# ThotDjehuty/polaroid

Hardware: AMD Instinct MI355X
Metric: Mrows/sec filter+groupby-agg on 1e9-row f64/i64; achieved HBM GB/s vs peak (higher is better)
Workload: dtype f64; 1 GPU; filter(close > 250).group_by(symbol).agg(open/high/low/close.sum()) 1e+09 rows per GPU, 100 groups (metric size; configs[1] = 1e8 rows); rows_per_gpu=1000000000, groups=100, global_batch=1000000000, columns=symbol:i64 open,high,low,close:f64, parallelism=single GPU

## Files before the change

### polaroid_amd/csrc/groupby.hip

```cpp
#include <hip/hip_runtime.h>

#include <algorithm>
#include <cmath>
#include <cstdio>
#include <cstdlib>
#include <cstring>
#include <mutex>
#include <numeric>
#include <string>
#include <tuple>
#include <vector>

#include "groupby_kernels.hpp"

namespace plgpu {

static int d2h_stage(int n, void* const* dst, const void* const* src, const size_t* bytes, hipStream_t s) {
    return plgpu_memcpy_d2h_many(n, dst, src, bytes, (void*)s);
}


#ifdef PLGPU_CHECKS
static std::vector<GbChecksTake>& gb_checks_takers() {
    static std::vector<GbChecksTake> v;
    return v;
}
void gb_checks_register(GbChecksTake f) { gb_checks_takers().push_back(f); }
#endif

constexpr int kPartMaxBits = 16;
constexpr int kPartOneLevel = 8;
constexpr int kPsDigitBits = 8;
constexpr int kPsThreads = 256;
constexpr int kPsPer = 16;
constexpr int kPsTile = kPsThreads * kPsPer;

struct PartOut {
    uint64_t* key;
    uint64_t* acc[kMaxAcc];
    uint32_t* rows;
    uint8_t* nulls;
    int64_t cap;
};

constexpr int kKeyRangeSlots = 256;
struct PsGeom {
    int64_t n;
    int64_t ntiles;
    const uint64_t* range;
    const uint32_t* tstart;
    const uint32_t* tpart;
    int32_t sh;
    int32_t dbits;
    int64_t* keyrange;
    int64_t sentinel;
    int32_t has_sentinel;
    int32_t _pad;
};

struct PsTile {
    int64_t base;
    int64_t lo, hi;
    int64_t mbase;
    int64_t ntq, tl;
};

__device__ __forceinline__ PsTile ps_tile(const PsGeom& g, int64_t t) {
    PsTile x;
    if (g.range == nullptr) {
        x.base = x.lo = t * kPsTile;
        x.hi = std::min<int64_t>(g.n, x.lo + kPsTile);
        x.mbase = 0;
        x.ntq = g.ntiles;
        x.tl = t;
    } else {
        const uint32_t q = g.tpart[t];
        const uint32_t t0 = g.tstart[q];
        x.ntq = (int64_t)(g.tstart[q + 1] - t0);
        x.tl = t - t0;
        x.mbase = (int64_t)t0 << g.dbits;
        const int64_t r0 = (int64_t)g.range[q], r1 = (int64_t)g.range[q + 1];
        x.base = (r0 & ~(int64_t)(kPsTile - 1)) + x.tl * kPsTile;
        x.lo = std::max<int64_t>(r0, x.base);
        x.hi = std::min<int64_t>(r1, x.base + kPsTile);
    }
    return x;
}

template <typename F>
__device__ __forceinline__ void ps_rows(const PsTile& tl, int c0, F&& f) {
    const uint32_t i0 = (uint32_t)(c0 + (int)(threadIdx.x & 63));
    if (tl.lo == tl.base && tl.hi - tl.base == kPsTile) {
#pragma unroll
        for (int k = 0; k < kPsPer; ++k) f(k, i0 + (uint32_t)(k * 64));
    } else {
        const uint32_t first = (uint32_t)(tl.lo - tl.base), last = (uint32_t)(tl.hi - tl.base - 1);
#pragma unroll
        for (int k = 0; k < kPsPer; ++k) f(k, min(max(i0 + (uint32_t)(k * 64), first), last));
    }
}

// ... 505 lines not shown
        if (runs) atomicAdd((unsigned long long*)&p.status[ST_RUNS], runs);
#pragma unroll
        for (int off = 32; off >= 1; off >>= 1) nlocal += __shfl_xor(nlocal, off, 64);
        if ((threadIdx.x & 63) == 0) red[0][threadIdx.x >> 6] = nlocal;
        __syncthreads();
        if (threadIdx.x == 0) {
            uint32_t t = 0;
            for (int w = 0; w < kPlanThreads / 64; ++w) t += red[0][w];
            atomicMax((unsigned long long*)&p.status[ST_LOCAL], (unsigned long long)t);
        }
        return;
    }
    const AccSpec& ac = p.acc[a];
    uint32_t mx = 0, mn = 0x7FF;
    const bool sqlo = ac.dop != DOP_NONE && (ac.dop & DOP_OPMASK) == DOP_SQLO;
    if (ac.flags & (A_FSUM | A_FSUMCAST)) {
        for (int64_t i0 = s0 + threadIdx.x; i0 < s1; i0 += (int64_t)blockDim.x * kPlanBatch) {
            uint64_t xb[kPlanBatch];
            bool okb[kPlanBatch];
#pragma unroll
            for (int u = 0; u < kPlanBatch; ++u) {
                const int64_t i = i0 + (int64_t)u * blockDim.x;
                const int64_t r = plan_row(i, n, samples);
                bool v = false;
                xb[u] = (i < s1 && r < n) ? acc_value(ac, r, v) : 0;
                if (psimple && i < s1 && r < n)
                    v = v && dev_valid(p.pred_col, r) && simple_pred(pisf, pop, dev_load(p.pred_col, r), pimm);
                okb[u] = i < s1 && r < n && v;
            }
#pragma unroll
            for (int u = 0; u < kPlanBatch; ++u) {
                if (!okb[u]) continue;
                uint64_t x = xb[u];
                if (ac.flags & A_FSUMCAST) x = f64_bits((double)(int64_t)x);
                const uint32_t ex = (uint32_t)(x >> 52) & 0x7FF;
                if (ex != 0x7FF && ex > mx) mx = ex;
                uint32_t el = ex;
                if (sqlo && ex != 0) {
                    const uint64_t m = (x & 0x000FFFFFFFFFFFFFull) | (1ull << 52);
                    el = ex + (uint32_t)__builtin_ctzll(m);
                }
                if ((x & 0x7fffffffffffffffull) != 0 && ex != 0x7FF && el < mn) mn = el;
            }
        }
    }
#pragma unroll
    for (int off = 32; off >= 1; off >>= 1) {
        const uint32_t o = __shfl_xor(mx, off, 64);
        mx = mx > o ? mx : o;
        const uint32_t q = __shfl_xor(mn, off, 64);
        mn = mn < q ? mn : q;
    }
    if ((threadIdx.x & 63) == 0) {
        red[0][threadIdx.x >> 6] = mx;
        red[1][threadIdx.x >> 6] = mn;
    }
    __syncthreads();
    if (threadIdx.x == 0) {
        for (int w = 1; w < kPlanThreads / 64; ++w) {
            mx = red[0][w] > mx ? red[0][w] : mx;
            mn = red[1][w] < mn ? red[1][w] : mn;
        }
        if (mx) atomicMax((unsigned long long*)&p.status[ST_MAXEX + a], (unsigned long long)mx);
        if (mn != 0x7FF) atomicMax((unsigned long long*)&p.status[ST_MINEX + a], (unsigned long long)(0x7FF - mn));
    }
}

static int32_t plan_bottom(uint64_t maxex) {
    int e = maxex == 0 ? 2046 : (int)maxex + kHeadroomBinades;
    if (e > 2046) e = 2046;
    return e - 1075 - (kSumWindowBits - 53);
}

__global__ void gb_init_table_kernel(uint64_t* gtab, int64_t words_per_field, int nfields, uint64_t min_init_mask) {
    for (int f = 0; f < nfields; ++f) {
        const uint64_t v = f == 0 ? kEmptyKey : (((min_init_mask >> f) & 1ull) ? ~0ull : 0ull);
        uint64_t* q = gtab + (int64_t)f * words_per_field;
        for (int64_t i = (int64_t)blockIdx.x * blockDim.x + threadIdx.x; i < words_per_field;
             i += (int64_t)gridDim.x * blockDim.x)
            q[i] = v;
    }
}


constexpr int kVarWords = 16;

__device__ __forceinline__ bool abs192(uint64_t& w0, uint64_t& w1, uint64_t& w2) {
    const bool neg = (int64_t)w2 < 0;
    if (neg) {
        w0 = ~w0; w1 = ~w1; w2 = ~w2;
        w0 += 1;
        const uint64_t c0 = w0 == 0;
        w1 += c0;
        w2 += (c0 && w1 == 0) ? 1 : 0;
    }
    return neg;
}

__device__ bool big_add_shifted(uint64_t (&acc)[kVarWords], const uint64_t* m, int k, int sh, bool negate) {
    int top = k - 1;
    while (top >= 0 && m[top] == 0) --top;
    if (top < 0) return true;
    const int bitlen = top * 64 + 64 - __clzll(m[top]);
    if (sh < 0 || bitlen + sh > kVarWords * 64 - 2) return false;
    const int ws = sh >> 6, bs = sh & 63;
    uint64_t carry = negate ? 1 : 0;
    for (int i = 0; i < kVarWords; ++i) {
        const int j = i - ws;
        uint64_t t = 0;
        if (j >= 0 && j <= k) {
            const uint64_t lo = j < k ? m[j] : 0ull;
            const uint64_t hi = (j >= 1 && j - 1 < k) ? m[j - 1] : 0ull;
            t = bs ? (lo << bs) | (hi >> (64 - bs)) : lo;
        }
        if (negate) t = ~t;
        const uint64_t s1 = acc[i] + t;
        const uint64_t c1 = s1 < t ? 1ull : 0ull;
        const uint64_t s2 = s1 + carry;
        const uint64_t c2 = s2 < s1 ? 1ull : 0ull;
        acc[i] = s2;
        carry = c1 | c2;
    }
    return true;
}

__device__ double big_to_double(const uint64_t (&acc)[kVarWords], int e2) {
    if ((int64_t)acc[kVarWords - 1] < 0) return 0.0;
    int t = kVarWords - 1;
    while (t >= 0 && acc[t] == 0) --t;
    if (t < 0) return 0.0;
    const int p = t * 64 + 63 - __clzll(acc[t]);
    const int q = p - 63;
    uint64_t x;
    bool sticky = false;
    if (q <= 0) {
        x = acc[0] << (-q);
    } else {
        const int w = q >> 6, b = q & 63;
        x = b ? (acc[w] >> b) | (acc[w + 1] << (64 - b)) : acc[w];
        sticky = b ? (acc[w] & ((1ull << b) - 1)) != 0 : false;
        for (int i = 0; i < w && !sticky; ++i) sticky = acc[i] != 0;
    }
    uint64_t keep = x >> 11;
    const uint64_t rem = x & 0x7FF;
    if (rem > 0x400 || (rem == 0x400 && (sticky || (keep & 1)))) ++keep;
    int ex = p - 52 + e2;
    if (keep == (1ull << 53)) {
        keep >>= 1;
        ++ex;
    }
    return ldexp((double)keep, ex);
}

__device__ bool var_exact(uint64_t a0, uint64_t a1, uint64_t a2, int b1, uint64_t h0, uint64_t h1, uint64_t h2,
                          int b2, uint64_t l0, uint64_t l1, uint64_t l2, int b3, uint64_t n, double& num) {
    (void)abs192(a0, a1, a2);
    const bool hneg = abs192(h0, h1, h2), lneg = abs192(l0, l1, l2);
    const uint64_t W1[3] = {a0, a1, a2};
    uint64_t sq[6] = {0, 0, 0, 0, 0, 0};
    for (int i = 0; i < 3; ++i) {
        unsigned __int128 c = 0;
        for (int j = 0; j < 3; ++j) {
            c += (unsigned __int128)W1[i] * W1[j] + sq[i + j];
            sq[i + j] = (uint64_t)c;
            c >>= 64;
        }
        sq[i + 3] = (uint64_t)c;
    }
    auto times_n = [&](uint64_t w0, uint64_t w1, uint64_t w2, uint64_t (&o)[4]) {
        unsigned __int128 c = (unsigned __int128)w0 * n;
        o[0] = (uint64_t)c;
        c = (c >> 64) + (unsigned __int128)w1 * n;
        o[1] = (uint64_t)c;
        c = (c >> 64) + (unsigned __int128)w2 * n;
        o[2] = (uint64_t)c;
        o[3] = (uint64_t)(c >> 64);
    };
    uint64_t nh[4], nl[4];
    times_n(h0, h1, h2, nh);
    times_n(l0, l1, l2, nl);
    const int e = min(min(b2, b3), 2 * b1);
    uint64_t acc[kVarWords];
    for (int i = 0; i < kVarWords; ++i) acc[i] = 0;
    if (!big_add_shifted(acc, nh, 4, b2 - e, hneg)) return false;
    if (!big_add_shifted(acc, nl, 4, b3 - e, lneg)) return false;
    if (!big_add_shifted(acc, sq, 6, 2 * b1 - e, true)) return false;
    num = big_to_double(acc, e);
    return true;
}

struct FinParams {
    OutSpec out[PLGPU_MAX_COLS * 2];
    int32_t nout;
    int32_t _pad;
    int64_t* out_keys;
    uint32_t* out_key_valid;
    uint64_t* out_first;
    int64_t cap;
    const double* wide[kMaxAcc];
    uint8_t* vbytes;
};

__device__ void fin_slot(const GbParams& p, const FinParams& fp, const uint64_t* tab, int64_t stride, int64_t s,
                         int special, int64_t g, uint64_t len) {
    if (g >= fp.cap) return;
    auto F = [&](int f) { return tab + (int64_t)f * stride + s; };
    const bool null_key = special == 1;
    fp.out_keys[g] = null_key ? 0 : (int64_t)(special == 2 ? kEmptyKey : *F(0));
    fp.vbytes[g] = null_key ? 0 : 1;
    if (fp.out_first) fp.out_first[g] = *F(p.f_first);
    for (int o = 0; o < fp.nout; ++o) {
        const OutSpec& os = fp.out[o];
        const AccSpec& ac = p.acc[os.acc];
        bool valid = true;
        const uint64_t cnt = ac.f_cnt >= 0 ? *F(ac.f_cnt) : len;
        const uint64_t flags = ac.f_flags >= 0 ? *F(ac.f_flags) : 0;
        switch (os.kind) {
        case PLGPU_AGG_LEN: ((uint32_t*)os.values)[g] = (uint32_t)len; break;
        case PLGPU_AGG_COUNT: ((uint32_t*)os.values)[g] = (uint32_t)cnt; break;
        case PLGPU_AGG_SUM:
        case PLGPU_AGG_MEAN: {
            if (os.kind == PLGPU_AGG_SUM && !os.in_isf) {
                dev_store(os.values, os.out_dtype, g, *F(ac.f_isum));
                break;
            }
            double sum;
            if (flags & FL_NAN || ((flags & FL_PINF) && (flags & FL_NINF))) sum = __builtin_nan("");
            else if (flags & FL_PINF) sum = __builtin_inf();
            else if (flags & FL_NINF) sum = -__builtin_inf();
            else if (fp.wide[os.acc]) sum = fp.wide[os.acc][s];
            else sum = fx_to_double(*F(ac.f_sum), *F(ac.f_sum + 1),
                                    *F(ac.f_sum + 2), p.bottoms[os.acc]);
            if (os.kind == PLGPU_AGG_MEAN) {
                if (cnt == 0) { valid = false; sum = 0.0; }
                else sum = sum / (double)cnt;
            }
            dev_store(os.values, os.out_dtype, g, f64_bits(sum));
            break;
        }
        case PLGPU_AGG_VAR:
        case PLGPU_AGG_STD: {
            double v = 0.0;
            if (cnt <= (uint64_t)os.ddof) {
                valid = false;
            } else if (flags) {
                v = __builtin_nan("");
            } else {
                const AccSpec& ah = p.acc[os.acc_hi];
                const AccSpec& al = p.acc[os.acc_lo];
                const uint64_t hf = *F(ah.f_flags) | *F(al.f_flags);
                double num = 0.0;
                const bool ok = hf == 0 &&
                                var_exact(*F(ac.f_sum), *F(ac.f_sum + 1),
                                          *F(ac.f_sum + 2), p.bottoms[os.acc],
                                          *F(ah.f_sum), *F(ah.f_sum + 1),
                                          *F(ah.f_sum + 2), p.bottoms[os.acc_hi],
                                          *F(al.f_sum), *F(al.f_sum + 1),
                                          *F(al.f_sum + 2), p.bottoms[os.acc_lo], cnt, num);
                if (!ok) {
                    atomicOr((unsigned long long*)&p.status[ST_VAR_OUT], 1ull);
                } else {
                    v = (num / (double)cnt) / (double)(cnt - (uint64_t)os.ddof);
                    if (os.kind == PLGPU_AGG_STD) v = __builtin_sqrt(v);
                }
            }
            ((double*)os.values)[g] = v;
            break;
        }
        case PLGPU_AGG_MIN:
        case PLGPU_AGG_MAX: {
            const uint64_t o = *F(os.kind == PLGPU_AGG_MIN ? ac.f_min : ac.f_max);
            const bool none = os.kind == PLGPU_AGG_MIN ? (o == ~0ull) : (o == 0ull);
            if (os.in_isf) {
                double v;
                if (cnt == 0) { valid = false; v = 0.0; }
                else if (none) v = __builtin_nan("");
                else v = as_f64(unord_f64(o));
                dev_store(os.values, os.out_dtype, g, f64_bits(v));
            } else {
                const uint64_t v = cnt == 0 ? 0ull : (os.in_uns ? o : (o ^ 0x8000000000000000ull));
                if (cnt == 0) valid = false;
                dev_store(os.values, os.out_dtype, g, v);
            }
            break;
        }
        case PLGPU_AGG_FIRST:
        case PLGPU_AGG_LAST: {
            const int64_t row = (int64_t)*F(os.kind == PLGPU_AGG_FIRST ? p.f_first : p.f_last);
            if (!gb_ok(row >= 0 && row < p.n, CK_FIRST_ROW)) {
                valid = false;
                break;
            }
            const uint64_t v0 = acc_value(ac, row, valid);
            const uint64_t v = valid ? v0 : 0ull;
            dev_store(os.values, os.out_dtype, g, v);
            break;
        }
        default: break;
        }
        if (os.validity) fp.vbytes[(int64_t)(1 + o) * fp.cap + g] = valid ? 1 : 0;
    }
}

__global__ __launch_bounds__(256) void gb_finalize_kernel(GbParams p, FinParams fp) {
    const int64_t total = p.gcap + 2;
    const int lane = threadIdx.x & 63, wid = threadIdx.x >> 6;
    const uint64_t lt = lane == 0 ? 0ull : (~0ull >> (64 - lane));
    __shared__ uint64_t wcnt[4];
    __shared__ unsigned long long gbase;
    const int64_t per = (((total + gridDim.x - 1) / gridDim.x) + 255) & ~int64_t(255);
    const int64_t lo = std::min<int64_t>(total, (int64_t)blockIdx.x * per), hi = std::min<int64_t>(total, lo + per);
    uint64_t mine = 0;
    for (int64_t s = lo + threadIdx.x; s < hi; s += blockDim.x) mine += *gfield(p, p.f_len, s) != 0 ? 1 : 0;
#pragma unroll
    for (int off = 32; off >= 1; off >>= 1) mine += __shfl_xor(mine, off, 64);
    if (lane == 0) wcnt[wid] = mine;
    __syncthreads();
    if (threadIdx.x == 0) {
        const uint64_t t = wcnt[0] + wcnt[1] + wcnt[2] + wcnt[3];
        gbase = t ? atomicAdd((unsigned long long*)&p.status[ST_GROUPS_OUT], (unsigned long long)t) : 0ull;
    }
    __syncthreads();
    uint64_t run = gbase;
    for (int64_t s0 = lo; s0 < hi; s0 += blockDim.x) {
        const int64_t s = s0 + threadIdx.x;
        const uint64_t len = s < hi ? *gfield(p, p.f_len, s) : 0ull;
        const uint64_t live = __ballot(len != 0);
        __syncthreads();
        if (lane == 0) wcnt[wid] = (uint64_t)__popcll(live);
        __syncthreads();
        uint64_t before = 0, chunk = 0;
        for (int w = 0; w < 4; ++w) {
            before += w < wid ? wcnt[w] : 0;
            chunk += wcnt[w];
        }
        const uint64_t base = run + before;
        run += chunk;
        if (len == 0) continue;
        const int64_t g = (int64_t)base + __popcll(live & lt);
        fin_slot(p, fp, p.gtab, p.gcap + 2, s, s == p.gcap ? 1 : (s == p.gcap + 1 ? 2 : 0), g, len);
    }
}

__global__ __launch_bounds__(256) void gb_finalize_regions_kernel(GbParams p, FinParams fp,
                                                                  const uint64_t* __restrict__ off, int lbits) {
    const int q = blockIdx.x;
    const uint64_t b = off[q], c = off[q + 1] - b;
    const int64_t t0 = (int64_t)q << lbits;
    for (uint64_t i = threadIdx.x; i < c; i += blockDim.x) {
        const int64_t s = t0 + (int64_t)i;
        fin_slot(p, fp, p.rtab, p.rcap, s, 0, (int64_t)(b + i), p.rtab[(int64_t)p.f_len * p.rcap + s]);
    }
    if (threadIdx.x == 0 && c) atomicAdd((unsigned long long*)&p.status[ST_GROUPS_OUT], (unsigned long long)c);
}

struct PackValid {
    uint32_t* dst[PLGPU_MAX_COLS * 2 + 1];
    int32_t n;
};
__global__ void gb_pack_valid_kernel(const uint8_t* __restrict__ vb, int64_t cap, PackValid pv) {
    const int64_t words = ((cap + 63) / 64) * 2;
    for (int64_t i = (int64_t)blockIdx.x * blockDim.x + threadIdx.x; i < words * pv.n;
         i += (int64_t)gridDim.x * blockDim.x) {
        const int c = (int)(i / words);
        const int64_t w = i - (int64_t)c * words;
        if (pv.dst[c] == nullptr) continue;
        const uint8_t* b = vb + (int64_t)c * cap + w * 32;
        const int m = (int)std::max<int64_t>(0, std::min<int64_t>(32, cap - w * 32));
        uint32_t bits = 0;
        for (int j = 0; j < m; ++j) bits |= (uint32_t)(b[j] != 0) << j;
        pv.dst[c][w] = bits;
    }
}

__global__ void widen_u32_kernel(const uint32_t* __restrict__ a, int64_t* __restrict__ b, int64_t n) {
    for (int64_t i = (int64_t)blockIdx.x * blockDim.x + threadIdx.x; i < n; i += (int64_t)gridDim.x * blockDim.x)
        b[i] = (int64_t)a[i];
}

template <typename T>
__global__ void gather_kernel(const T* __restrict__ src, const int64_t* __restrict__ perm, T* __restrict__ dst,
                              int64_t n) {
    for (int64_t i = (int64_t)blockIdx.x * blockDim.x + threadIdx.x; i < n; i += (int64_t)gridDim.x * blockDim.x)
        if (gb_ok(perm[i] >= 0 && perm[i] < n, CK_PERM)) dst[i] = src[perm[i]];
}
__global__ void narrow_i64_kernel(const int64_t* __restrict__ a, void* __restrict__ b, int32_t dt, int64_t n) {
    for (int64_t i = (int64_t)blockIdx.x * blockDim.x + threadIdx.x; i < n; i += (int64_t)gridDim.x * blockDim.x)
        dev_store(b, dt, i, (uint64_t)a[i]);
}
__global__ void gather_bits_kernel(const uint32_t* __restrict__ src, const int64_t* __restrict__ perm,
                                   uint32_t* __restrict__ dst, int64_t n) {
    const int64_t words = (n + 31) / 32;
    for (int64_t w = (int64_t)blockIdx.x * blockDim.x + threadIdx.x; w < words;
         w += (int64_t)gridDim.x * blockDim.x) {
        uint32_t bits = 0;
        const int m = (int)std::min<int64_t>(32, n - w * 32);
        for (int k = 0; k < m; ++k) {
            const int64_t j = perm[w * 32 + k];
            bits |= ((src[j >> 5] >> (j & 31)) & 1u) << k;
        }
        dst[w] = bits;
    }
}

__device__ __forceinline__ int dest_rank(uint64_t kind, uint64_t key, int world) {
    if (kind != 0 || world <= 1) return 0;
    const uint64_t h = (key ^ (key >> 31)) * 0xC2B2AE3D27D4EB4Full;
    return (int)((h >> 33) % (uint64_t)world);
}

__device__ __forceinline__ bool slot_record(const GbParams& p, int64_t s, uint64_t& kind, uint64_t& key) {
    if (*gfield(p, p.f_len, s) == 0) return false;
    kind = s == p.gcap ? 1 : (s == p.gcap + 1 ? 2 : 0);
    key = kind == 0 ? *gfield(p, 0, s) : (kind == 2 ? kEmptyKey : 0);
    return true;
}

__global__ void gb_export_count_kernel(GbParams p, int world, uint64_t* counts) {
    for (int64_t s = (int64_t)blockIdx.x * blockDim.x + threadIdx.x; s < p.gcap + 2;
         s += (int64_t)gridDim.x * blockDim.x) {
        uint64_t kind, key;
        if (!slot_record(p, s, kind, key)) continue;
        atomicAdd((unsigned long long*)&counts[dest_rank(kind, key, world)], 1ull);
    }
}

__global__ void gb_export_kernel(GbParams p, int world, uint64_t* cursor, uint64_t* out, WideRec wr, int rw) {
    for (int64_t s = (int64_t)blockIdx.x * blockDim.x + threadIdx.x; s < p.gcap + 2;
         s += (int64_t)gridDim.x * blockDim.x) {
        uint64_t kind, key;
        if (!slot_record(p, s, kind, key)) continue;
        const uint64_t idx = atomicAdd((unsigned long long*)&cursor[dest_rank(kind, key, world)], 1ull);
        uint64_t* r = out + idx * rw;
        r[0] = kind;
        r[1] = key;
        for (int f = 1; f < p.nfields; ++f) r[1 + f] = *gfield(p, f, s);
        for (int i = 0; i < wr.n; ++i) {
            const int64_t* d = wr.digits[i] + s * wr.nwords[i];
            for (int k = 0; k < wr.nwords[i]; ++k) r[wr.off[i] + k] = (uint64_t)d[k];
        }
    }
}

__device__ __forceinline__ bool shl192(uint64_t& w0, uint64_t& w1, uint64_t& w2, int d, int guard = 0) {
    if (d == 0 && guard == 0) return true;
    const uint64_t sign = (uint64_t)((int64_t)w2 >> 63);
    const int top = d + guard;
    if (top >= 191) return (w0 | w1 | w2) == 0;
    const uint64_t x[3] = {w0, w1, w2};
    for (int b = 191 - top; b < 192; b += 64) {
        const int lo = b, hi = b + 64 < 192 ? b + 64 : 192;
// ... 435 lines not shown
        if (rc) return rc;
        di.out_dtype = lp.out_dtype;
        di.kind = 0;
        di.cb = -1;
        if (lp.n == 1 && lp.code[0].op == D_COL) {
            di.kind = 1;
            di.ca = lp.code[0].arg;
            continue;
        }
        if (lp.n != 3 || lp.code[2].arg != PLGPU_F64) continue;
        int32_t op;
        switch (lp.code[2].op) {
        case D_ADD_F: op = DOP_ADD; break;
        case D_SUB_F: op = DOP_SUB; break;
        case D_MUL_F: op = DOP_MUL; break;
        case D_DIV_F: op = DOP_DIV; break;
        case D_DIV_FS: op = DOP_DIVS; break;
        default: continue;
        }
        const DevInstr &i0 = lp.code[0], &i1 = lp.code[1];
        auto f64col = [&](const DevInstr& i) { return i.op == D_COL && cols[i.arg].dtype == PLGPU_F64; };
        if (f64col(i0) && f64col(i1)) {
            di.kind = 2, di.ca = i0.arg, di.cb = i1.arg, di.dop = op;
        } else if (f64col(i0) && i1.op == D_LIT) {
            di.kind = 2, di.ca = i0.arg, di.dop = op | DOP_LIT, di.imm = i1.imm;
        } else if (i0.op == D_LIT && f64col(i1)) {
            di.kind = 2, di.ca = i1.arg, di.dop = op | DOP_LIT | DOP_SWAP, di.imm = i0.imm;
        }
    }
    return PLGPU_OK;
}

struct GbRun {
    Plan pl;
    DevProgram dp;
    int pred = 0;
    hipStream_t s = nullptr;
    DevBuf<uint64_t> status;
    int32_t* bottoms = nullptr;
    DevBuf<uint64_t> gtab;
    uint64_t st[ST_WORDS];
    int32_t hb[kMaxAcc];
    int gbits = 10;
    int attempts = 0;
    float ms = 0.f;
    int32_t key_dtype = PLGPU_I64;
    bool maintain = false;
    bool want_first = false;
    int world = 1;
    uint32_t wide = 0;
    int wide_exmin[kMaxAcc] = {0};
    int wide_exmax[kMaxAcc] = {0};
    DevBuf<int64_t> wide_digits[kMaxAcc];
    DevBuf<double> wide_sum[kMaxAcc];
    int64_t est_groups = -1;
    bool wide_round = true;
    std::string plan_ckey;
    bool kp_fallback = false;
    bool kp_bad = false;
    bool part = false;
    int pbits = 0;
    int part_lbits = 0;
    int part_blocks = 1;
    int part_levels = 0;
    int rbits = 0;
    bool compact_ok = false;
    bool compact_now = false;
    DevBuf<uint32_t> region_cnt;
    DevBuf<uint64_t> rtab;
    bool has_null_key = false;
    int64_t null_key = 0;
    DevBuf<uint64_t> pbuf;
    DevBuf<uint64_t> prange;
    const uint64_t* part_range = nullptr;
    int64_t part_rows_total = 0;
    std::vector<uint64_t> part_hrange;
    PartOut pout;
    const plgpu_column* cols = nullptr;
    int32_t ncols = 0;
    const Deriv* deriv = nullptr;
    std::vector<InSpec> ins;
    std::vector<plgpu_column> mat;
    std::vector<int> acc_input;

    GbRun() {
        std::memset(st, 0, sizeof st);
        std::memset(hb, 0, sizeof hb);
        std::memset(&pout, 0, sizeof pout);
    }
    ~GbRun() {
        for (auto& c : mat) plgpu_column_release(&c);
    }
};

static int d2h_status(GbRun& R) {
    void* d[1] = {R.st};
    const void* src[1] = {R.status};
    const size_t b[1] = {sizeof R.st};
    return d2h_stage(1, d, src, b, R.s);
}

static int gb_materialize(GbRun& R, int j, plgpu_column* out) {
    if (R.deriv == nullptr || j < 0 || j >= (int)R.deriv->in.size())
        return fail(PLGPU_ERR_INVALID, "internal: derived input index out of range");
    const DerivIn& di = R.deriv->in[j];
    plgpu_column c;
    std::memset(&c, 0, sizeof c);
    int rc;
    if (di.kind == 3) {
        const plgpu_column& x = R.cols[di.ca];
        if ((rc = make_owned_column(&c, PLGPU_F64, x.offset + x.length, false, R.s))) return rc;
        c.offset = x.offset;
        c.length = x.length;
        c.validity = x.validity;
        c.null_count = x.null_count;
        const int g = (int)std::min<int64_t>((x.length + 255) / 256, 256 * 32);
        if (x.length > 0) sq_split_kernel<<<g, 256, 0, R.s>>>(to_dev(x), x.length, di.dop, (uint64_t*)c.values);
        if (hipGetLastError() != hipSuccess) {
            plgpu_column_release(&c);
            return fail(PLGPU_ERR_HIP, "var square split");
        }
    } else {
        rc = plgpu_eval(R.cols, R.ncols, di.prog, di.n, &c, R.s);
        if (rc) return rc;
    }
    R.mat.push_back(c);
    *out = c;
    return PLGPU_OK;
}

static int gb_unfuse(GbRun& R) {
    GbParams& p = R.pl.p;
    for (int a = 0; a < p.nacc; ++a) {
        if (p.acc[a].dop == DOP_NONE) continue;
        plgpu_column c;
        int rc = gb_materialize(R, R.acc_input[a] - R.ncols, &c);
        if (rc) return rc;
        p.acc[a].c = to_dev(c);
        p.acc[a].dop = DOP_NONE;
        std::memset(&p.acc[a].c2, 0, sizeof p.acc[a].c2);
        if (p.pred_acc == a) p.pred_acc = -1;
    }
    return PLGPU_OK;
}

static bool gb_has_fused(const GbRun& R) {
    for (int a = 0; a < R.pl.p.nacc; ++a)
        if (R.pl.p.acc[a].dop != DOP_NONE) return true;
    return false;
}

static int gb_prepare(GbRun& R, const plgpu_column* key, const plgpu_column* cols, int32_t ncols,
                      const plgpu_instr* program, int32_t n_instr, const plgpu_agg* aggs, int32_t naggs,
                      bool maintain_order, bool force_counts, void* stream, const Deriv* deriv = nullptr) {
    R.s = as_stream(stream);
    if (key == nullptr) return fail(PLGPU_ERR_INVALID, "key is NULL");
    if (ncols < 0 || ncols > PLGPU_MAX_COLS) return fail(PLGPU_ERR_INVALID, "too many columns (max 8)");
    if (naggs < 0 || naggs > PLGPU_MAX_COLS * 2) return fail(PLGPU_ERR_INVALID, "too many aggregations (max 16)");
    if (!dtype_is_int(key->dtype)) return fail(PLGPU_ERR_SCHEMA, "group-by key must be an integer column");
    for (int i = 0; i < ncols; ++i)
        if (cols[i].length != key->length) return fail(PLGPU_ERR_SHAPE, "columns must match the key length");
    R.key_dtype = key->dtype;
    R.maintain = maintain_order;
    R.cols = cols;
    R.ncols = ncols;
    R.deriv = deriv;
    std::memset(&R.dp, 0, sizeof R.dp);
    int rc;
    if (program != nullptr && n_instr > 0) {
        if ((rc = lower_program(cols, ncols, program, n_instr, &R.dp))) return rc;
        if (R.dp.out_dtype != PLGPU_BOOL) return fail(PLGPU_ERR_SCHEMA, "filter predicate must be of type `Boolean`");
        R.pred = R.dp.simple ? 1 : 2;
    }
    R.ins = column_inputs(cols, ncols);
// ... 113 lines not shown
}

bool plan_cache_get(const std::string& key, PlanStats* out) {
    std::lock_guard<std::mutex> g(g_plan_mu);
    for (size_t i = g_plan_cache.size(); i-- > 0;) {
        if (g_plan_cache[i].first != key) continue;
        *out = g_plan_cache[i].second;
        std::rotate(g_plan_cache.begin() + (ptrdiff_t)i, g_plan_cache.begin() + (ptrdiff_t)i + 1, g_plan_cache.end());
        return true;
    }
    return false;
}

void plan_cache_erase(const std::string& key) {
    std::lock_guard<std::mutex> g(g_plan_mu);
    for (size_t i = 0; i < g_plan_cache.size(); ++i)
        if (g_plan_cache[i].first == key) {
            g_plan_cache.erase(g_plan_cache.begin() + (ptrdiff_t)i);
            return;
        }
}

void plan_cache_put(const std::string& key, const PlanStats& v) {
    std::lock_guard<std::mutex> g(g_plan_mu);
    for (auto& e : g_plan_cache)
        if (e.first == key) {
            e.second = v;
            return;
        }
    if (g_plan_cache.size() >= kPlanCacheEntries) g_plan_cache.erase(g_plan_cache.begin());
    g_plan_cache.emplace_back(key, v);
}
}

namespace {
std::vector<std::pair<std::string, MkPack>> g_pack_cache;

std::string pack_key(const MkKeys& mk, int64_t n) {
    std::string k((const char*)&mk, sizeof mk);
    k.append((const char*)&n, sizeof n);
    return k;
}

bool pack_cache_get(const std::string& key, MkPack* out) {
    std::lock_guard<std::mutex> g(g_plan_mu);
    for (auto& e : g_pack_cache)
        if (e.first == key) {
            *out = e.second;
            return true;
        }
    return false;
}

void pack_cache_put(const std::string& key, const MkPack& v) {
    std::lock_guard<std::mutex> g(g_plan_mu);
    for (auto& e : g_pack_cache)
        if (e.first == key) {
            e.second = v;
            return;
        }
    if (g_pack_cache.size() >= kPlanCacheEntries) g_pack_cache.erase(g_pack_cache.begin());
    g_pack_cache.emplace_back(key, v);
}
}

void gb_plan_cache_clear() {
    std::lock_guard<std::mutex> g(g_plan_mu);
    g_plan_cache.clear();
    g_pack_cache.clear();
}

static int gb_hll_count(GbRun& R, int64_t* out) {
    DevBuf<uint32_t> regs;
    std::vector<uint32_t> h(1 << kHllBits);
    int rc = regs.alloc(h.size() * 4, R.s);
    if (rc) return rc;
    hipError_t e = hipMemsetAsync(regs, 0, h.size() * 4, R.s);
    if (e == hipSuccess) {
        KtScope kt("gb_hll_kernel", R.s);
        gb_hll_kernel<<<num_cus() * 4, 256, 0, R.s>>>(R.pl.p.key, R.pl.p.n, regs);
        e = hipGetLastError();
    }
    if (e == hipSuccess) e = hipMemcpyAsync(h.data(), regs, h.size() * 4, hipMemcpyDeviceToHost, R.s);
    if (e == hipSuccess) e = hipStreamSynchronize(R.s);
    if (e != hipSuccess) return hip_fail(e, "gb_hll_kernel");
    *out = (int64_t)hll_estimate(h.data());
    return PLGPU_OK;
}

static int gb_plan(GbRun& R, const int32_t* fixed) {
    Plan& pl = R.pl;
    GbParams& p = pl.p;
    const int64_t n = p.n;
    const bool ps = R.pred == 1;
    const bool use_cache = fixed == nullptr && options().plan_cache != 0 && n >= (int64_t(1) << 24);
    const std::string ckey = use_cache ? plan_key(R) : std::string();
    PlanStats cached;
    const bool hit = use_cache && plan_cache_get(ckey, &cached);
    if (hit) {
        std::memcpy(R.st, cached.st, sizeof R.st);
        R.plan_ckey = ckey;
    } else {
        {
            KtScope kt("gb_plan_kernel", R.s);
            gb_plan_kernel<<<p.nacc * kPlanBlocks + kPlanKeyBlocks, kPlanThreads, 0, R.s>>>(
                p, R.status + kPlanSetWord, kPlanSamples, ps ? 1 : 0, ps ? R.dp.simple_isf : 0,
                ps ? R.dp.simple_op : 0, ps ? R.dp.simple_imm : 0ull);
        }
        PLGPU_HIP(hipGetLastError());
        if (int rs = d2h_status(R)) return rs;
        bool unsampled = false;
        for (int a = 0; a < p.nacc; ++a)
            if ((p.acc[a].flags & (A_FSUM | A_FSUMCAST)) && R.st[ST_MAXEX + a] == 0) unsampled = true;
        if (ps && unsampled) {
            gb_plan_kernel<<<p.nacc * kPlanBlocks, kPlanThreads, 0, R.s>>>(p, R.status + kPlanSetWord, kPlanSamples,
                                                                           0, 0, 0, 0ull);
            PLGPU_HIP(hipGetLastError());
            if (int rs = d2h_status(R)) return rs;
        }
        if (use_cache) {
            std::memcpy(cached.st, R.st, sizeof R.st);
            cached.hll = -1;
            plan_cache_put(ckey, cached);
        }
    }
    R.st[ST_SAMPLED] = (uint64_t)std::min<int64_t>(n, kPlanSamples);
    pl.runs = options().runs >= 0 ? options().runs != 0 : R.st[ST_RUNS] * 2 > R.st[ST_SAMPLED];
    for (int a = 0; a < kMaxAcc; ++a) R.hb[a] = a < p.nacc ? plan_bottom(R.st[ST_MAXEX + a]) : 0;
    if (fixed)
        for (int a = 0; a < kMaxAcc; ++a) R.hb[a] = fixed[a];
    int64_t hll = -1;
    const uint64_t local = R.st[ST_LOCAL];
    const uint64_t per_range = (uint64_t)std::min<int64_t>(n, kPlanSamples) / kPlanKeyBlocks;
    const bool clustered = n >= (int64_t(1) << 22) && local > 0 && local * 4 <= per_range * 3 && options().local != 0;
    if (clustered && R.st[ST_DISTINCT] >= (uint64_t)kPlanSetSlots / 2)
        hll = std::min<int64_t>(n, (int64_t)local * kPlanKeyBlocks * 2);
    if (hll < 0 && R.st[ST_DISTINCT] >= (uint64_t)kPlanSetSlots / 2 && n > 4 * (int64_t)kPlanSamples) {
        if (p.kp.n > 0) {
            if (options().debug)
                fprintf(stderr, "[plgpu] key pack fallback: %llu distinct of %llu sampled\n",
                        (unsigned long long)R.st[ST_DISTINCT], (unsigned long long)R.st[ST_SAMPLED]);
            R.kp_fallback = true;
            return PLGPU_OK;
        }
        if (hit && cached.hll >= 0) {
            hll = cached.hll;
        } else {
            int rc = gb_hll_count(R, &hll);
            if (rc) return rc;
            if (use_cache) {
                cached.hll = hll;
                plan_cache_put(ckey, cached);
            }
        }
    }
    size_tables(&pl, R.st[ST_DISTINCT], R.st[ST_SAMPLED], &R.gbits, hll, &R.est_groups);
    const int gpath = options().gb_path;
    if (gpath == 0) {
        pl.use_lds = false;
        pl.lds_bytes = 0;
    } else if ((gpath == 1 || gpath == 2) && !pl.use_lds) {
        int lb = 12;
        while (lb > 6 && (size_t)p.nfields * ((1u << lb) + 2) * 8 + kWgScratch > 160 * 1024) --lb;
        pl.use_lds = true;
        p.lbits = lb;
        p.lcap = 1 << lb;
        pl.lds_bytes = (size_t)p.nfields * (p.lcap + 2) * 8;
    }
    pl.local = false;
    const int lbits0 = p.lbits, lcap0 = p.lcap;
    const size_t lds0 = pl.lds_bytes;
    {
        if (!pl.use_lds && clustered && gpath < 0) {
            const int lb = log2_ceil(std::max<int64_t>(64, 2 * (int64_t)local));
            const size_t bytes = (size_t)p.nfields * ((1u << lb) + 2) * 8;
            if (bytes + kWgScratch <= (size_t)160 * 1024) {
                pl.local = pl.use_lds = true;
                p.lbits = lb;
// ... 152 lines not shown
    case 1: return gbp_pass<1, false, false, NUL>(R, g, none, cnt, part, scatter, out);
    default: return gbp_pass<2, false, false, NUL>(R, g, none, cnt, part, scatter, out);
    }
}
static hipError_t gbp_pass1(const GbRun& R, bool f8, bool nul, const PsGeom& g, uint32_t* cnt, uint64_t* part,
                            bool scatter, const PartOut& out) {
    return nul ? gbp_pass1_nul<true>(R, f8, g, cnt, part, scatter, out)
               : gbp_pass1_nul<false>(R, f8, g, cnt, part, scatter, out);
}

static int gbp_alloc(GbRun& R, int64_t sel, bool nul, DevBuf<uint64_t>* owner, PartOut* o) {
    const GbParams& p = R.pl.p;
    const int64_t rows = ((int64_t)std::max<int64_t>(sel, 2) + 17) & ~int64_t(15);
    const bool want_rows = p.f_first >= 0 || p.f_last >= 0;
    const size_t rwords = want_rows ? ((size_t)rows + 1) / 2 : 0;
    const size_t words = (size_t)rows * (1 + p.nacc) + rwords + (nul ? ((size_t)rows + 7) / 8 : 0);
    int rc = owner->alloc(words * 8, R.s);
    if (rc) return rc;
    uint64_t* buf = owner->get();
    std::memset(o, 0, sizeof *o);
    o->key = buf;
    for (int a = 0; a < p.nacc; ++a) o->acc[a] = buf + (size_t)rows * (1 + a);
    o->rows = want_rows ? (uint32_t*)(buf + (size_t)rows * (1 + p.nacc)) : nullptr;
    o->nulls = nul ? (uint8_t*)(buf + (size_t)rows * (1 + p.nacc) + rwords) : nullptr;
    o->cap = rows;
    return PLGPU_OK;
}

static int gb_partition(GbRun& R) {
    GbParams& p = R.pl.p;
    hipStream_t s = R.s;
    if (p.key.values == nullptr || p.key.dtype == PLGPU_STR || p.n <= 0 || p.n >= 0xFFFFFFFFll)
        return fail(PLGPU_ERR_INVALID, "partitioned group-by: needs a key column and 1 .. 2^32 - 1 rows");
    for (int a = 0; a < p.nacc; ++a)
        if (p.acc[a].c.values == nullptr)
            return fail(PLGPU_ERR_INVALID, "partitioned group-by: an aggregated column without values");
    const int B = R.pbits;
    const int lv = options().part_levels;
    const bool two = B >= 2 && (B > kPartOneLevel || lv == 2) && !(lv == 1 && B <= kPartOneLevel);
    const int b1 = two ? B / 2 : B, b2 = B - b1;
    const int P1 = 1 << b1, P = 1 << B;
    auto c8 = [](const DevCol& c) { return dtype_bytes(c.dtype) == 8 && c.dtype != PLGPU_STR; };
    bool f8 = c8(p.key) && R.pred <= 1 && (R.pred == 0 || c8(p.pred_col));
    for (int a = 0; a < p.nacc; ++a) f8 = f8 && c8(p.acc[a].c);
    bool nul = p.key.validity != nullptr || (R.pred == 1 && p.pred_col.validity != nullptr);
    const bool nul_cnt = nul;
    for (int a = 0; a < p.nacc; ++a) nul = nul || p.acc[a].c.validity != nullptr;
    bool nul_out = R.pl.sum_only ? p.key.validity != nullptr : nul;
    const bool want_sent = R.pl.sum_only && p.key.validity != nullptr && p.key.dtype == PLGPU_I64 && f8 &&
                           options().part_null_sentinel != 0;
    PsGeom g1;
    std::memset(&g1, 0, sizeof g1);
    g1.n = p.n;
    g1.ntiles = (p.n + kPsTile - 1) / kPsTile;
    g1.sh = b1 ? 64 - b1 : 0;
    g1.dbits = b1;
    const int64_t ncnt1 = g1.ntiles << b1;
    DevBuf<uint32_t> cnt;
    DevBuf<uint64_t> part;
    int rc = R.prange.alloc((size_t)(P + 1 + (two ? P1 + 1 : 0)) * 8, s);
    uint64_t* range = R.prange;
    uint64_t* range1 = two ? R.prange + P + 1 : range;
    if (!rc) rc = cnt.alloc((size_t)ncnt1 * 4, s);
    if (!rc)
        rc = part.alloc((size_t)((ncnt1 + kScanChunk - 1) / kScanChunk + 2 + 2 * kKeyRangeSlots) * 8, s);
    std::vector<uint64_t> hr1((size_t)P1 + 1);
    std::vector<int64_t> krange(2 * kKeyRangeSlots);
    for (int i = 0; i < kKeyRangeSlots; ++i) krange[2 * i] = INT64_MAX, krange[2 * i + 1] = INT64_MIN;
    if (!rc && want_sent) {
        g1.keyrange = (int64_t*)(part + (ncnt1 + kScanChunk - 1) / kScanChunk + 2);
        if (hipMemcpyAsync(g1.keyrange, krange.data(), krange.size() * 8, hipMemcpyHostToDevice, s) != hipSuccess)
            rc = fail(PLGPU_ERR_HIP, "key range init");
    }
    if (!rc) {
        hipError_t e = gbp_pass1(R, f8, nul_cnt, g1, cnt, part, false, R.pout);
        const int64_t nb = std::max<int64_t>(1, (ncnt1 + kScanChunk - 1) / kScanChunk);
        if (e == hipSuccess) {
            gbp_bounds_kernel<<<(P1 + 256) / 256, 256, 0, s>>>(cnt, part + nb, P1, g1.ntiles, range1);
            e = hipGetLastError();
        }
        if (e == hipSuccess) e = hipMemcpyAsync(hr1.data(), range1, (size_t)(P1 + 1) * 8, hipMemcpyDeviceToHost, s);
        if (e == hipSuccess && g1.keyrange)
            e = hipMemcpyAsync(krange.data(), g1.keyrange, krange.size() * 8, hipMemcpyDeviceToHost, s);
        if (e == hipSuccess) e = hipStreamSynchronize(s);
        if (e != hipSuccess) rc = hip_fail(e, "gbp_count_kernel");
    }
    R.has_null_key = false;
    if (!rc && g1.keyrange) {
        int64_t lo = INT64_MAX, hi = INT64_MIN;
        for (int i = 0; i < kKeyRangeSlots; ++i) lo = std::min(lo, krange[2 * i]), hi = std::max(hi, krange[2 * i + 1]);
        if (lo > hi) R.null_key = 0, R.has_null_key = true;
        else if (hi < INT64_MAX) R.null_key = hi + 1, R.has_null_key = true;
        else if (lo > INT64_MIN + 1) R.null_key = lo - 1, R.has_null_key = true;
        g1.keyrange = nullptr;
        if (R.has_null_key) {
            g1.has_sentinel = 1;
            g1.sentinel = R.null_key;
            nul_out = false;
        }
    }
    DevBuf<uint64_t> buf1;
    PartOut out1;
    if (!rc) rc = gbp_alloc(R, (int64_t)hr1[P1], nul_out, &buf1, &out1);
    if (!rc) {
        const hipError_t e = gbp_pass1(R, f8, nul, g1, cnt, part, true, out1);
        if (e != hipSuccess) rc = hip_fail(e, "gbp_scatter_kernel");
    }
    cnt.reset();
    part.reset();
    if (rc) return rc;
    std::vector<uint64_t> hr;
    if (!two) {
        R.pbuf = std::move(buf1);
        R.pout = out1;
        hr = hr1;
    } else {
        std::vector<uint32_t> ts((size_t)P1 + 1);
        uint64_t t = 0;
        for (int q = 0; q < P1; ++q) {
            ts[q] = (uint32_t)t;
            if (hr1[q + 1] > hr1[q]) t += ((hr1[q + 1] - 1) / kPsTile) - (hr1[q] / kPsTile) + 1;
        }
        ts[P1] = (uint32_t)t;
        PsGeom g2;
        std::memset(&g2, 0, sizeof g2);
        g2.ntiles = (int64_t)t;
        g2.range = range1;
        g2.sh = 64 - B;
        g2.dbits = b2;
        g2.has_sentinel = g1.has_sentinel;
        g2.sentinel = g1.sentinel;
        const int64_t ncnt2 = g2.ntiles << b2;
        DevBuf<uint32_t> meta;
        rc = meta.alloc((size_t)(P1 + 1 + std::max<int64_t>(g2.ntiles, 1)) * 4, s);
        if (!rc) rc = cnt.alloc((size_t)std::max<int64_t>(ncnt2, 1) * 4, s);
        if (!rc) rc = part.alloc((size_t)((ncnt2 + kScanChunk - 1) / kScanChunk + 2) * 8, s);
        hr.resize((size_t)P + 1);
        if (!rc) {
            g2.tstart = meta;
            g2.tpart = meta + P1 + 1;
            hipError_t e = hipMemcpyAsync(meta, ts.data(), ts.size() * 4, hipMemcpyHostToDevice, s);
            if (e == hipSuccess && g2.ntiles > 0) {
                gbp_tpart_kernel<<<(unsigned)std::min<int64_t>((g2.ntiles + 255) / 256, 4096), 256, 0, s>>>(
                    meta, P1, g2.ntiles, meta + P1 + 1);
                e = hipGetLastError();
            }
            if (e == hipSuccess && g2.ntiles > 0)
                e = nul_out ? gbp_pass<0, true, true, true>(R, g2, out1, cnt, part, false, out1)
                            : gbp_pass<0, true, true>(R, g2, out1, cnt, part, false, out1);
            if (e == hipSuccess) {
                gbp_bounds2_kernel<<<(P + 256) / 256, 256, 0, s>>>(cnt, range1, meta, P1, b2, range);
                e = hipGetLastError();
            }
            if (e == hipSuccess) e = hipMemcpyAsync(hr.data(), range, (size_t)(P + 1) * 8, hipMemcpyDeviceToHost, s);
            if (e == hipSuccess) e = hipStreamSynchronize(s);
            if (e != hipSuccess) rc = hip_fail(e, "gbp_count_kernel (level 2)");
        }
        if (!rc) rc = gbp_alloc(R, (int64_t)hr[P], nul_out, &R.pbuf, &R.pout);
        if (!rc && g2.ntiles > 0) {
            const hipError_t e = nul_out ? gbp_pass<0, true, true, true>(R, g2, out1, cnt, part, true, R.pout)
                                         : gbp_pass<0, true, true>(R, g2, out1, cnt, part, true, R.pout);
            if (e != hipSuccess) rc = hip_fail(e, "gbp_scatter_kernel (level 2)");
        }
        if (rc) return rc;
    }
    uint64_t maxpart = 0;
    for (int q = 0; q < P; ++q) maxpart = std::max<uint64_t>(maxpart, hr[q + 1] - hr[q]);
    R.part_hrange = hr;
    R.part_rows_total = (int64_t)hr[P];
    R.part_range = range;
    R.part_levels = two ? 2 : 1;
    const int64_t wpc = 4;
    int nb = (int)std::max<int64_t>(1, (wpc * (int64_t)num_cus() + P - 1) / P);
    while ((int64_t)maxpart > (int64_t)nb * (kMaxRowsPerWg / 2)) nb *= 2;
    R.part_blocks = nb;
    if (nb == 1 && options().part_direct != 0) {
        R.rbits = R.part_lbits;
        R.gbits = R.pbits + R.part_lbits;
    }
    return PLGPU_OK;
}

int radix_partition8(const DevCol& key, const DevCol* cols, int ncols, int64_t n, int bits, hipStream_t s,
                     RadixParts* out) {
    if (ncols < 0 || ncols > kMaxAcc || bits < 0 || bits > kPartMaxBits || n <= 0 || n >= 0xFFFFFFFFll)
        return fail(PLGPU_ERR_INVALID, "radix partition: 0..6 columns, 0..16 bits, 1 .. 2^32 - 1 rows");
    auto c8 = [](const DevCol& c) {
        return c.values != nullptr && c.validity == nullptr && dtype_bytes(c.dtype) == 8 && c.dtype != PLGPU_STR;
    };
    if (!c8(key)) return fail(PLGPU_ERR_INVALID, "radix partition: null-free 8-byte columns");
    for (int i = 0; i < ncols; ++i)
        if (!c8(cols[i])) return fail(PLGPU_ERR_INVALID, "radix partition: null-free 8-byte columns");
    GbRun R;
    R.s = s;
    GbParams& p = R.pl.p;
    std::memset(&p, 0, sizeof p);
    p.key = key;
    p.n = n;
    p.nacc = ncols;
    for (int i = 0; i < ncols; ++i) p.acc[i].c = cols[i];
    p.pred_acc = -1;
    p.f_first = p.f_last = -1;
    R.pred = 0;
    R.pbits = bits;
    const int rc = gb_partition(R);
    if (rc) return rc;
    out->buf = std::move(R.pbuf);
    out->key = R.pout.key;
    for (int i = 0; i < ncols; ++i) out->col[i] = R.pout.acc[i];
    out->range = std::move(R.prange);
    out->bounds = R.part_range;
    out->hrange = R.part_hrange;
    out->levels = R.part_levels;
    return PLGPU_OK;
}

static hipError_t launch_partitioned(const GbRun& R) {
    Plan pp = R.pl;
    GbParams& q = pp.p;
    const GbParams& p = R.pl.p;
    std::memset(&q.key, 0, sizeof q.key);
    q.key.values = R.pout.key;
    q.key.dtype = PLGPU_I64;
    for (int a = 0; a < p.nacc; ++a) {
        DevCol c;
        std::memset(&c, 0, sizeof c);
        c.values = R.pout.acc[a];
        c.dtype = p.acc[a].isf ? PLGPU_F64 : PLGPU_I64;
        q.acc[a].c = c;
    }
    q.n = R.part_rows_total;
    q.row_begin = 0;
    q.n_full = 0;
    q.part_range = R.part_range;
    q.part_rows = R.pout.rows;
    q.part_nulls = R.pout.nulls;
    q.has_null_key = R.has_null_key ? 1 : 0;
    q.null_key = R.null_key;
    q.part_blocks = R.part_blocks;
    q.lbits = R.part_lbits;
    q.lcap = 1 << R.part_lbits;
    if (pp.sum_only && p.nacc >= 1 && p.nacc <= 6) {
        const int grid = (1 << R.pbits) * R.part_blocks;
        switch (p.nacc) {
        case 1: return launch_part_fast_limbs<1>(pp, grid, R.s);
        case 2: return launch_part_fast_limbs<2>(pp, grid, R.s);
        case 3: return launch_part_fast_limbs<3>(pp, grid, R.s);
        case 4: return launch_part_fast_limbs<4>(pp, grid, R.s);
        case 5: return launch_part_fast_limbs<5>(pp, grid, R.s);
        default: return launch_part_fast_limbs<6>(pp, grid, R.s);
        }
    }
    const size_t lds = (size_t)p.nfields * (q.lcap + 2) * 8;
    static bool attr_set = false;
    if (!attr_set) {
        (void)hipFuncSetAttribute((const void*)gb_kernel<0, true, true>, hipFuncAttributeMaxDynamicSharedMemorySize,
                                  160 * 1024);
        attr_set = true;
    }
    DevProgram none;
    std::memset(&none, 0, sizeof none);
    gb_kernel<0, true, true><<<(1 << R.pbits) * R.part_blocks, kGbThreads, lds, R.s>>>(q, none);
    return hipGetLastError();
}

static int gb_alloc_table(GbRun& R) {
    GbParams& p = R.pl.p;
    R.gtab.reset();
    R.rtab.reset();
    p.rtab = nullptr;
    p.rcap = 0;
    p.region_cnt = nullptr;
    p.gbits = R.gbits;
    p.rbits = R.rbits;
    if (R.compact_now) {
        p.rcap = int64_t(1) << (R.pbits + R.part_lbits);
        int rc = R.rtab.alloc((size_t)p.rcap * p.nfields * 8, R.s);
        if (rc) return rc;
        p.rtab = R.rtab;
        p.region_cnt = R.region_cnt;
        p.gbits = std::max(16, R.pbits + 2);
        p.rbits = 0;
    }
    p.gcap = int64_t(1) << p.gbits;
    const size_t wpf = (size_t)(p.gcap + 2);
    int rc = R.gtab.alloc(wpf * p.nfields * 8, R.s);
    if (rc) return rc;
    p.gtab = R.gtab;
    const int ig = (int)std::min<int64_t>((int64_t)(wpf + 255) / 256, 256 * 8);
    gb_init_table_kernel<<<ig, 256, 0, R.s>>>(R.gtab, (int64_t)wpf, p.nfields, p.min_init_mask);
    PLGPU_HIP(hipMemsetAsync(R.status, 0, 6 * 8, R.s));
    PLGPU_HIP(hipMemsetAsync(R.status + ST_MAXEX, 0, (ST_WORDS - ST_MAXEX) * 8, R.s));
    PLGPU_HIP(hipGetLastError());
    return PLGPU_OK;
}

static int gb_refit(GbRun& R, uint32_t flagged, int32_t* hint, bool* changed, uint32_t* wide) {
    GbParams& p = R.pl.p;
    *changed = false;
    *wide = 0;
    for (int a = 0; a < kMaxAcc; ++a) hint[a] = R.hb[a];
    if (!flagged) return PLGPU_OK;
    for (int a = 0; a < p.nacc; ++a)
        if ((flagged >> a) & 1u) gb_maxexp_kernel<<<std::max(1, num_cus() * 4), 256, 0, R.s>>>(p, a);
    PLGPU_HIP(hipGetLastError());
    if (int rs = d2h_status(R)) return rs;
    for (int a = 0; a < p.nacc; ++a) {
        if (!((flagged >> a) & 1u)) continue;
        const int tmax = std::max((int)R.st[ST_MAXEX + a], 1);
        const int tmin = std::max(0x7FF - (int)R.st[ST_MINEX + a], 1);
        if (tmax - tmin <= kSumWindowBits - 53) {
            hint[a] = tmax - 1075 - (kSumWindowBits - 53);
            *changed = *changed || hint[a] != R.hb[a];
        } else {
            *wide |= 1u << a;
            R.wide_exmin[a] = std::min(tmin, tmax);
            R.wide_exmax[a] = tmax;
        }
    }
    return PLGPU_OK;
}

static int gb_wide(GbRun& R, bool round = true) {
    GbParams& p = R.pl.p;
    for (int a = 0; a < p.nacc; ++a) {
        if (!((R.wide >> a) & 1u)) continue;
        R.wide_digits[a].reset();
        R.wide_sum[a].reset();
        const int exmin = R.wide_exmin[a];
        const int nwords = wide_nwords(exmin, R.wide_exmax[a]);
        const size_t slots = (size_t)(p.gcap + 2);
        int rc = R.wide_digits[a].alloc(slots * nwords * 8, R.s);
        if (!rc && round) rc = R.wide_sum[a].alloc(slots * 8, R.s);
        if (rc) return rc;
        PLGPU_HIP(hipMemsetAsync(R.wide_digits[a], 0, slots * nwords * 8, R.s));
        const int g = std::max(1, num_cus() * 8);
        if (R.pred == 0) gb_wide_kernel<0><<<g, 256, 0, R.s>>>(p, R.dp, a, exmin, nwords, R.wide_digits[a]);
        else if (R.pred == 1) gb_wide_kernel<1><<<g, 256, 0, R.s>>>(p, R.dp, a, exmin, nwords, R.wide_digits[a]);
        else gb_wide_kernel<2><<<g, 256, 0, R.s>>>(p, R.dp, a, exmin, nwords, R.wide_digits[a]);
        if (round) {
            const int fg = (int)std::min<int64_t>((p.gcap + 2 + 255) / 256, 256 * 16);
            gb_wide_round_kernel<<<fg, 256, 0, R.s>>>(p, exmin, nwords, R.wide_digits[a], R.wide_sum[a]);
        }
        PLGPU_HIP(hipGetLastError());
    }
    return PLGPU_OK;
}

static int wide_layout(const GbRun& R, WideRec& wr) {
    std::memset(&wr, 0, sizeof wr);
    int w = R.pl.p.nfields + 1;
    for (int a = 0; a < R.pl.p.nacc; ++a) {
        if (!((R.wide >> a) & 1u)) continue;
        wr.acc[wr.n] = a;
        wr.nwords[wr.n] = wide_nwords(R.wide_exmin[a], R.wide_exmax[a]);
        wr.off[wr.n] = w;
        wr.digits[wr.n] = R.wide_digits[a];
        w += wr.nwords[wr.n];
        ++wr.n;
    }
    return w;
}

static int gb_main(GbRun& R, bool auto_refit, bool* refit, int32_t* hint) {
    Plan& pl = R.pl;
    GbParams& p = pl.p;
    const int64_t n = p.n;
    const bool debug = options().debug != 0;
    if (refit) *refit = false;
    hipEvent_t ev0 = ev_acquire(), ev1 = ev_acquire();
    if (ev0 == nullptr || ev1 == nullptr) {
        ev_release(ev0);
        ev_release(ev1);
        return fail(PLGPU_ERR_HIP, "hipEventCreate failed");
    }
    int rc = PLGPU_OK;
    if (R.part && n > 0 && R.pbuf == nullptr) rc = gb_partition(R);
    for (R.attempts = 0; rc == PLGPU_OK; ++R.attempts) {
        R.compact_now = R.compact_ok && R.part && n > 0 && pl.sum_only && pl.limbs == 2 && R.rbits > 0 &&
                        R.part_blocks == 1 && R.wide == 0 && options().part_compact != 0;
        if (R.compact_now && R.region_cnt == nullptr &&
            (rc = R.region_cnt.alloc(((size_t)1 << R.pbits) * 4, R.s)))
            break;
        if ((rc = gb_alloc_table(R))) break;
        PLGPU_HIP(hipMemcpyAsync(R.bottoms, R.hb, sizeof R.hb, hipMemcpyHostToDevice, R.s));
        for (int a = 0; a < kMaxAcc; ++a) p.bottom[a] = R.hb[a];
        PLGPU_HIP(hipEventRecord(ev0, R.s));
        if (n > 0 && R.part) {
            KtScope kt("gb_part_agg_kernel", R.s);
            PLGPU_HIP(launch_partitioned(R));
        } else if (n > 0) {
            if (p.n_full > 0) {
                PLGPU_HIP(launch_fast_dispatch(pl, R.dp, R.pred, R.s));
            } else {
                PLGPU_HIP(launch_main_dispatch(pl, R.dp, R.pred, R.s));
            }
        }
        PLGPU_HIP(hipEventRecord(ev1, R.s));
        if (int rs = d2h_status(R)) return rs;
        if (debug) {
            fprintf(stderr,
                    "[plgpu] gb attempt %d: n=%lld grid=%d/%d lds=%d lcap=%d gcap=%lld nfields=%d lds_bytes=%zu "
                    "fast=%lld sumonly=%d distinct=%llu/%llu newkeys=%llu special=%llu global_rows=%llu full=%llu "
                    "selected=%llu fx=%llx limbs=%d runs=%d nacc=%d\n",
                    R.attempts, (long long)n, pl.grid, pl.fast_grid, (int)pl.use_lds, p.lcap, (long long)p.gcap,
                    p.nfields, pl.lds_bytes, (long long)p.n_full, (int)pl.sum_only,
                    (unsigned long long)R.st[ST_DISTINCT], (unsigned long long)R.st[ST_SAMPLED],
                    (unsigned long long)R.st[ST_NEWKEYS], (unsigned long long)R.st[ST_SPECIAL],
                    (unsigned long long)R.st[ST_GLOBAL_ROWS], (unsigned long long)R.st[ST_TABLE_FULL],
                    (unsigned long long)R.st[ST_SELECTED], (unsigned long long)R.st[ST_FXFLAGS], pl.limbs, (int)pl.runs,
                    p.nacc);
        }
        if (R.st[ST_KPACK]) {
            R.kp_bad = true;
            break;
        }
        bool again = false;
        if (R.st[ST_TABLE_FULL] > 0 && R.compact_now) {
            R.compact_ok = false;
            again = true;
        } else if (R.st[ST_TABLE_FULL] > 0) {
            R.rbits = 0;
            R.gbits = std::max(R.gbits + 3, log2_ceil((int64_t)R.st[ST_NEWKEYS] * 4));
            if (R.attempts == 0 && p.key.values != nullptr && p.kp.n == 0) {
                int64_t hll = 0;
                if ((rc = gb_hll_count(R, &hll))) break;
                R.gbits = std::max(R.gbits, log2_ceil(std::min<int64_t>(n, hll + hll / 4 + 1024) * 2));
            }
            again = true;
        }
        uint32_t flagged = 0;
        for (int a = 0; a < p.nacc; ++a)
            if ((p.acc[a].flags & (A_FSUM | A_FSUMCAST)) && ((R.st[ST_FXFLAGS] >> (2 * a)) & 3u)) flagged |= 1u << a;
        flagged &= ~R.wide;
        if (flagged && pl.limbs == 2 && (p.n_full > 0 || R.part) && pl.sum_only) {
            pl.limbs = 3;
            again = true;
            uint32_t over = 0;
            for (int a = 0; a < p.nacc; ++a)
                if ((R.st[ST_FXFLAGS] >> (2 * a)) & 1u) over |= 1u << a;
            flagged = over;
        }
        if (flagged) {
            int32_t h[kMaxAcc];
            bool changed = false;
            uint32_t wide = 0;
            if ((rc = gb_refit(R, flagged, h, &changed, &wide))) break;
            if (wide && !auto_refit) {
                rc = fail(PLGPU_ERR_CAPACITY,
                          "f64 sum: the values of one column span more binades than the partitioned "
                          "group-by's fixed-point window; use the single-GPU group-by for this column");
                break;
            }
            R.wide |= wide;
            if (wide && R.compact_now) again = true;
            if (changed) {
                if (auto_refit) {
                    for (int a = 0; a < kMaxAcc; ++a)
                        if (!((R.wide >> a) & 1u)) R.hb[a] = h[a];
                    again = true;
                } else {
                    if (refit) *refit = true;
                    if (hint)
                        for (int a = 0; a < kMaxAcc; ++a) hint[a] = h[a];
                }
            }
        }
        if (!again) break;
        if (R.attempts >= 3) {
            rc = fail(PLGPU_ERR_CAPACITY, "group-by did not converge after retries");
            break;
        }
    }
    if (rc == PLGPU_OK) (void)hipEventElapsedTime(&R.ms, ev0, ev1);
    ev_release(ev0);
    ev_release(ev1);
    if (!R.plan_ckey.empty() &&
        (rc != PLGPU_OK || R.attempts > 0 || R.kp_bad ||
         (int64_t)R.st[ST_NEWKEYS] > 2 * std::max<int64_t>(R.est_groups, 4096)))
        plan_cache_erase(R.plan_ckey);
    if (rc == PLGPU_OK && R.wide && !R.kp_bad) rc = gb_wide(R, R.wide_round);
    return rc;
}

static int64_t gb_groups(const GbRun& R) {
    return (int64_t)R.st[ST_NEWKEYS] + ((R.st[ST_SPECIAL] & 1) ? 1 : 0) + ((R.st[ST_SPECIAL] & 2) ? 1 : 0);
}

static void gb_fill_info(const GbRun& R, plgpu_groupby_info* info) {
    const GbParams& p = R.pl.p;
    std::memset(info, 0, sizeof *info);
    info->rows_in = p.n;
    info->rows_selected = (int64_t)R.st[ST_SELECTED];
    info->groups = gb_groups(R);
    info->global_path_rows = (int64_t)R.st[ST_GLOBAL_ROWS];
    info->reruns = R.attempts;
    info->lds_slots = R.pl.use_lds ? p.lcap : 0;
    info->grid = p.n_full > 0 ? R.pl.launched_grid : R.pl.grid;
    info->table_capacity = p.gcap;
    info->main_kernel_ms = R.ms;
    info->path = R.part ? 3 : (p.n_full > 0 ? (R.pl.launched_var ? 4 : (R.pl.sum_only ? 2 : 1)) : 0);
    info->sum_limbs = (p.n_full > 0 || R.part) && R.pl.sum_only ? R.pl.limbs : 3;
    info->local_range = R.pl.local ? 1 : 0;
    info->register_runs = p.n_full > 0 && !R.part && R.pl.launched_runs ? 1 : 0;
    info->key_pack = p.kp.n;
    info->part_layout = R.part ? (R.pbits | (R.part_levels << 8)) : 0;
    info->fused_variant = p.n_full > 0 && !R.part ? R.pl.launched_variant : 0;
    for (int a = 0; a < p.nacc; ++a)
        if (((R.st[ST_FXFLAGS] >> (2 * a)) & 2u) && !((R.wide >> a) & 1u)) info->sum_inexact |= 1 << a;
}

static int gb_finalize(GbRun& R, int32_t naggs, plgpu_column* out_key, plgpu_column* out_aggs,
                       DevBuf<uint64_t>* keep_first = nullptr) {
    Plan& pl = R.pl;
    GbParams& p = pl.p;
    hipStream_t s = R.s;
    const int64_t groups = gb_groups(R);
    FinParams fp;
    std::memset(&fp, 0, sizeof fp);
    int rc = make_owned_column(out_key, PLGPU_I64, groups, true, s);
    for (int i = 0; i < naggs && rc == PLGPU_OK; ++i) {
        const OutSpec& o = pl.outs[i];
        const bool nullable = o.kind == PLGPU_AGG_MEAN || o.kind == PLGPU_AGG_MIN || o.kind == PLGPU_AGG_MAX ||
                              o.kind == PLGPU_AGG_FIRST || o.kind == PLGPU_AGG_LAST || o.kind == PLGPU_AGG_VAR ||
                              o.kind == PLGPU_AGG_STD;
        if (o.kind == PLGPU_AGG_VAR || o.kind == PLGPU_AGG_STD) {
            const bool wide = ((R.wide >> o.acc) | (R.wide >> o.acc_hi) | (R.wide >> o.acc_lo)) & 1u;
            if (wide || R.hb[o.acc] < -484)
                rc = fail(PLGPU_ERR_CAPACITY, "var: the fused second moment is out of its exact range");
        }
        if (rc == PLGPU_OK) rc = make_owned_column(&out_aggs[i], o.out_dtype, groups, nullable, s);
    }
    DevBuf<uint64_t> first;
    if (rc == PLGPU_OK && (R.maintain || keep_first) && groups > 0) rc = first.alloc(groups * 8, s);
    if (rc == PLGPU_OK && groups > 0) {
        fp.nout = naggs;
        for (int i = 0; i < naggs; ++i) {
            fp.out[i] = pl.outs[i];
            fp.out[i].values = (void*)out_aggs[i].values;
            fp.out[i].validity = (uint32_t*)out_aggs[i].validity;
        }
        fp.out_keys = (int64_t*)out_key->values;
        fp.out_key_valid = (uint32_t*)out_key->validity;
        fp.out_first = first;
        fp.cap = groups;
        for (int a = 0; a < kMaxAcc; ++a) fp.wide[a] = R.wide_sum[a];
        DevBuf<uint8_t> vbytes;
        rc = vbytes.alloc((size_t)(1 + naggs) * groups, s);
        if (rc) {
            plgpu_column_release(out_key);
            for (int i = 0; i < naggs; ++i) plgpu_column_release(&out_aggs[i]);
            return rc;
        }
        fp.vbytes = vbytes;
        const int fg = (int)std::min<int64_t>((p.gcap + 2 + 255) / 256, 256 * 16);
        DevBuf<uint64_t> roff;
        const int nreg = R.compact_now ? 1 << R.pbits : 0;
        if (nreg) {
            const int64_t nb = std::max<int64_t>(1, (nreg + kScanChunk - 1) / kScanChunk);
            rc = roff.alloc((size_t)(nreg + 1 + nb + 2) * 8, s);
            if (!rc && scan_exclusive<uint32_t>(R.region_cnt, nreg, roff, roff + nreg + 1, s) != hipSuccess)
                rc = fail(PLGPU_ERR_HIP, "region count scan");
            if (rc) {
                plgpu_column_release(out_key);
                for (int i = 0; i < naggs; ++i) plgpu_column_release(&out_aggs[i]);
                return rc;
            }
        }
        {
            KtScope kt("gb_finalize_kernel", s);
            if (nreg) gb_finalize_regions_kernel<<<nreg, 256, 0, s>>>(p, fp, roff, R.part_lbits);
            gb_finalize_kernel<<<fg, 256, 0, s>>>(p, fp);
            PackValid pv;
            std::memset(&pv, 0, sizeof pv);
            pv.n = 1 + naggs;
            pv.dst[0] = (uint32_t*)out_key->validity;
            for (int i = 0; i < naggs; ++i) pv.dst[1 + i] = (uint32_t*)out_aggs[i].validity;
            const int64_t work = ((groups + 63) / 64) * 2 * pv.n;
            gb_pack_valid_kernel<<<(unsigned)std::min<int64_t>((work + 255) / 256, 4096), 256, 0, s>>>(vbytes, groups,
                                                                                                       pv);
        }
        vbytes.reset();
        roff.reset();
        hipError_t e = hipGetLastError();
        if (e != hipSuccess) rc = hip_fail(e, "gb_finalize_kernel");
        uint64_t produced = 0, var_out = 0;
        if (rc == PLGPU_OK) {
            void* d[2] = {&produced, &var_out};
            const void* src[2] = {R.status + ST_GROUPS_OUT, R.status + ST_VAR_OUT};
            const size_t b[2] = {8, 8};
            rc = d2h_stage(2, d, src, b, s);
        }
        if (rc == PLGPU_OK && var_out)
            rc = fail(PLGPU_ERR_CAPACITY, "var: the fused second moment is out of its exact range");
        if (rc == PLGPU_OK && (int64_t)produced != groups) {
            char buf[256];
            snprintf(buf, sizeof buf,
                     "internal: group count mismatch (inserted %llu + specials %llu, finalized %llu, "
                     "global rows %llu, table_full %llu)",
                     (unsigned long long)R.st[ST_NEWKEYS], (unsigned long long)R.st[ST_SPECIAL],
                     (unsigned long long)produced, (unsigned long long)R.st[ST_GLOBAL_ROWS],
                     (unsigned long long)R.st[ST_TABLE_FULL]);
            rc = fail(PLGPU_ERR_CAPACITY, buf);
        }
    }
    if (rc == PLGPU_OK && R.maintain && groups > 1) {
        plgpu_column fc, pidx;
        std::memset(&fc, 0, sizeof fc);
        std::memset(&pidx, 0, sizeof pidx);
        fc.dtype = PLGPU_I64;
        fc.length = groups;
        fc.values = first;
        rc = plgpu_arg_sort(&fc, 0, 0, &pidx, s);
        DevBuf<int64_t> dperm;
        if (rc == PLGPU_OK) rc = dperm.alloc(groups * 8, s);
        if (rc == PLGPU_OK) {
            const int gg = (int)std::min<int64_t>((groups + 255) / 256, 4096);
            widen_u32_kernel<<<gg, 256, 0, s>>>((const uint32_t*)pidx.values, dperm, groups);
            auto permute = [&](plgpu_column* c) -> int {
                plgpu_column nc;
                int r2 = make_owned_column(&nc, c->dtype, groups, c->validity != nullptr, s);
                if (r2) return r2;
                switch (dtype_bytes(c->dtype)) {
                case 8:
                    gather_kernel<uint64_t><<<gg, 256, 0, s>>>((const uint64_t*)c->values, dperm,
                                                               (uint64_t*)nc.values, groups);
                    break;
                case 4:
                    gather_kernel<uint32_t><<<gg, 256, 0, s>>>((const uint32_t*)c->values, dperm,
                                                               (uint32_t*)nc.values, groups);
                    break;
                case 2:
                    gather_kernel<uint16_t><<<gg, 256, 0, s>>>((const uint16_t*)c->values, dperm,
                                                               (uint16_t*)nc.values, groups);
                    break;
                case 1:
                    gather_kernel<uint8_t><<<gg, 256, 0, s>>>((const uint8_t*)c->values, dperm,
                                                              (uint8_t*)nc.values, groups);
                    break;
                default:
                    plgpu_column_release(&nc);
                    return fail(PLGPU_ERR_SCHEMA, "group order: unsupported output dtype");
                }
                if (c->validity) {
                    (void)hipMemsetAsync((void*)nc.validity, 0, ((groups + 63) / 64) * 8, s);
                    gather_bits_kernel<<<gg, 256, 0, s>>>((const uint32_t*)c->validity, dperm,
                                                          (uint32_t*)nc.validity, groups);
                }
                plgpu_column_release(c);
                *c = nc;
                return PLGPU_OK;
            };
            rc = permute(out_key);
            for (int i = 0; i < naggs && rc == PLGPU_OK; ++i) rc = permute(&out_aggs[i]);
            if (rc == PLGPU_OK && keep_first) {
                DevBuf<uint64_t> sf;
                rc = sf.alloc(groups * 8, s);
                if (rc == PLGPU_OK) {
                    gather_kernel<uint64_t><<<gg, 256, 0, s>>>(first, dperm, sf, groups);
                    first = std::move(sf);
                }
            }
            hipError_t e = hipGetLastError();
            if (rc == PLGPU_OK && e != hipSuccess) rc = hip_fail(e, "permute");
        }
        dperm.reset();
        plgpu_column_release(&pidx);
    }
    if (rc == PLGPU_OK && R.key_dtype != PLGPU_I64 && dtype_bytes(R.key_dtype) > 0) {
        plgpu_column nk;
        rc = make_owned_column(&nk, R.key_dtype, groups, true, s);
        if (rc == PLGPU_OK && groups > 0) {
            const int gg = (int)std::min<int64_t>((groups + 255) / 256, 4096);
            narrow_i64_kernel<<<gg, 256, 0, s>>>((const int64_t*)out_key->values, (void*)nk.values, R.key_dtype,
                                                 groups);
            (void)hipMemcpyAsync((void*)nk.validity, out_key->validity, ((groups + 63) / 64) * 8,
                                 hipMemcpyDeviceToDevice, s);
        }
        if (rc == PLGPU_OK) {
            plgpu_column_release(out_key);
            *out_key = nk;
        }
    }
    if (rc == PLGPU_OK) {
        out_key->null_count = (R.st[ST_SPECIAL] & 1) ? 1 : 0;
        hipError_t e = hipStreamSynchronize(s);
        if (e != hipSuccess) rc = hip_fail(e, "finalize sync");
    }
    if (rc == PLGPU_OK && keep_first) *keep_first = std::move(first);
    if (rc) {
        plgpu_column_release(out_key);
        for (int i = 0; i < naggs; ++i) plgpu_column_release(&out_aggs[i]);
    }
    return rc;
}

__global__ void mk_hash_kernel(MkKeys k, int64_t n, uint64_t seed, uint64_t mask, uint64_t* __restrict__ out) {
    for (int64_t r = (int64_t)blockIdx.x * blockDim.x + threadIdx.x; r < n; r += (int64_t)gridDim.x * blockDim.x) {
        out[r] = mk_row_hash(k, r, seed) & mask;
    }
}

__device__ __forceinline__ int64_t g_lookup(const GbParams& p, uint64_t key) {
    if (key == kEmptyKey) return p.gcap + 1;
    const int lim = g_probe_limit(p);
    for (int i = 0; i < lim; ++i) {
        const uint64_t s = g_slot(p, key, (uint64_t)i);
        const uint64_t k = p.gtab[s];
        if (k == key) return (int64_t)s;
        if (k == kEmptyKey) return -1;
    }
    return -1;
}

__global__ __launch_bounds__(256) void mk_rep_kernel(GbParams p, MkKeys k, uint64_t* __restrict__ vw,
                                                     uint32_t* __restrict__ vm) {
    const int64_t total = p.gcap + 2;
    for (int64_t s = (int64_t)blockIdx.x * blockDim.x + threadIdx.x; s < total; s += (int64_t)gridDim.x * blockDim.x) {
        if (*gfield(p, p.f_len, s) == 0) continue;
        const int64_t rep = (int64_t)*gfield(p, p.f_first, s);
        if (!gb_ok(rep >= 0 && rep < p.n, CK_REP_ROW)) continue;
        uint32_t m = 0;
        for (int i = 0; i < k.n; ++i) {
            const bool v = dev_valid(k.c[i], rep);
            m |= (v ? 1u : 0u) << i;
            vw[(int64_t)i * total + s] = v ? mk_word(k.c[i], rep) : 0ull;
        }
        vm[s] = m;
    }
}

__global__ __launch_bounds__(256) void mk_verify_kernel(GbParams p, MkKeys k, const uint64_t* __restrict__ hashes,
                                                        int64_t n, const uint64_t* __restrict__ vw,
                                                        const uint32_t* __restrict__ vm,
                                                        uint32_t* __restrict__ collision) {
    const int64_t total = p.gcap + 2;
    bool bad = false;
    for (int64_t r = (int64_t)blockIdx.x * blockDim.x + threadIdx.x; r < n; r += (int64_t)gridDim.x * blockDim.x) {
        const int64_t s = g_lookup(p, hashes[r]);
        if (s < 0 || !gb_ok(s < total, CK_VERIFY_SLOT) || *gfield(p, p.f_len, s) == 0) continue;
        const uint32_t m = vm[s];
        for (int i = 0; i < k.n; ++i) {
            const bool v = dev_valid(k.c[i], r);
            bad |= v != (bool)((m >> i) & 1u);
            if (!v) continue;
            if (k.c[i].dtype == PLGPU_STR)
                bad |= !str_equal(k.c[i], r, k.c[i], (int64_t)*gfield(p, p.f_first, s));
            else
                bad |= mk_word(k.c[i], r) != vw[(int64_t)i * total + s];
        }
    }
    if (__any(bad) && (threadIdx.x & 63) == 0) atomicOr(collision, 1u);
}

__global__ void mk_gather_key_kernel(DevCol c, const uint64_t* __restrict__ rows, int64_t g_n, int64_t n, void* out,
                                     uint32_t* out_valid) {
    for (int64_t g = (int64_t)blockIdx.x * blockDim.x + threadIdx.x; g < g_n; g += (int64_t)gridDim.x * blockDim.x) {
        const int64_t r = (int64_t)rows[g];
        if (!gb_ok(r >= 0 && r < n, CK_KEY_ROW)) continue;
        const bool v = dev_valid(c, r);
        const uint64_t x = dev_load(c, r);
        if (c.dtype == PLGPU_BOOL) {
            if (x & 1) atomicOr(&((uint32_t*)out)[g >> 5], 1u << (g & 31));
        } else {
            dev_store(out, c.dtype, g, x);
        }
        if (out_valid && v) atomicOr(&out_valid[g >> 5], 1u << (g & 31));
    }
}

}

using namespace plgpu;

static int gb_single_impl(const plgpu_column* key, const plgpu_column* cols, int32_t ncols, const Deriv* deriv,
                          const plgpu_instr* program, int32_t n_instr, const plgpu_agg* aggs, int32_t naggs,
                          int32_t maintain_order, plgpu_column* out_key, plgpu_column* out_aggs,
                          plgpu_groupby_info* info, void* stream) {
    if (out_key == nullptr) return fail(PLGPU_ERR_INVALID, "out_key is NULL");
    std::memset(out_key, 0, sizeof *out_key);
    for (int i = 0; i < naggs && out_aggs; ++i) std::memset(&out_aggs[i], 0, sizeof(plgpu_column));
    GbRun R;
    int rc = gb_prepare(R, key, cols, ncols, program, n_instr, aggs, naggs, maintain_order != 0, false, stream,
                        deriv);
    R.compact_ok = maintain_order == 0;
    if (!rc) rc = gb_plan(R, nullptr);
    if (!rc) rc = gb_main(R, true, nullptr, nullptr);
    if (rc) return rc;
    if (info) gb_fill_info(R, info);
    return gb_finalize(R, naggs, out_key, out_aggs);
}

PLGPU_API int plgpu_group_by_agg(const plgpu_column* key, const plgpu_column* cols, int32_t ncols,
                                 const plgpu_instr* program, int32_t n_instr, const plgpu_agg* aggs, int32_t naggs,
                                 int32_t maintain_order, plgpu_column* out_key, plgpu_column* out_aggs,
                                 plgpu_groupby_info* info, void* stream) {
    return gb_single_impl(key, cols, ncols, nullptr, program, n_instr, aggs, naggs, maintain_order, out_key,
                          out_aggs, info, stream);
}

PLGPU_API int plgpu_debug_checks(uint32_t* out) {
    if (out == nullptr) return fail(PLGPU_ERR_INVALID, "NULL argument");
    *out = 0;
#ifdef PLGPU_CHECKS
    PLGPU_HIP(hipDeviceSynchronize());
    for (GbChecksTake f : gb_checks_takers()) *out |= f();
    return PLGPU_OK;
#else
    return PLGPU_OK;
#endif
}

struct plgpu_gb_partial {
    GbRun run;
};

PLGPU_API int plgpu_gb_record_words(const plgpu_column* cols, int32_t ncols, const plgpu_agg* aggs, int32_t naggs,
                                    int32_t* out_words) {
    if (out_words == nullptr || (cols == nullptr && ncols > 0)) return fail(PLGPU_ERR_INVALID, "NULL argument");
    if (ncols < 0 || ncols > PLGPU_MAX_COLS) return fail(PLGPU_ERR_INVALID, "too many columns (max 8)");
    std::vector<plgpu_column> c2(cols, cols + ncols);
    for (auto& c : c2) c.length = 0;
    plgpu_column k;
    std::memset(&k, 0, sizeof k);
    k.dtype = PLGPU_I64;
    Plan pl;
    DevProgram dp;
    std::memset(&dp, 0, sizeof dp);
    const std::vector<InSpec> ins = column_inputs(c2.data(), ncols);
    const int rc = plan_groupby(&k, c2.data(), ncols, ins.data(), ncols, aggs, naggs, false, dp, &pl, true);
    if (rc) return rc;
    *out_words = pl.p.nfields + 1;
    return PLGPU_OK;
}

PLGPU_API int plgpu_gb_plan_bottoms(const plgpu_column* key, const plgpu_column* cols, int32_t ncols,
                                    const plgpu_agg* aggs, int32_t naggs, int32_t* out_bottoms, void* stream) {
    if (out_bottoms == nullptr) return fail(PLGPU_ERR_INVALID, "out_bottoms is NULL");
    GbRun R;
    int rc = gb_prepare(R, key, cols, ncols, nullptr, 0, aggs, naggs, false, true, stream);
    if (!rc) rc = gb_plan(R, nullptr);
    if (rc) return rc;
    for (int a = 0; a < kMaxAcc; ++a) out_bottoms[a] = R.hb[a];
    return PLGPU_OK;
}

PLGPU_API int plgpu_gb_partial_begin(const plgpu_column* key, const plgpu_column* cols, int32_t ncols,
                                     const plgpu_instr* program, int32_t n_instr, const plgpu_agg* aggs,
                                     int32_t naggs, const int32_t* bottoms, int32_t world, plgpu_gb_partial** out,
                                     int64_t* out_records, int32_t* out_bottoms_used, int32_t* out_refit,
                                     int32_t* out_bottoms_hint, plgpu_groupby_info* info, void* stream) {
    if (out == nullptr || out_records == nullptr || out_bottoms_used == nullptr || out_refit == nullptr ||
        out_bottoms_hint == nullptr)
        return fail(PLGPU_ERR_INVALID, "NULL argument");
    if (world < 1) return fail(PLGPU_ERR_INVALID, "world must be >= 1");
    *out = nullptr;
    for (int i = 0; i < naggs && aggs; ++i)
        if (aggs[i].kind == PLGPU_AGG_FIRST || aggs[i].kind == PLGPU_AGG_LAST)
            return fail(PLGPU_ERR_INVALID, "first / last aggregations are not supported on the partitioned path");
    plgpu_gb_partial* h = new plgpu_gb_partial();
    GbRun& R = h->run;
    R.world = world;
    R.wide_round = false;
    bool refit = false;
    int rc = gb_prepare(R, key, cols, ncols, program, n_instr, aggs, naggs, false, true, stream);
    if (!rc) rc = gb_plan(R, bottoms);
    if (!rc) rc = gb_main(R, bottoms == nullptr, &refit, out_bottoms_hint);
    if (rc) {
        delete h;
        return rc;
    }
    for (int a = 0; a < kMaxAcc; ++a) {
        out_bottoms_used[a] = R.hb[a];
        if (!refit) out_bottoms_hint[a] = R.hb[a];
    }
    *out_refit = refit ? 1 : 0;
    *out_records = gb_groups(R);
    if (info) gb_fill_info(R, info);
    *out = h;
    return PLGPU_OK;
}

PLGPU_API int plgpu_gb_partial_wide(const plgpu_gb_partial* h, int32_t* out_wide, int32_t* out_exmin,
                                    int32_t* out_exmax) {
    if (h == nullptr || out_wide == nullptr || out_exmin == nullptr || out_exmax == nullptr)
        return fail(PLGPU_ERR_INVALID, "NULL argument");
    const GbRun& R = h->run;
    const GbParams& p = R.pl.p;
    for (int a = 0; a < kMaxAcc; ++a) {
        out_wide[a] = 0;
        out_exmin[a] = 0x7FF;
        out_exmax[a] = 0;
        if (a >= p.nacc || !(p.acc[a].flags & (A_FSUM | A_FSUMCAST))) continue;
        if ((R.wide >> a) & 1u) {
            out_wide[a] = 1;
            out_exmin[a] = R.wide_exmin[a];
            out_exmax[a] = R.wide_exmax[a];
        } else {
            out_exmin[a] = std::max(1, R.hb[a] + 1075);
            out_exmax[a] = std::min(0x7FE, std::max(out_exmin[a], R.hb[a] + 1075 + kSumWindowBits - 53));
        }
    }
    return PLGPU_OK;
}

PLGPU_API int plgpu_gb_partial_set_wide(plgpu_gb_partial* h, const int32_t* wide, const int32_t* exmin,
                                        const int32_t* exmax) {
    if (h == nullptr || wide == nullptr || exmin == nullptr || exmax == nullptr)
        return fail(PLGPU_ERR_INVALID, "NULL argument");
    GbRun& R = h->run;
    const GbParams& p = R.pl.p;
    uint32_t mask = 0;
    for (int a = 0; a < kMaxAcc; ++a) {
        if (!wide[a]) continue;
        if (a >= p.nacc || !(p.acc[a].flags & (A_FSUM | A_FSUMCAST)))
            return fail(PLGPU_ERR_INVALID, "wide: only f64 sums take digit states");
        if (exmin[a] < 1 || exmax[a] > 0x7FE || exmin[a] > exmax[a])
            return fail(PLGPU_ERR_INVALID, "wide: bad exponent range");
        if (((R.wide >> a) & 1u) && (exmin[a] > R.wide_exmin[a] || exmax[a] < R.wide_exmax[a]))
            return fail(PLGPU_ERR_INVALID, "wide: the agreed range must cover this rank's");
        mask |= 1u << a;
    }
    if (mask == 0) return R.wide ? fail(PLGPU_ERR_INVALID, "wide: this rank holds a wide sum") : PLGPU_OK;
    if ((R.wide & ~mask) != 0) return fail(PLGPU_ERR_INVALID, "wide: this rank holds a wide sum");
    R.wide = mask;
    for (int a = 0; a < kMaxAcc; ++a)
        if ((mask >> a) & 1u) {
            R.wide_exmin[a] = exmin[a];
            R.wide_exmax[a] = exmax[a];
        }
    int rc = gb_wide(R, false);
    if (rc == PLGPU_OK) {
        hipError_t e = hipStreamSynchronize(R.s);
        if (e != hipSuccess) rc = hip_fail(e, "gb_wide_kernel");
    }
    return rc;
}

PLGPU_API int plgpu_gb_partial_record_words(const plgpu_gb_partial* h, int32_t* out_words) {
    if (h == nullptr || out_words == nullptr) return fail(PLGPU_ERR_INVALID, "NULL argument");
    WideRec wr;
    *out_words = wide_layout(h->run, wr);
    return PLGPU_OK;
}

PLGPU_API int plgpu_gb_partial_export(plgpu_gb_partial* h, void* dst_records, int64_t* out_counts, void* stream) {
    if (h == nullptr || out_counts == nullptr) return fail(PLGPU_ERR_INVALID, "NULL argument");
    GbRun& R = h->run;
    hipStream_t s = stream ? as_stream(stream) : R.s;
    const GbParams& p = R.pl.p;
    const int W = R.world;
    WideRec wr;
    const int rw = wide_layout(R, wr);
    for (int i = 0; i < wr.n; ++i)
        if (wr.digits[i] == nullptr) return fail(PLGPU_ERR_INVALID, "wide: digits missing");
    DevBuf<uint64_t> counts;
    int rc = counts.alloc((size_t)W * 16, s);
    if (rc) return rc;
    PLGPU_HIP(hipMemsetAsync(counts, 0, (size_t)W * 16, s));
    const int fg = (int)std::min<int64_t>((p.gcap + 2 + 255) / 256, 256 * 16);
    gb_export_count_kernel<<<fg, 256, 0, s>>>(p, W, counts);
    std::vector<uint64_t> hc(W), cur(W);
    PLGPU_HIP(hipMemcpyAsync(hc.data(), counts, (size_t)W * 8, hipMemcpyDeviceToHost, s));
    PLGPU_HIP(hipStreamSynchronize(s));
    uint64_t run = 0;
    for (int w = 0; w < W; ++w) {
        cur[w] = run;
        run += hc[w];
        out_counts[w] = (int64_t)hc[w];
    }
    if (run > 0) {
        if (dst_records == nullptr) return fail(PLGPU_ERR_INVALID, "dst_records is NULL");
        PLGPU_HIP(hipMemcpyAsync(counts + W, cur.data(), (size_t)W * 8, hipMemcpyHostToDevice, s));
        gb_export_kernel<<<fg, 256, 0, s>>>(p, W, counts + W, (uint64_t*)dst_records, wr, rw);
        PLGPU_HIP(hipGetLastError());
    }
    PLGPU_HIP(hipStreamSynchronize(s));
    return PLGPU_OK;
}

PLGPU_API void plgpu_gb_partial_free(plgpu_gb_partial* h) { delete h; }

__device__ __forceinline__ int route_rank(const DevCol& key, int64_t r, int world) {
    if (!dev_valid(key, r)) return dest_rank(1, 0, world);
    const uint64_t k = dev_load(key, r);
    return dest_rank(k == kEmptyKey ? 2 : 0, k, world);
}

__global__ void gb_route_kernel(DevCol key, int64_t n, int world, int pass, unsigned long long* ctr,
                                uint32_t* __restrict__ perm) {
    for (int64_t r = (int64_t)blockIdx.x * blockDim.x + threadIdx.x; r < n; r += (int64_t)gridDim.x * blockDim.x) {
        const int d = route_rank(key, r, world);
        const unsigned long long at = atomicAdd(&ctr[d], 1ull);
        if (pass) perm[at] = (uint32_t)r;
    }
}

PLGPU_API int plgpu_gb_route(const plgpu_column* key, int32_t world, plgpu_column* out_perm, int64_t* out_counts,
                             void* stream) {
    if (key == nullptr || out_perm == nullptr || out_counts == nullptr) return fail(PLGPU_ERR_INVALID, "NULL argument");
    if (world < 1 || world > 1024) return fail(PLGPU_ERR_INVALID, "world must be 1..1024");
    if (!dtype_is_int(key->dtype) || dtype_bytes(key->dtype) > 8 || key->dtype == PLGPU_U64)
        return fail(PLGPU_ERR_SCHEMA, "route key must be a signed or 32-bit integer column");
    const int64_t n = key->length;
    if (n < 0 || n >= 0xFFFFFFFFll) return fail(PLGPU_ERR_CAPACITY, "route input exceeds the u32 index space");
    std::memset(out_perm, 0, sizeof *out_perm);
    hipStream_t s = as_stream(stream);
    int rc = make_owned_column(out_perm, PLGPU_U32, n, false, s);
    if (rc) return rc;
    DevBuf<unsigned long long> ctr;
    if ((rc = ctr.alloc((size_t)world * 16, s))) {
        plgpu_column_release(out_perm);
        return rc;
    }
    const DevCol k = to_dev(*key);
    const int g = (int)std::max<int64_t>(1, std::min<int64_t>((n + 255) / 256, 4096));
    std::vector<unsigned long long> hc(world), cur(world);
    hipError_t e = hipMemsetAsync(ctr, 0, (size_t)world * 8, s);
    if (e == hipSuccess && n > 0) {
        gb_route_kernel<<<g, 256, 0, s>>>(k, n, world, 0, ctr, nullptr);
        e = hipGetLastError();
    }
    if (e == hipSuccess) e = hipMemcpyAsync(hc.data(), ctr, (size_t)world * 8, hipMemcpyDeviceToHost, s);
    if (e == hipSuccess) e = hipStreamSynchronize(s);
    unsigned long long run = 0;
    for (int w = 0; w < world; ++w) {
        cur[w] = run;
        run += hc[w];
        out_counts[w] = (int64_t)hc[w];
    }
    if (e == hipSuccess && n > 0) {
        e = hipMemcpyAsync(ctr + world, cur.data(), (size_t)world * 8, hipMemcpyHostToDevice, s);
        if (e == hipSuccess) {
            gb_route_kernel<<<g, 256, 0, s>>>(k, n, world, 1, ctr + world, (uint32_t*)out_perm->values);
            e = hipGetLastError();
        }
        if (e == hipSuccess) e = hipStreamSynchronize(s);
    }
    if (e != hipSuccess) {
        plgpu_column_release(out_perm);
        return hip_fail(e, "gb_route_kernel");
    }
    return PLGPU_OK;
}

static bool mk_packable(const plgpu_column* keys, int32_t nkeys) {
    for (int i = 0; i < nkeys; ++i) {
        const int32_t dt = keys[i].dtype;
        if ((!dtype_is_int(dt) && dt != PLGPU_BOOL) || dt == PLGPU_U64) return false;
    }
    return true;
}

static void mk_ranges_to_ord(const int64_t* ranges, int32_t nkeys, uint64_t* h) {
    for (int i = 0; i < nkeys; ++i) {
        h[3 * i] = (uint64_t)ranges[3 * i] ^ 0x8000000000000000ull;
        h[3 * i + 1] = (uint64_t)ranges[3 * i + 1] ^ 0x8000000000000000ull;
        h[3 * i + 2] = ranges[3 * i + 2] != 0;
    }
}

PLGPU_API int plgpu_key_ranges(const plgpu_column* keys, int32_t nkeys, int64_t* out_ranges, void* stream) {
    if (keys == nullptr || out_ranges == nullptr) return fail(PLGPU_ERR_INVALID, "NULL argument");
    if (nkeys < 1 || nkeys > kMaxKeys) return fail(PLGPU_ERR_INVALID, "number of key columns must be 1..8");
    if (!mk_packable(keys, nkeys)) return fail(PLGPU_ERR_SCHEMA, "packed keys must be integer or Boolean columns");
    MkKeys mk;
    std::memset(&mk, 0, sizeof mk);
    mk.n = nkeys;
    const int64_t n = keys[0].length;
    for (int i = 0; i < nkeys; ++i) {
        if (keys[i].length != n) return fail(PLGPU_ERR_SHAPE, "key columns must have equal lengths");
        mk.c[i] = to_dev(keys[i]);
    }
    hipStream_t s = as_stream(stream);
    DevBuf<unsigned long long> st;
    int rc = st.alloc(3 * kMaxKeys * 8, s);
    if (rc) return rc;
    unsigned long long h[3 * kMaxKeys];
    for (int i = 0; i < kMaxKeys; ++i) h[3 * i] = ~0ull, h[3 * i + 1] = 0, h[3 * i + 2] = 0;
    hipError_t e = hipMemcpyAsync(st, h, sizeof h, hipMemcpyHostToDevice, s);
    if (e == hipSuccess && n > 0) {
        const int g = (int)std::min<int64_t>((n + 255) / 256, (int64_t)num_cus() * 16);
        mk_range_kernel<<<g, 256, 0, s>>>(mk, n, st);
        e = hipGetLastError();
    }
    if (e == hipSuccess) e = hipMemcpyAsync(h, st, sizeof h, hipMemcpyDeviceToHost, s);
    if (e == hipSuccess) e = hipStreamSynchronize(s);
    if (e != hipSuccess) return hip_fail(e, "key range pass");
    for (int i = 0; i < nkeys; ++i) {
        out_ranges[3 * i] = (int64_t)(h[3 * i] ^ 0x8000000000000000ull);
        out_ranges[3 * i + 1] = (int64_t)(h[3 * i + 1] ^ 0x8000000000000000ull);
        out_ranges[3 * i + 2] = h[3 * i + 2] ? 1 : 0;
    }
    return PLGPU_OK;
}

PLGPU_API int plgpu_key_pack(const plgpu_column* keys, int32_t nkeys, const int64_t* ranges, plgpu_column* out_codes,
                             int32_t* out_ok, void* stream) {
    if (keys == nullptr || ranges == nullptr || out_codes == nullptr || out_ok == nullptr)
        return fail(PLGPU_ERR_INVALID, "NULL argument");
    if (nkeys < 1 || nkeys > kMaxKeys) return fail(PLGPU_ERR_INVALID, "number of key columns must be 1..8");
    if (!mk_packable(keys, nkeys)) return fail(PLGPU_ERR_SCHEMA, "packed keys must be integer or Boolean columns");
    std::memset(out_codes, 0, sizeof *out_codes);
    *out_ok = 0;
    MkKeys mk;
    std::memset(&mk, 0, sizeof mk);
    mk.n = nkeys;
    const int64_t n = keys[0].length;
    for (int i = 0; i < nkeys; ++i) {
        if (keys[i].length != n) return fail(PLGPU_ERR_SHAPE, "key columns must have equal lengths");
        mk.c[i] = to_dev(keys[i]);
    }
    uint64_t h[3 * kMaxKeys];
    mk_ranges_to_ord(ranges, nkeys, h);
    MkPack pk;
    std::memset(&pk, 0, sizeof pk);
    pk.n = nkeys;
    mk_plan_from_ranges(h, nkeys, &pk);
    if (!pk.ok) return PLGPU_OK;
    hipStream_t s = as_stream(stream);
    int rc = make_owned_column(out_codes, PLGPU_I64, n, false, s);
    if (rc) return rc;
    if (n > 0) {
        const int g = (int)std::min<int64_t>((n + 255) / 256, (int64_t)num_cus() * 16);
        mk_pack_launch(mk, pk, n, (uint64_t*)out_codes->values, nullptr, nullptr, g, s);
        hipError_t e = hipGetLastError();
        if (e == hipSuccess) e = hipStreamSynchronize(s);
        if (e != hipSuccess) {
            plgpu_column_release(out_codes);
            return hip_fail(e, "mk_pack_kernel");
        }
    }
    *out_ok = 1;
    return PLGPU_OK;
}

PLGPU_API int plgpu_key_unpack(const plgpu_column* codes, const int32_t* dtypes, int32_t nkeys, const int64_t* ranges,
                               plgpu_column* out_keys, void* stream) {
    if (codes == nullptr || dtypes == nullptr || ranges == nullptr || out_keys == nullptr)
        return fail(PLGPU_ERR_INVALID, "NULL argument");
    if (nkeys < 1 || nkeys > kMaxKeys) return fail(PLGPU_ERR_INVALID, "number of key columns must be 1..8");
    if (codes->dtype != PLGPU_I64) return fail(PLGPU_ERR_SCHEMA, "packed codes must be an Int64 column");
    for (int i = 0; i < nkeys; ++i) std::memset(&out_keys[i], 0, sizeof(plgpu_column));
    uint64_t h[3 * kMaxKeys];
    mk_ranges_to_ord(ranges, nkeys, h);
    MkPack pk;
    std::memset(&pk, 0, sizeof pk);
    pk.n = nkeys;
    mk_plan_from_ranges(h, nkeys, &pk);
    if (!pk.ok) return fail(PLGPU_ERR_INVALID, "these key ranges do not pack into 63 bits");
    hipStream_t s = as_stream(stream);
    const int64_t groups = codes->length;
    const int gg = (int)std::max<int64_t>(1, std::min<int64_t>((groups + 255) / 256, 4096));
    const int64_t* cv = (const int64_t*)codes->values + codes->offset;
    int rc = PLGPU_OK;
    for (int i = 0; i < nkeys && !rc; ++i) {
        const bool nullable = pk.nullable[i] != 0;
        rc = make_owned_column(&out_keys[i], dtypes[i], groups, nullable, s);
        if (rc || groups == 0) continue;
        if (dtypes[i] == PLGPU_BOOL) (void)hipMemsetAsync((void*)out_keys[i].values, 0, ((groups + 63) / 64) * 8, s);
        if (nullable) (void)hipMemsetAsync((void*)out_keys[i].validity, 0, ((groups + 63) / 64) * 8, s);
        mk_unpack_kernel<<<gg, 256, 0, s>>>(cv, nullptr, groups, pk, i, dtypes[i], (void*)out_keys[i].values,
                                            (uint32_t*)out_keys[i].validity);
        hipError_t e = hipGetLastError();
        if (e != hipSuccess) rc = hip_fail(e, "mk_unpack_kernel");
    }
    if (!rc) {
        hipError_t e = hipStreamSynchronize(s);
        if (e != hipSuccess) rc = hip_fail(e, "key unpack");
    }
    if (rc)
        for (int i = 0; i < nkeys; ++i) plgpu_column_release(&out_keys[i]);
    return rc;
}

__global__ __launch_bounds__(256) void float_code_kernel(DevCol c, int64_t n, int64_t* __restrict__ out,
                                                         uint64_t* __restrict__ valid_words) {
    for (int64_t r0 = (int64_t)blockIdx.x * blockDim.x; r0 < n; r0 += (int64_t)gridDim.x * blockDim.x) {
        const int64_t r = r0 + threadIdx.x;
        const bool in = r < n;
        const bool v = in && dev_valid(c, r);
        if (in) out[r] = v ? (int64_t)mk_word(c, r) : 0;
        const uint64_t b = __ballot(v);
        if (valid_words && (threadIdx.x & 63) == 0 && r < n) valid_words[r >> 6] = b;
    }
}

PLGPU_API int plgpu_float_key_encode(const plgpu_column* keys, plgpu_column* out_codes, void* stream) {
    if (keys == nullptr || out_codes == nullptr) return fail(PLGPU_ERR_INVALID, "NULL argument");
    std::memset(out_codes, 0, sizeof *out_codes);
    if (keys->dtype != PLGPU_F64 && keys->dtype != PLGPU_F32)
        return fail(PLGPU_ERR_SCHEMA, "float key codes of a non-float column");
    hipStream_t s = as_stream(stream);
    const int64_t n = keys->length;
    int rc = make_owned_column(out_codes, PLGPU_I64, n, keys->validity != nullptr, s);
    if (rc) return rc;
    if (n > 0) {
        const int g = (int)std::min<int64_t>((n + 255) / 256, (int64_t)num_cus() * 16);
        float_code_kernel<<<g, 256, 0, s>>>(to_dev(*keys), n, (int64_t*)out_codes->values,
                                            (uint64_t*)out_codes->validity);
        hipError_t e = hipGetLastError();
        if (e == hipSuccess) e = hipStreamSynchronize(s);
        if (e != hipSuccess) {
            plgpu_column_release(out_codes);
            return hip_fail(e, "float key codes");
        }
    }
    return PLGPU_OK;
}

static int gb_merge_impl(const void* records, int64_t n_records, int32_t nsrc, const int64_t* src_records,
                         const int32_t* src_bottoms, const plgpu_column* cols, int32_t ncols, const plgpu_agg* aggs,
                         int32_t naggs, const int32_t* bottoms, int32_t key_dtype, plgpu_column* out_key,
                         plgpu_column* out_aggs, plgpu_groupby_info* info, void* stream,
                         const int32_t* wide = nullptr, const int32_t* wide_exmin = nullptr,
                         const int32_t* wide_exmax = nullptr) {
    if (out_key == nullptr || (cols == nullptr && ncols > 0)) return fail(PLGPU_ERR_INVALID, "NULL argument");
    if (ncols < 0 || ncols > PLGPU_MAX_COLS) return fail(PLGPU_ERR_INVALID, "too many columns (max 8)");
    if (n_records < 0 || (n_records > 0 && records == nullptr)) return fail(PLGPU_ERR_INVALID, "bad records");
    int32_t tb[kMaxAcc];
    std::vector<int64_t> start;
    std::vector<int32_t> shift;
    if (nsrc > 0) {
        start.assign(nsrc + 1, 0);
        for (int j = 0; j < nsrc; ++j) {
            if (src_records[j] < 0) return fail(PLGPU_ERR_INVALID, "bad source record count");
            start[j + 1] = start[j] + src_records[j];
        }
        if (start[nsrc] != n_records) return fail(PLGPU_ERR_INVALID, "source record counts do not add up");
        for (int a = 0; a < kMaxAcc; ++a) {
            bool any = false;
            tb[a] = 0;
            for (int j = 0; j < nsrc; ++j) {
                if (src_records[j] == 0) continue;
                const int32_t b = src_bottoms[j * kMaxAcc + a];
                tb[a] = any ? std::min(tb[a], b) : b;
                any = true;
            }
            if (!any) tb[a] = src_bottoms[a];
        }
        shift.assign((size_t)nsrc * kMaxAcc, 0);
        for (int j = 0; j < nsrc; ++j)
            for (int a = 0; a < kMaxAcc; ++a)
                if (src_records[j] > 0) shift[j * kMaxAcc + a] = src_bottoms[j * kMaxAcc + a] - tb[a];
    } else {
        if (bottoms == nullptr) return fail(PLGPU_ERR_INVALID, "NULL argument");
        for (int a = 0; a < kMaxAcc; ++a) tb[a] = bottoms[a];
    }
    std::memset(out_key, 0, sizeof *out_key);
    for (int i = 0; i < naggs && out_aggs; ++i) std::memset(&out_aggs[i], 0, sizeof(plgpu_column));
    std::vector<plgpu_column> c2(cols, cols + ncols);
    for (auto& c : c2) c.length = 0;
    plgpu_column k;
    std::memset(&k, 0, sizeof k);
    k.dtype = dtype_is_int(key_dtype) ? key_dtype : PLGPU_I64;
    GbRun R;
    int rc = gb_prepare(R, &k, c2.data(), ncols, nullptr, 0, aggs, naggs, false, true, stream);
    if (rc) return rc;
    for (int a = 0; a < kMaxAcc; ++a) {
        R.hb[a] = tb[a];
        R.pl.p.bottom[a] = tb[a];
    }
    R.gbits = log2_ceil(std::max<int64_t>(1024, n_records * 2));
    GbParams& p = R.pl.p;
    if (wide) {
        for (int a = 0; a < kMaxAcc; ++a) {
            if (!wide[a]) continue;
            if (a >= p.nacc || !(p.acc[a].flags & (A_FSUM | A_FSUMCAST)))
                return fail(PLGPU_ERR_INVALID, "wide: only f64 sums take digit states");
            if (wide_exmin[a] < 1 || wide_exmax[a] > 0x7FE || wide_exmin[a] > wide_exmax[a])
                return fail(PLGPU_ERR_INVALID, "wide: bad exponent range");
            R.wide |= 1u << a;
            R.wide_exmin[a] = wide_exmin[a];
            R.wide_exmax[a] = wide_exmax[a];
        }
    }
    DevBuf<int64_t> dsrc;
    if (nsrc > 0) {
        const size_t bytes = (size_t)(nsrc + 1) * 8 + shift.size() * 4;
        if ((rc = dsrc.alloc(bytes, R.s))) return rc;
        std::vector<uint8_t> h(bytes);
        std::memcpy(h.data(), start.data(), (size_t)(nsrc + 1) * 8);
        std::memcpy(h.data() + (size_t)(nsrc + 1) * 8, shift.data(), shift.size() * 4);
        hipError_t e = hipMemcpyAsync(dsrc, h.data(), bytes, hipMemcpyHostToDevice, R.s);
        if (e == hipSuccess) e = hipStreamSynchronize(R.s);
        if (e != hipSuccess) return hip_fail(e, "merge sources");
    }
    for (R.attempts = 0;; ++R.attempts) {
        if ((rc = gb_alloc_table(R))) break;
        for (int a = 0; a < kMaxAcc && !rc; ++a) {
            if (!((R.wide >> a) & 1u)) continue;
            const size_t words = (size_t)(p.gcap + 2) * wide_nwords(R.wide_exmin[a], R.wide_exmax[a]);
            rc = R.wide_digits[a].alloc(words * 8, R.s);
            if (!rc && hipMemsetAsync(R.wide_digits[a], 0, words * 8, R.s) != hipSuccess)
                rc = fail(PLGPU_ERR_HIP, "wide digits");
        }
        if (rc) break;
        WideRec wr;
        const int rw = wide_layout(R, wr);
        hipError_t e = hipMemcpyAsync(R.bottoms, R.hb, sizeof R.hb, hipMemcpyHostToDevice, R.s);
        if (e == hipSuccess && n_records > 0) {
            const int g = (int)std::min<int64_t>((n_records + 255) / 256, 256 * 16);
            gb_merge_kernel<<<g, 256, 0, R.s>>>(p, (const uint64_t*)records, n_records, nsrc, dsrc,
                                                dsrc ? (const int32_t*)(dsrc + nsrc + 1) : nullptr, wr, rw);
            e = hipGetLastError();
        }
        if (e == hipSuccess) e = hipMemcpyAsync(R.st, R.status, sizeof R.st, hipMemcpyDeviceToHost, R.s);
        if (e == hipSuccess) e = hipStreamSynchronize(R.s);
        if (e != hipSuccess) {
            rc = hip_fail(e, "gb_merge_kernel");
            break;
        }
        if (R.st[ST_SHIFT_OVF]) {
            rc = fail(PLGPU_ERR_CAPACITY,
                      "multi-GPU group-by: the ranks' f64 sums span more binades than one 192-bit state holds");
            break;
        }
        if (R.st[ST_TABLE_FULL] == 0) break;
        if (R.attempts >= 3) {
            rc = fail(PLGPU_ERR_CAPACITY, "merge did not converge");
            break;
        }
        R.gbits += 3;
    }
    dsrc.reset();
    for (int a = 0; a < kMaxAcc && !rc; ++a) {
        if (!((R.wide >> a) & 1u)) continue;
        rc = R.wide_sum[a].alloc((size_t)(p.gcap + 2) * 8, R.s);
        if (rc) break;
        const int fg = (int)std::min<int64_t>((p.gcap + 2 + 255) / 256, 256 * 16);
        gb_wide_round_kernel<<<fg, 256, 0, R.s>>>(p, R.wide_exmin[a], wide_nwords(R.wide_exmin[a], R.wide_exmax[a]),
                                                  R.wide_digits[a], R.wide_sum[a]);
        if (hipGetLastError() != hipSuccess) rc = fail(PLGPU_ERR_HIP, "gb_wide_round_kernel");
    }
    if (rc) return rc;
    if (info) gb_fill_info(R, info);
    return gb_finalize(R, naggs, out_key, out_aggs);
}

PLGPU_API int plgpu_gb_merge(const void* records, int64_t n_records, const plgpu_column* cols, int32_t ncols,
                             const plgpu_agg* aggs, int32_t naggs, const int32_t* bottoms, int32_t key_dtype,
                             plgpu_column* out_key, plgpu_column* out_aggs, plgpu_groupby_info* info, void* stream) {
    return gb_merge_impl(records, n_records, 0, nullptr, nullptr, cols, ncols, aggs, naggs, bottoms, key_dtype,
                         out_key, out_aggs, info, stream);
}

PLGPU_API int plgpu_gb_merge_sources(const void* records, int32_t n_sources, const int64_t* src_records,
                                     const int32_t* src_bottoms, const plgpu_column* cols, int32_t ncols,
                                     const plgpu_agg* aggs, int32_t naggs, int32_t key_dtype, plgpu_column* out_key,
                                     plgpu_column* out_aggs, plgpu_groupby_info* info, void* stream) {
    if (n_sources < 1 || src_records == nullptr || src_bottoms == nullptr)
        return fail(PLGPU_ERR_INVALID, "merge: need >= 1 source with its record count and windows");
    int64_t n = 0;
    for (int j = 0; j < n_sources; ++j) n += src_records[j];
    return gb_merge_impl(records, n, n_sources, src_records, src_bottoms, cols, ncols, aggs, naggs, nullptr,
                         key_dtype, out_key, out_aggs, info, stream);
}

PLGPU_API int plgpu_gb_merge_sources_wide(const void* records, int32_t n_sources, const int64_t* src_records,
                                          const int32_t* src_bottoms, const int32_t* wide, const int32_t* wide_exmin,
                                          const int32_t* wide_exmax, const plgpu_column* cols, int32_t ncols,
                                          const plgpu_agg* aggs, int32_t naggs, int32_t key_dtype,
                                          plgpu_column* out_key, plgpu_column* out_aggs, plgpu_groupby_info* info,
                                          void* stream) {
    if (n_sources < 1 || src_records == nullptr || src_bottoms == nullptr)
        return fail(PLGPU_ERR_INVALID, "merge: need >= 1 source with its record count and windows");
    if (wide == nullptr || wide_exmin == nullptr || wide_exmax == nullptr)
        return fail(PLGPU_ERR_INVALID, "NULL argument");
    int64_t n = 0;
    for (int j = 0; j < n_sources; ++j) n += src_records[j];
    return gb_merge_impl(records, n, n_sources, src_records, src_bottoms, cols, ncols, aggs, naggs, nullptr,
                         key_dtype, out_key, out_aggs, info, stream, wide, wide_exmin, wide_exmax);
}

static void kp_span(KeyPack& k, int i) {
    const int bits = k.bits[i];
    if (bits >= 64) {
        k.span[i] = ~0ull;
        k.mode[i] = (k.c[i].dtype == PLGPU_I32 || k.c[i].dtype == PLGPU_U32) ? 2 : 0;
        k.span32[i] = 0xFFFFFFFFu;
        return;
    }
    const uint64_t mask = bits >= 64 ? ~0ull : (1ull << bits) - 1;
    const uint64_t ordb = k.base[i] ^ 0x8000000000000000ull;
    k.span[i] = std::min<uint64_t>(mask, ~0ull - ordb);
    const int32_t dt = k.c[i].dtype;
    const int64_t b = (int64_t)k.base[i];
    k.mode[i] = 0;
    if (dt == PLGPU_I32 || dt == PLGPU_U32) {
        const bool in_range = dt == PLGPU_I32 ? (b >= INT32_MIN && b <= INT32_MAX) : (b >= 0 && b <= (int64_t)UINT32_MAX);
        k.mode[i] = in_range ? 1 : 2;
        k.x32[i] = dt == PLGPU_I32 ? 0x80000000u : 0u;
        k.b32[i] = (uint32_t)b ^ k.x32[i];
        const uint32_t m32 = bits >= 32 ? 0xFFFFFFFFu : (1u << bits) - 1;
        k.span32[i] = std::min<uint32_t>(m32, 0xFFFFFFFFu - k.b32[i]);
    }
}

static KeyPack kp_from_plan(const MkKeys& mk, const MkPack& pk, int64_t n) {
    KeyPack k;
    std::memset(&k, 0, sizeof k);
    if (!options().fuse_keys || mk.n < 1 || mk.n > kKpFast || n < (int64_t(1) << 20)) return k;
    for (int i = 0; i < mk.n; ++i) {
        const DevCol& c = mk.c[i];
        const bool w8 = c.dtype == PLGPU_I64, w4 = c.dtype == PLGPU_I32 || c.dtype == PLGPU_U32;
        if (!(w8 || w4) || c.validity != nullptr || (c.offset & 1) != 0 ||
            ((uintptr_t)c.values & (w8 ? 15 : 7)) != 0)
            return k;
    }
    for (int i = 0; i < mk.n; ++i) {
        k.c[i] = mk.c[i];
        k.base[i] = (uint64_t)pk.minv[i] - (pk.nullable[i] ? 1u : 0u);
        k.shift[i] = pk.shift[i];
        k.bits[i] = pk.bits[i];
        kp_span(k, i);
    }
    k.n = mk.n;
    return k;
}

static int gb_multi_decode(const MkPack& pk, const plgpu_column* keys, int32_t nkeys, plgpu_column& hout,
                           plgpu_column* out_keys, plgpu_column* out_aggs, int32_t naggs, hipStream_t s) {
    int rc = PLGPU_OK;
    const int64_t groups = hout.length;
    const int gg = (int)std::max<int64_t>(1, std::min<int64_t>((groups + 255) / 256, 4096));
    for (int i = 0; i < nkeys && !rc; ++i) {
        const bool nullable = pk.nullable[i] != 0;
        rc = make_owned_column(&out_keys[i], keys[i].dtype, groups, nullable, s);
        if (rc || groups == 0) continue;
        if (keys[i].dtype == PLGPU_BOOL) (void)hipMemsetAsync((void*)out_keys[i].values, 0, ((groups + 63) / 64) * 8, s);
        if (nullable) (void)hipMemsetAsync((void*)out_keys[i].validity, 0, ((groups + 63) / 64) * 8, s);
        {
            KtScope kt("mk_unpack_kernel", s);
            mk_unpack_kernel<<<gg, 256, 0, s>>>((const int64_t*)hout.values, nullptr, groups, pk, i, keys[i].dtype,
                                                (void*)out_keys[i].values, (uint32_t*)out_keys[i].validity);
        }
        hipError_t e = hipGetLastError();
        if (e != hipSuccess) rc = hip_fail(e, "mk_unpack_kernel");
    }
    plgpu_column_release(&hout);
    if (rc) {
        for (int i = 0; i < nkeys; ++i) plgpu_column_release(&out_keys[i]);
        for (int i = 0; i < naggs; ++i) plgpu_column_release(&out_aggs[i]);
    }
    return rc;
}

static int gb_multi_packed(const MkKeys& mk, MkPack pk, int64_t n, const plgpu_column* keys, int32_t nkeys,
                           const plgpu_column* cols, int32_t ncols, const Deriv* deriv, const plgpu_instr* program,
                           int32_t n_instr, const plgpu_agg* aggs, int32_t naggs, int32_t maintain_order,
                           plgpu_column* out_keys, plgpu_column* out_aggs, plgpu_groupby_info* info, void* stream,
                           bool checked = false, bool* repack = nullptr) {
    hipStream_t s = as_stream(stream);
    if (repack) *repack = false;
    const KeyPack kp = kp_from_plan(mk, pk, n);
    if (options().debug)
        fprintf(stderr, "[plgpu] gb_multi_packed: n=%lld keys=%d fused key pack=%d checked=%d\n", (long long)n, mk.n,
                kp.n, (int)checked);
    if (kp.n > 0) {
        plgpu_column ck;
        std::memset(&ck, 0, sizeof ck);
        ck.dtype = PLGPU_I64;
        ck.length = n;
        ck.values = keys[0].values;
        plgpu_column hout;
        std::memset(&hout, 0, sizeof hout);
        GbRun R;
        int rc = gb_prepare(R, &ck, cols, ncols, program, n_instr, aggs, naggs, maintain_order != 0, false, stream,
                            deriv);
        if (!rc) {
            R.pl.p.kp = kp;
            rc = gb_plan(R, nullptr);
        }
        if (!rc && !R.kp_fallback) {
            rc = gb_main(R, true, nullptr, nullptr);
            if (!rc && R.kp_bad) {
                if (!checked) return fail(PLGPU_ERR_HIP, "fused key packing: a row outside the exact packing plan");
                *repack = true;
                return PLGPU_OK;
            }
            if (!rc && info) gb_fill_info(R, info);
            if (!rc) rc = gb_finalize(R, naggs, &hout, out_aggs);
            if (rc) return rc;
            return gb_multi_decode(pk, keys, nkeys, hout, out_keys, out_aggs, naggs, s);
        }
        if (rc) return rc;
    }
    DevBuf<uint64_t> codes;
    int rc = codes.alloc((size_t)std::max<int64_t>(n, 1) * 8 + (checked ? 8 : 0), s);
    if (rc) return rc;
    if (n > 0) {
        unsigned int* outside = checked ? (unsigned int*)(codes + std::max<int64_t>(n, 1)) : nullptr;
        hipError_t e = hipSuccess;
        if (outside) e = hipMemsetAsync(outside, 0, 4, s);
        const int g = (int)std::min<int64_t>((n + 255) / 256, (int64_t)num_cus() * 16);
        if (e == hipSuccess) {
            mk_pack_launch(mk, pk, n, codes, nullptr, outside, g, s);
            e = hipGetLastError();
        }
        unsigned int bad = 0;
        if (e == hipSuccess && outside) e = hipMemcpyAsync(&bad, outside, 4, hipMemcpyDeviceToHost, s);
        if (e == hipSuccess && outside) e = hipStreamSynchronize(s);
        if (e != hipSuccess) rc = hip_fail(e, "mk_pack_kernel");
        if (!rc && bad) {
            *repack = true;
            return PLGPU_OK;
        }
    }
    plgpu_column ck;
    std::memset(&ck, 0, sizeof ck);
    ck.dtype = PLGPU_I64;
    ck.length = n;
    ck.values = codes;
    plgpu_column hout;
    std::memset(&hout, 0, sizeof hout);
    {
        GbRun R;
        if (!rc)
            rc = gb_prepare(R, &ck, cols, ncols, program, n_instr, aggs, naggs, maintain_order != 0, false, stream,
                            deriv);
        if (!rc) rc = gb_plan(R, nullptr);
        if (!rc) rc = gb_main(R, true, nullptr, nullptr);
        if (!rc && info) gb_fill_info(R, info);
        if (!rc) rc = gb_finalize(R, naggs, &hout, out_aggs);
    }
    codes.reset();
    if (rc) return rc;
    return gb_multi_decode(pk, keys, nkeys, hout, out_keys, out_aggs, naggs, s);
}

static int gb_str_fused(const plgpu_column& key, const plgpu_column* cols, int32_t ncols, const Deriv* deriv,
                        const plgpu_instr* program, int32_t n_instr, const plgpu_agg* aggs, int32_t naggs,
                        int32_t maintain_order, plgpu_column* out_keys, plgpu_column* out_aggs,
                        plgpu_groupby_info* info, hipStream_t s, bool* done) {
    *done = false;
    const int64_t n = key.length;
    int64_t data_end = 0;
    PLGPU_HIP(hipMemcpyAsync(&data_end, (const int64_t*)key.values + key.offset + n, 8, hipMemcpyDeviceToHost, s));
    PLGPU_HIP(hipStreamSynchronize(s));
    KeyPack kp;
    std::memset(&kp, 0, sizeof kp);
    kp.n = 1;
    kp.c[0] = dev_col(key);
    kp.bits[0] = 64;
    kp.span[0] = ~0ull;
    kp.data_end = data_end;
    plgpu_column ck;
    std::memset(&ck, 0, sizeof ck);
    ck.dtype = PLGPU_I64;
    ck.length = n;
    ck.values = key.values;
    GbRun R;
    int rc = gb_prepare(R, &ck, cols, ncols, program, n_instr, aggs, naggs, maintain_order != 0, false, s, deriv);
    if (!rc) {
        R.pl.p.kp = kp;
        rc = gb_plan(R, nullptr);
    }
    if (rc || R.kp_fallback) return rc;
    rc = gb_main(R, true, nullptr, nullptr);
    if (rc || R.kp_bad) return rc;
    plgpu_column hout;
    std::memset(&hout, 0, sizeof hout);
    if (info) gb_fill_info(R, info);
    if ((rc = gb_finalize(R, naggs, &hout, out_aggs))) return rc;
    rc = str_from_codes(hout, &out_keys[0], s);
    plgpu_column_release(&hout);
    if (rc) {
        for (int i = 0; i < naggs; ++i) plgpu_column_release(&out_aggs[i]);
        return rc;
    }
    *done = true;
    return PLGPU_OK;
}

static int gb_multi_impl(const plgpu_column* keys, int32_t nkeys, const plgpu_column* cols, int32_t ncols,
                         const Deriv* deriv, const plgpu_instr* program, int32_t n_instr, const plgpu_agg* aggs,
                         int32_t naggs, int32_t maintain_order, plgpu_column* out_keys, plgpu_column* out_aggs,
                         plgpu_groupby_info* info, void* stream) {
    if (keys == nullptr || out_keys == nullptr) return fail(PLGPU_ERR_INVALID, "keys / out_keys is NULL");
    if (nkeys < 1 || nkeys > kMaxKeys) return fail(PLGPU_ERR_INVALID, "number of key columns must be 1..8");
    for (int i = 0; i < nkeys; ++i) std::memset(&out_keys[i], 0, sizeof(plgpu_column));
    for (int i = 0; i < naggs && out_aggs; ++i) std::memset(&out_aggs[i], 0, sizeof(plgpu_column));
    const int64_t n = keys[0].length;
    MkKeys mk;
    std::memset(&mk, 0, sizeof mk);
    mk.n = nkeys;
    for (int i = 0; i < nkeys; ++i) {
        const int32_t dt = keys[i].dtype;
        if (!dtype_is_int(dt) && !dtype_is_float(dt) && dt != PLGPU_BOOL && dt != PLGPU_STR)
            return fail(PLGPU_ERR_SCHEMA, "group-by keys must be integer, float, Boolean or String columns");
        if (keys[i].length != n) return fail(PLGPU_ERR_SHAPE, "key columns must have equal lengths");
        mk.c[i] = to_dev(keys[i]);
    }
    hipStream_t s = as_stream(stream);
    if (nkeys == 1 && keys[0].dtype == PLGPU_STR && keys[0].validity == nullptr && n >= (int64_t(1) << 20) &&
        options().fuse_keys) {
        bool done = false;
        const int rc = gb_str_fused(keys[0], cols, ncols, deriv, program, n_instr, aggs, naggs, maintain_order,
                                    out_keys, out_aggs, info, s, &done);
        if (rc || done) return rc;
    }
    {
        bool any_str = false, short_all = true;
        plgpu_column ck[kMaxKeys];
        std::memset(ck, 0, sizeof ck);
        int rc = PLGPU_OK;
        for (int i = 0; i < nkeys; ++i) {
            ck[i] = keys[i];
            if (keys[i].dtype != PLGPU_STR || !short_all || rc) continue;
            any_str = true;
            bool sh = false;
            rc = str_short_codes(keys[i], &ck[i], &sh, s);
            short_all = short_all && sh;
        }
        if (any_str && !rc && short_all) {
            if (nkeys == 1)
                rc = gb_single_impl(&ck[0], cols, ncols, deriv, program, n_instr, aggs, naggs, maintain_order,
                                    &out_keys[0], out_aggs, info, stream);
            else
                rc = gb_multi_impl(ck, nkeys, cols, ncols, deriv, program, n_instr, aggs, naggs, maintain_order,
                                   out_keys, out_aggs, info, stream);
            for (int i = 0; i < nkeys && !rc; ++i) {
                if (keys[i].dtype != PLGPU_STR) continue;
                plgpu_column strs;
                rc = str_from_codes(out_keys[i], &strs, s);
                plgpu_column_release(&out_keys[i]);
                if (!rc) out_keys[i] = strs;
            }
            if (rc) {
                for (int i = 0; i < nkeys; ++i) plgpu_column_release(&out_keys[i]);
                for (int i = 0; i < naggs && out_aggs; ++i) plgpu_column_release(&out_aggs[i]);
            }
        }
        for (int i = 0; i < nkeys; ++i)
            if (keys[i].dtype == PLGPU_STR && ck[i].dtype == PLGPU_I64) str_codes_free(&ck[i], s);
        if (rc || (any_str && short_all)) return rc;
    }
    if (nkeys == 1 && (keys[0].dtype == PLGPU_I32 || keys[0].dtype == PLGPU_U32) && keys[0].validity == nullptr &&
        n >= (int64_t(1) << 20) && options().fuse_keys) {
        MkPack pk;
        std::memset(&pk, 0, sizeof pk);
        pk.n = 1;
        pk.ok = 1;
        pk.bits[0] = 64;
        bool repack = false;
        const int rc = gb_multi_packed(mk, pk, n, keys, nkeys, cols, ncols, deriv, program, n_instr, aggs, naggs,
                                       maintain_order, out_keys, out_aggs, info, stream, true, &repack);
        if (rc || !repack) return rc;
    }
    const int hg = (int)std::min<int64_t>((n + 255) / 256, (int64_t)num_cus() * 16);
    {
        MkPack pk;
        int rc = PLGPU_OK;
        const bool reuse = options().plan_cache != 0 && n >= (int64_t(1) << 24);
        const std::string pkey = reuse ? pack_key(mk, n) : std::string();
        if (n >= (int64_t(1) << 20)) {
            if (!(reuse && pack_cache_get(pkey, &pk))) {
                if ((rc = mk_plan_pack_sampled(mk, n, &pk, s))) return rc;
                if (reuse && pk.ok) pack_cache_put(pkey, pk);
            }
            if (pk.ok) {
                bool repack = false;
                rc = gb_multi_packed(mk, pk, n, keys, nkeys, cols, ncols, deriv, program, n_instr, aggs, naggs,
                                     maintain_order, out_keys, out_aggs, info, stream, true, &repack);
                if (rc || !repack) return rc;
            }
        }
        rc = mk_plan_pack(mk, n, nullptr, 0, std::max(hg, 1), &pk, s);
        if (rc) return rc;
        if (reuse && pk.ok) pack_cache_put(pkey, pk);
        if (pk.ok) return gb_multi_packed(mk, pk, n, keys, nkeys, cols, ncols, deriv, program, n_instr, aggs, naggs,
                                          maintain_order, out_keys, out_aggs, info, stream);
    }
    DevBuf<uint64_t> hashes;
    DevBuf<uint32_t> collision;
    int rc = hashes.alloc((size_t)std::max<int64_t>(n, 1) * 8, s);
    if (!rc) rc = collision.alloc(4, s);
    plgpu_column hk;
    std::memset(&hk, 0, sizeof hk);
    hk.dtype = PLGPU_I64;
    hk.length = n;
    hk.values = hashes;
    bool done = false;
    for (int attempt = 0; attempt < 4 && !rc && !done; ++attempt) {
        const uint64_t seed = 0x243F6A8885A308D3ull * (uint64_t)(2 * attempt + 1);
        const uint64_t mask = attempt == 0 && options().mk_collide ? 7ull : ~0ull;
        if (n > 0) mk_hash_kernel<<<std::max(hg, 1), 256, 0, s>>>(mk, n, seed, mask, hashes);
        hipError_t e = hipGetLastError();
        if (e != hipSuccess) { rc = hip_fail(e, "mk_hash_kernel"); break; }
        GbRun R;
        R.want_first = true;
        rc = gb_prepare(R, &hk, cols, ncols, program, n_instr, aggs, naggs, maintain_order != 0, false, stream, deriv);
        if (!rc) rc = gb_plan(R, nullptr);
        if (!rc) rc = gb_main(R, true, nullptr, nullptr);
        if (rc) break;
        plgpu_column hout;
        DevBuf<uint64_t> first;
        if ((rc = gb_finalize(R, naggs, &hout, out_aggs, &first))) break;
        const int64_t groups = hout.length;
        plgpu_column_release(&hout);
        uint32_t coll = 0;
        if (n > 0 && groups > 0) {
            const int64_t total = R.pl.p.gcap + 2;
            DevBuf<uint64_t> vw;
            if ((rc = vw.alloc((size_t)total * (nkeys * 8 + 4), s))) break;
            uint32_t* vmask = (uint32_t*)(vw + (size_t)total * nkeys);
            (void)hipMemsetAsync(collision, 0, 4, s);
            mk_rep_kernel<<<(unsigned)std::min<int64_t>((total + 255) / 256, 4096), 256, 0, s>>>(R.pl.p, mk, vw,
                                                                                               vmask);
            mk_verify_kernel<<<std::max(hg, 1), 256, 0, s>>>(R.pl.p, mk, hashes, n, vw, vmask, collision);
            vw.reset();
            e = hipGetLastError();
            if (e == hipSuccess) e = hipMemcpyAsync(&coll, collision, 4, hipMemcpyDeviceToHost, s);
            if (e == hipSuccess) e = hipStreamSynchronize(s);
            if (e != hipSuccess) rc = hip_fail(e, "mk_verify_kernel");
        }
        if (!rc && !coll) {
            const int gg = (int)std::min<int64_t>((groups + 255) / 256, 4096);
            for (int i = 0; i < nkeys && !rc; ++i) {
                const bool nullable = keys[i].validity != nullptr;
                if (keys[i].dtype == PLGPU_STR) {
                    rc = str_gather(mk.c[i], nullptr, (const int64_t*)first.get(), nullptr, 0, groups, nullable,
                                    &out_keys[i], s);
                    continue;
                }
                rc = make_owned_column(&out_keys[i], keys[i].dtype, groups, nullable, s);
                if (rc || groups == 0) continue;
                if (keys[i].dtype == PLGPU_BOOL) (void)hipMemsetAsync((void*)out_keys[i].values, 0, ((groups + 63) / 64) * 8, s);
                if (nullable) (void)hipMemsetAsync((void*)out_keys[i].validity, 0, ((groups + 63) / 64) * 8, s);
                mk_gather_key_kernel<<<gg, 256, 0, s>>>(mk.c[i], first, groups, n, (void*)out_keys[i].values,
                                                        (uint32_t*)out_keys[i].validity);
                e = hipGetLastError();
                if (e != hipSuccess) rc = hip_fail(e, "mk_gather_key_kernel");
            }
            if (!rc) {
                e = hipStreamSynchronize(s);
                if (e != hipSuccess) rc = hip_fail(e, "multi-key gather");
            }
            if (!rc && info) {
                gb_fill_info(R, info);
                info->reruns += attempt;
            }
            done = !rc;
        }
        if (!done)
            for (int i = 0; i < naggs; ++i) plgpu_column_release(&out_aggs[i]);
    }
    if (!rc && !done) rc = fail(PLGPU_ERR_CAPACITY, "multi-key group-by: unresolved 64-bit hash collisions");
    if (rc)
        for (int i = 0; i < nkeys; ++i) plgpu_column_release(&out_keys[i]);
    return rc;
}

PLGPU_API int plgpu_group_by_agg_multi(const plgpu_column* keys, int32_t nkeys, const plgpu_column* cols,
                                       int32_t ncols, const plgpu_instr* program, int32_t n_instr,
                                       const plgpu_agg* aggs, int32_t naggs, int32_t maintain_order,
                                       plgpu_column* out_keys, plgpu_column* out_aggs, plgpu_groupby_info* info,
                                       void* stream) {
    return gb_multi_impl(keys, nkeys, cols, ncols, nullptr, program, n_instr, aggs, naggs, maintain_order, out_keys,
                         out_aggs, info, stream);
}

static int gb_keyless(const plgpu_column* cols, int32_t ncols, const Deriv* deriv, const plgpu_instr* program,
                      int32_t n_instr, const plgpu_agg* aggs, int32_t naggs, plgpu_column* out_aggs,
                      plgpu_groupby_info* info, void* stream) {
    if (ncols < 1) return fail(PLGPU_ERR_INVALID, "a global reduction needs at least one column (the length)");
    plgpu_column k;
    std::memset(&k, 0, sizeof k);
    k.dtype = PLGPU_I64;
    k.length = cols[0].length;
    k.device_id = cols[0].device_id;
    plgpu_column out_key;
    int rc = gb_single_impl(&k, cols, ncols, deriv, program, n_instr, aggs, naggs, 0, &out_key, out_aggs, info,
                            stream);
    if (rc) return rc;
    const int64_t groups = out_key.length;
    plgpu_column_release(&out_key);
    if (groups == 1) return PLGPU_OK;
    if (groups != 0) return fail(PLGPU_ERR_CAPACITY, "internal: a global reduction produced several groups");
    hipStream_t s = as_stream(stream);
    for (int i = 0; i < naggs && rc == PLGPU_OK; ++i) {
        const int32_t dt = out_aggs[i].dtype;
        const bool has_valid = out_aggs[i].validity != nullptr;
        plgpu_column_release(&out_aggs[i]);
        rc = make_owned_column(&out_aggs[i], dt, 1, has_valid, s);
        if (rc) break;
        const int32_t kind = aggs[i].kind & 0xFF;
        const bool valid = kind == PLGPU_AGG_SUM || kind == PLGPU_AGG_LEN || kind == PLGPU_AGG_COUNT;
        const size_t vb = dt == PLGPU_BOOL ? 8 : (size_t)std::max(dtype_bytes(dt), 1);
        hipError_t e = hipMemsetAsync((void*)out_aggs[i].values, 0, vb, s);
        if (e == hipSuccess && has_valid) e = hipMemsetAsync((void*)out_aggs[i].validity, valid ? 0x01 : 0x00, 1, s);
        if (e == hipSuccess && has_valid) e = hipMemsetAsync((uint8_t*)out_aggs[i].validity + 1, 0, 7, s);
        if (e != hipSuccess) rc = hip_fail(e, "empty reduction");
        out_aggs[i].null_count = (has_valid && !valid) ? 1 : 0;
    }
    if (rc == PLGPU_OK) {
        hipError_t e = hipStreamSynchronize(s);
        if (e != hipSuccess) rc = hip_fail(e, "empty reduction");
    }
    if (rc)
        for (int i = 0; i < naggs; ++i) plgpu_column_release(&out_aggs[i]);
    return rc;
}

PLGPU_API int plgpu_group_by_agg_ex(const plgpu_column* keys, int32_t nkeys, const plgpu_column* cols, int32_t ncols,
                                    const plgpu_agg_input* inputs, int32_t ninputs, const plgpu_instr* program,
                                    int32_t n_instr, const plgpu_agg* aggs, int32_t naggs, int32_t maintain_order,
                                    plgpu_column* out_keys, plgpu_column* out_aggs, plgpu_groupby_info* info,
                                    void* stream) {
    if (nkeys < 0 || nkeys > kMaxKeys) return fail(PLGPU_ERR_INVALID, "number of key columns must be 0..8");
    if (nkeys > 0 && (keys == nullptr || out_keys == nullptr)) return fail(PLGPU_ERR_INVALID, "keys / out_keys is NULL");
    if (ninputs < 0 || (ninputs > 0 && inputs == nullptr)) return fail(PLGPU_ERR_INVALID, "bad aggregation inputs");
    if (ncols < 0 || ncols > PLGPU_MAX_COLS) return fail(PLGPU_ERR_INVALID, "too many columns (max 8)");
    if (naggs > 0 && out_aggs == nullptr) return fail(PLGPU_ERR_INVALID, "out_aggs is NULL");
    for (int i = 0; i < naggs; ++i) std::memset(&out_aggs[i], 0, sizeof(plgpu_column));
    for (int i = 0; i < nkeys; ++i) std::memset(&out_keys[i], 0, sizeof(plgpu_column));
    Deriv d;
    int rc = classify_inputs(cols, ncols, inputs, ninputs, &d);
    if (rc) return rc;
    std::vector<plgpu_agg> ag(aggs, aggs + std::max(naggs, 0));
    int hi_of[PLGPU_MAX_COLS];
    for (int c = 0; c < PLGPU_MAX_COLS; ++c) hi_of[c] = -1;
    bool any_var = false;
    for (int i = 0; i < naggs; ++i) {
        const int base = aggs[i].kind & 0xFF;
        if (base != PLGPU_AGG_VAR && base != PLGPU_AGG_STD) continue;
        const int c = aggs[i].col;
        if (c < 0 || c >= ncols || cols[c].dtype != PLGPU_F64)
            return fail(PLGPU_ERR_INVALID, "var / std in one pass take a Float64 column");
        if (hi_of[c] < 0) {
            hi_of[c] = ncols + (int)d.in.size();
            for (int q = 0; q < 2; ++q) {
                DerivIn di;
                std::memset(&di, 0, sizeof di);
                di.kind = 3;
                di.ca = c;
                di.cb = -1;
                di.dop = (q == 0 ? DOP_SQHI : DOP_SQLO) | DOP_LIT;
                di.out_dtype = PLGPU_F64;
                d.in.push_back(di);
            }
        }
        ag[i].kind = (aggs[i].kind & 0xFFFF) | (hi_of[c] << 16);
        any_var = true;
    }
    const Deriv* dv = (ninputs > 0 || any_var) ? &d : nullptr;
    const plgpu_agg* ap = naggs > 0 ? ag.data() : aggs;
    if (nkeys == 0) return gb_keyless(cols, ncols, dv, program, n_instr, ap, naggs, out_aggs, info, stream);
    const bool narrow = nkeys == 1 && (keys[0].dtype == PLGPU_I32 || keys[0].dtype == PLGPU_U32) &&
                        keys[0].validity == nullptr && keys[0].length >= (int64_t(1) << 20) && options().fuse_keys;
    if (nkeys == 1 && dtype_is_int(keys[0].dtype) && !narrow)
        return gb_single_impl(&keys[0], cols, ncols, dv, program, n_instr, ap, naggs, maintain_order, &out_keys[0],
                              out_aggs, info, stream);
    return gb_multi_impl(keys, nkeys, cols, ncols, dv, program, n_instr, ap, naggs, maintain_order, out_keys,
                         out_aggs, info, stream);
}

__global__ __launch_bounds__(256) void var_finalize_kernel(DevCol ss, DevCol cnt, int64_t n, int32_t ddof,
                                                           int32_t take_sqrt, double* __restrict__ out,
                                                           uint64_t* __restrict__ out_valid) {
    for (int64_t i0 = (int64_t)blockIdx.x * blockDim.x; i0 < n; i0 += (int64_t)gridDim.x * blockDim.x) {
        const int64_t i = i0 + threadIdx.x;
        bool valid = false;
        if (i < n) {
            const uint64_t c = dev_valid(cnt, i) ? dev_load(cnt, i) : 0;
            double v = 0.0;
            if (c > (uint64_t)ddof && dev_valid(ss, i)) {
                v = as_f64(dev_load(ss, i)) / (double)(c - (uint64_t)ddof);
                if (v < 0.0) v = 0.0;
                if (take_sqrt) v = __builtin_sqrt(v);
                valid = true;
            }
            out[i] = v;
        }
        const uint64_t w = __ballot(valid);
        if ((threadIdx.x & 63) == 0 && i < n) out_valid[i >> 6] = w;
    }
}

PLGPU_API int plgpu_var_finalize(const plgpu_column* sum_sq, const plgpu_column* count, int32_t ddof,
                                 int32_t take_sqrt, plgpu_column* out, void* stream) {
    hipStream_t s = as_stream(stream);
    if (sum_sq == nullptr || count == nullptr || out == nullptr) return fail(PLGPU_ERR_INVALID, "NULL argument");
    std::memset(out, 0, sizeof *out);
    if (sum_sq->dtype != PLGPU_F64 || (count->dtype != PLGPU_U32 && count->dtype != PLGPU_I64))
        return fail(PLGPU_ERR_SCHEMA, "var finalize takes Float64 sums and UInt32 / Int64 counts");
    if (sum_sq->length != count->length) return fail(PLGPU_ERR_SHAPE, "columns differ in length");
    if (ddof < 0 || ddof > 255) return fail(PLGPU_ERR_INVALID, "ddof must be 0..255");
    const int64_t n = sum_sq->length;
    int rc = make_owned_column(out, PLGPU_F64, n, true, s);
    if (rc || n == 0) return rc;
    const unsigned g = (unsigned)std::min<int64_t>((n + 255) / 256, 4096);
    var_finalize_kernel<<<g, 256, 0, s>>>(to_dev(*sum_sq), to_dev(*count), n, ddof, take_sqrt,
                                          (double*)out->values, (uint64_t*)out->validity);
    hipError_t e = hipGetLastError();
    if (e == hipSuccess) e = hipStreamSynchronize(s);
    if (e != hipSuccess) {
        plgpu_column_release(out);
        return hip_fail(e, "var finalize");
    }
    return PLGPU_OK;
}

constexpr uint32_t kSqEmpty = 0xFFFFFFFFu;

constexpr uint32_t kSqNoMean = 0x80000000u;
constexpr int kSqLdsBits = 11;

__global__ __launch_bounds__(256) void sq_build_kernel(DevCol gk, DevCol mean, int64_t ng, int bits,
                                                       uint64_t* __restrict__ tkey, uint64_t* __restrict__ tval,
                                                       uint32_t* __restrict__ tidx, uint32_t* __restrict__ null_g) {
    const int64_t g = (int64_t)blockIdx.x * blockDim.x + threadIdx.x;
    if (g >= ng) return;
    const uint32_t tag = (uint32_t)g | (dev_valid(mean, g) ? 0u : kSqNoMean);
    if (!dev_valid(gk, g)) {
        null_g[0] = tag;
        null_g[1] = (uint32_t)dev_load(mean, g);
        null_g[2] = (uint32_t)(dev_load(mean, g) >> 32);
        return;
    }
    const uint64_t k = dev_load(gk, g);
    const uint32_t mask = (1u << bits) - 1;
    for (uint32_t h = hash_slot(k, bits);; h = (h + 1) & mask) {
        if (atomicCAS(&tidx[h], kSqEmpty, tag) == kSqEmpty) {
            tkey[h] = k;
            tval[h] = dev_load(mean, g);
            return;
        }
    }
}

__device__ __forceinline__ double sq_as_f64(const DevCol& c, int64_t r) {
    const uint64_t b = dev_load(c, r);
    switch (c.dtype) {
    case PLGPU_F64:
    case PLGPU_F32: return as_f64(b);
    case PLGPU_U64: return (double)b;
    default: return (double)(int64_t)b;
    }
}

template <bool LDS>
__global__ __launch_bounds__(256) void sq_dev_kernel(DevCol rk, DevCol x, int64_t n, int bits,
                                                     const uint64_t* __restrict__ gkey,
                                                     const uint64_t* __restrict__ gval,
                                                     const uint32_t* __restrict__ gidx,
                                                     const uint32_t* __restrict__ null_g,
                                                     double* __restrict__ out, uint64_t* __restrict__ out_valid) {
    extern __shared__ uint64_t sq_lds[];
    const uint32_t slots = 1u << bits, mask = slots - 1;
    const uint64_t* tkey = gkey;
    const uint64_t* tval = gval;
    const uint32_t* tidx = gidx;
    if (LDS) {
        uint64_t* k = sq_lds;
        uint64_t* v = sq_lds + slots;
        uint32_t* t = (uint32_t*)(sq_lds + 2 * slots);
        for (uint32_t h = threadIdx.x; h < slots; h += blockDim.x) {
            k[h] = gkey[h];
            v[h] = gval[h];
            t[h] = gidx[h];
        }
        __syncthreads();
        tkey = k;
        tval = v;
        tidx = t;
    }
    const uint32_t null_tag = null_g[0];
    const uint64_t null_mean = (uint64_t)null_g[1] | ((uint64_t)null_g[2] << 32);
    constexpr int R = 4;
    for (int64_t base = (int64_t)blockIdx.x * 256 * R; base < n; base += (int64_t)gridDim.x * 256 * R) {
        uint64_t kk[R];
        double xv[R];
        bool kv[R], xok[R];
#pragma unroll
        for (int j = 0; j < R; ++j) {
            const int64_t i = base + j * 256 + threadIdx.x;
            xok[j] = i < n && dev_valid(x, i);
            kv[j] = i < n && dev_valid(rk, i);
            kk[j] = i < n ? dev_load(rk, i) : 0;
            xv[j] = i < n ? sq_as_f64(x, i) : 0.0;
        }
#pragma unroll
        for (int j = 0; j < R; ++j) {
            const int64_t i = base + j * 256 + threadIdx.x;
            uint32_t tag = kSqEmpty;
            uint64_t m = 0;
            if (xok[j]) {
                if (!kv[j]) {
                    tag = null_tag;
                    m = null_mean;
                } else {
                    for (uint32_t h = hash_slot(kk[j], bits);; h = (h + 1) & mask) {
                        const uint32_t t = tidx[h];
                        if (t == kSqEmpty) break;
                        if (tkey[h] == kk[j]) {
                            tag = t;
                            m = tval[h];
                            break;
                        }
                    }
                }
            }
            const bool valid = xok[j] && tag != kSqEmpty && !(tag & kSqNoMean);
            const double d = xv[j] - as_f64(m);
            if (i < n) out[i] = valid ? d * d : 0.0;
            const uint64_t w = __ballot(valid);
            if ((threadIdx.x & 63) == 0 && i < n) out_valid[i >> 6] = w;
        }
    }
}

PLGPU_API int plgpu_group_sq_dev(const plgpu_column* row_key, const plgpu_column* x, const plgpu_column* group_key,
                                 const plgpu_column* group_mean, plgpu_column* out, void* stream) {
    hipStream_t s = as_stream(stream);
    if (!row_key || !x || !group_key || !group_mean || !out) return fail(PLGPU_ERR_INVALID, "NULL argument");
    std::memset(out, 0, sizeof *out);
    const int32_t kt = row_key->dtype;
    if (kt != group_key->dtype || (!dtype_is_int(kt) && kt != PLGPU_BOOL))
        return fail(PLGPU_ERR_SCHEMA, "squared deviations take one integer / Boolean key of one dtype");
    if (x->dtype == PLGPU_STR || group_mean->dtype != PLGPU_F64)
        return fail(PLGPU_ERR_SCHEMA, "squared deviations take a numeric x and Float64 means");
    if (row_key->length != x->length || group_key->length != group_mean->length)
        return fail(PLGPU_ERR_SHAPE, "columns differ in length");
    const int64_t n = x->length, ng = group_key->length;
    if (ng >= (int64_t)1 << 30) return fail(PLGPU_ERR_SHAPE, "too many groups");
    int rc = make_owned_column(out, PLGPU_F64, n, true, s);
    if (rc || n == 0) return rc;
    int bits = 6;
    while (((int64_t)1 << bits) < 2 * ng) ++bits;
    const size_t slots = (size_t)1 << bits;
    DevBuf<uint64_t> tkey;
    DevBuf<uint32_t> tidx;
    if ((rc = tkey.alloc(slots * 16, s)) || (rc = tidx.alloc(slots * 4 + 12, s))) {
        plgpu_column_release(out);
        return rc;
    }
    hipError_t e = hipMemsetAsync(tidx, 0xFF, slots * 4 + 12, s);
    uint64_t* tval = tkey + slots;
    uint32_t* null_g = tidx + slots;
    if (e == hipSuccess && ng > 0)
        sq_build_kernel<<<(unsigned)((ng + 255) / 256), 256, 0, s>>>(dev_col(*group_key), dev_col(*group_mean), ng,
                                                                     bits, tkey, tval, tidx, null_g);
    if (e == hipSuccess) e = hipGetLastError();
    if (e == hipSuccess) {
        const int64_t steps = (n + 1023) / 1024;
        if (bits <= kSqLdsBits) {
            const unsigned g = (unsigned)std::min<int64_t>(steps, (int64_t)num_cus() * 8);
            sq_dev_kernel<true><<<g, 256, slots * 20, s>>>(dev_col(*row_key), dev_col(*x), n, bits, tkey, tval, tidx,
                                                            null_g, (double*)out->values, (uint64_t*)out->validity);
        } else {
            const unsigned g = (unsigned)std::min<int64_t>(steps, (int64_t)1 << 30);
            sq_dev_kernel<false><<<g, 256, 0, s>>>(dev_col(*row_key), dev_col(*x), n, bits, tkey, tval, tidx, null_g,
                                                   (double*)out->values, (uint64_t*)out->validity);
        }
        e = hipGetLastError();
    }
    if (e == hipSuccess) e = hipStreamSynchronize(s);
    if (e != hipSuccess) {
        plgpu_column_release(out);
        return hip_fail(e, "squared deviations");
    }
    return PLGPU_OK;
}
```

### polaroid_amd/csrc/plgpu_internal.hpp

```cpp
#pragma once

#include <hip/hip_runtime.h>
#include <stdint.h>

#include <cstring>

#include <string>
#include <vector>

#include "../../include/polaroid_gpu.h"

#define PLGPU_API extern "C" __attribute__((visibility("default")))

namespace plgpu {

void set_error(const std::string& msg);
int fail(int code, const std::string& msg);
int hip_fail(hipError_t e, const char* what);

#define PLGPU_HIP(expr)                                   \
    do {                                                  \
        hipError_t _e = (expr);                           \
        if (_e != hipSuccess) return plgpu::hip_fail(_e, #expr); \
    } while (0)

hipStream_t as_stream(void* s);

struct Options {
    int debug = 0;
    int no_pack = 0;
    int mk_collide = 0;
    int runs = -1;
    int local = -1;
    int ktime = 0;
    int fuse_keys = 1;
    int plan_cache = 1;
    int grid_rounds = 0;
    int gb_path = -1;
    int part_bits = -1;
    int part_levels = -1;
    int part_direct = 1;
    int part_lds_kb = 0;
    int part_compact = 1;
    int rl_stream = 0;
    int rl_grid = 0;
    int filt_pipe = 1;
    int part_threads = 0;
    int rl_div = 1;
    int rl_full = 1;
    int rl_mean_hot = 1;
    int rl_var_hot = 1;
    int rl_var128 = 1;
    int alloc_skew = 0;
    int alloc_contig = 0;
    int srt_w4 = 0;
    int srt_up_tiles = 1;
    int part_rows4 = 0;
    int wave_report = 0;
    int part_null_sentinel = 1;
    int filt_fused = 0;
    int var_pos = 1;
    int sum_pos = 1;
    int gb_pair = 1;
    int join_radix = 1;
    int join_radix_keys = 0;
    int join_radix_load = 0;
    int join_radix_batch = 0;
    int over_presorted = 1;
    int asof_path = 0;
};
Options& options();

void gb_plan_cache_clear();
hipEvent_t ev_acquire();
void ev_release(hipEvent_t e);
bool kt_begin(hipStream_t s, hipEvent_t* a, hipEvent_t* b);
void kt_end(const char* name, hipEvent_t a, hipEvent_t b, hipStream_t s);
struct KtScope {
    const char* name;
    hipEvent_t a = nullptr, b = nullptr;
    hipStream_t s;
    KtScope(const char* nm, hipStream_t st) : name(nm), s(st) {
        if (options().ktime && !kt_begin(st, &a, &b)) a = b = nullptr;
    }
    ~KtScope() {
        if (a) kt_end(name, a, b, s);
    }
    KtScope(const KtScope&) = delete;
    KtScope& operator=(const KtScope&) = delete;
};
int dev_alloc(void** p, size_t bytes, hipStream_t s);
void dev_free(void* p, hipStream_t s);

template <typename T>
class DevBuf {
    T* p_ = nullptr;
    hipStream_t s_ = nullptr;

public:
    DevBuf() = default;
    DevBuf(DevBuf&& o) noexcept : p_(o.p_), s_(o.s_) { o.p_ = nullptr; }
    DevBuf& operator=(DevBuf&& o) noexcept {
        if (this != &o) {
            reset();
            p_ = o.p_;
            s_ = o.s_;
            o.p_ = nullptr;
        }
        return *this;
    }
    DevBuf(const DevBuf&) = delete;
    DevBuf& operator=(const DevBuf&) = delete;
    ~DevBuf() { reset(); }

    int alloc(size_t bytes, hipStream_t s) {
        reset();
        s_ = s;
        void* v = nullptr;
        const int rc = dev_alloc(&v, bytes, s);
        p_ = (T*)v;
        return rc;
    }
    void reset() {
        if (p_) dev_free(p_, s_);
        p_ = nullptr;
    }
    T* release() {
        T* r = p_;
        p_ = nullptr;
        return r;
    }
    T* get() const { return p_; }
    operator T*() const { return p_; }
};

inline int num_cus() {
    static int g_num_cus = 0;
    if (g_num_cus == 0) {
        int dev = 0;
        hipDeviceProp_t prop;
        if (hipGetDevice(&dev) == hipSuccess && hipGetDeviceProperties(&prop, dev) == hipSuccess)
            g_num_cus = prop.multiProcessorCount;
        else
            g_num_cus = 256;
    }
    return g_num_cus;
}

inline int log2_ceil(int64_t x) {
    int b = 0;
    while ((int64_t(1) << b) < x) ++b;
    return b;
}

// ... 620 lines not shown
```

### polaroid_amd/csrc/runtime.cpp

```cpp
#include <hip/hip_runtime.h>

#include <cstdio>
#include <cstdlib>
#include <algorithm>
#include <cmath>
#include <cstdint>
#include <cstring>
#include <map>
#include <mutex>
#include <string>
#include <unordered_map>
#include <vector>

#include "plgpu_internal.hpp"

namespace plgpu {

static thread_local std::string g_last_error;

void set_error(const std::string& msg) { g_last_error = msg; }

int fail(int code, const std::string& msg) {
    g_last_error = msg;
    return code;
}

int hip_fail(hipError_t e, const char* what) {
    g_last_error = std::string("HIP error: ") + hipGetErrorString(e) + " at " + what;
    (void)hipGetLastError();
    return e == hipErrorOutOfMemory ? PLGPU_ERR_OOM : PLGPU_ERR_HIP;
}

hipStream_t as_stream(void* s) { return reinterpret_cast<hipStream_t>(s); }

namespace {
struct OptField {
    const char* name;
    const char* env;
    int Options::*f;
};
const OptField kOptFields[] = {
    {"debug", "PLGPU_DEBUG", &Options::debug},
    {"no_pack", "PLGPU_NO_PACK", &Options::no_pack},
    {"mk_collide", "PLGPU_MK_COLLIDE", &Options::mk_collide},
    {"runs", "PLGPU_RUNS", &Options::runs},
    {"local", "PLGPU_LOCAL", &Options::local},
    {"ktime", "PLGPU_KTIME", &Options::ktime},
    {"fuse_keys", "PLGPU_FUSE_KEYS", &Options::fuse_keys},
    {"grid_rounds", "PLGPU_GRID_ROUNDS", &Options::grid_rounds},
    {"plan_cache", "PLGPU_PLAN_CACHE", &Options::plan_cache},
    {"gb_path", "PLGPU_GB_PATH", &Options::gb_path},
    {"part_bits", "PLGPU_PART_BITS", &Options::part_bits},
    {"part_levels", "PLGPU_PART_LEVELS", &Options::part_levels},
    {"part_direct", "PLGPU_PART_DIRECT", &Options::part_direct},
    {"part_compact", "PLGPU_PART_COMPACT", &Options::part_compact},
    {"rl_var128", "PLGPU_RL_VAR128", &Options::rl_var128},
    {"rl_var_hot", "PLGPU_RL_VAR_HOT", &Options::rl_var_hot},
    {"rl_mean_hot", "PLGPU_RL_MEAN_HOT", &Options::rl_mean_hot},
    {"over_presorted", "PLGPU_OVER_PRESORTED", &Options::over_presorted},
    {"alloc_skew", "PLGPU_ALLOC_SKEW", &Options::alloc_skew},
    {"alloc_contig", "PLGPU_ALLOC_CONTIG", &Options::alloc_contig},
    {"srt_w4", "PLGPU_SRT_W4", &Options::srt_w4},
    {"srt_up_tiles", "PLGPU_SRT_UP_TILES", &Options::srt_up_tiles},
    {"part_rows4", "PLGPU_PART_ROWS4", &Options::part_rows4},
    {"wave_report", "PLGPU_WAVE_REPORT", &Options::wave_report},
    {"part_null_sentinel", "PLGPU_PART_NULL_SENTINEL", &Options::part_null_sentinel},
    {"part_lds_kb", "PLGPU_PART_LDS_KB", &Options::part_lds_kb},
    {"rl_stream", "PLGPU_RL_STREAM", &Options::rl_stream},
    {"rl_grid", "PLGPU_RL_GRID", &Options::rl_grid},
    {"filt_pipe", "PLGPU_FILT_PIPE", &Options::filt_pipe},
    {"rl_div", "PLGPU_RL_DIV", &Options::rl_div},
    {"part_threads", "PLGPU_PART_THREADS", &Options::part_threads},
    {"gb_pair", "PLGPU_GB_PAIR", &Options::gb_pair},
    {"rl_full", "PLGPU_RL_FULL", &Options::rl_full},
    {"filt_fused", "PLGPU_FILT_FUSED", &Options::filt_fused},
    {"var_pos", "PLGPU_VAR_POS", &Options::var_pos},
    {"sum_pos", "PLGPU_SUM_POS", &Options::sum_pos},
    {"join_radix", "PLGPU_JOIN_RADIX", &Options::join_radix},
    {"join_radix_keys", "PLGPU_JOIN_RADIX_KEYS", &Options::join_radix_keys},
    {"join_radix_load", "PLGPU_JOIN_RADIX_LOAD", &Options::join_radix_load},
    {"join_radix_batch", "PLGPU_JOIN_RADIX_BATCH", &Options::join_radix_batch},
    {"asof_path", "PLGPU_ASOF_PATH", &Options::asof_path},
};
const OptField* opt_field(const char* name) {
    for (const OptField& f : kOptFields)
        if (!strcmp(name, f.name)) return &f;
    return nullptr;
}
}

static Options read_env_options() {
    Options o;
    for (const OptField& f : kOptFields) {
        const char* e = getenv(f.env);
        if (e) o.*(f.f) = atoi(e);
    }
    return o;
}

Options& options() {
    static Options o = read_env_options();
    return o;
}

namespace {
struct KtPending {
    const char* name;
    hipEvent_t a, b;
};
struct KtSum {
    std::string name;
    double ms = 0.0;
    int64_t count = 0;
};
std::mutex g_kt_mu;
std::vector<KtPending> g_kt_pending;
std::vector<hipEvent_t> g_kt_pool;
std::vector<KtSum> g_kt_sums;

hipEvent_t kt_event() {
    if (!g_kt_pool.empty()) {
        hipEvent_t e = g_kt_pool.back();
        g_kt_pool.pop_back();
        return e;
    }
    hipEvent_t e = nullptr;
    if (hipEventCreate(&e) != hipSuccess) return nullptr;
    return e;
}
}

hipEvent_t ev_acquire() {
    std::lock_guard<std::mutex> g(g_kt_mu);
    return kt_event();
}

void ev_release(hipEvent_t e) {
    if (e == nullptr) return;
    std::lock_guard<std::mutex> g(g_kt_mu);
    g_kt_pool.push_back(e);
}

bool kt_begin(hipStream_t s, hipEvent_t* a, hipEvent_t* b) {
    std::lock_guard<std::mutex> g(g_kt_mu);
    *a = kt_event();
    *b = kt_event();
    if (*a == nullptr || *b == nullptr || hipEventRecord(*a, s) != hipSuccess) {
        if (*a) g_kt_pool.push_back(*a);
        if (*b) g_kt_pool.push_back(*b);
        *a = *b = nullptr;
        return false;
    }
    return true;
}

void kt_end(const char* name, hipEvent_t a, hipEvent_t b, hipStream_t s) {
    std::lock_guard<std::mutex> g(g_kt_mu);
    (void)hipEventRecord(b, s);
    g_kt_pending.push_back({name, a, b});
}

namespace {
struct Pool {
    std::mutex mu;
    std::multimap<size_t, void*> free_blocks;
    std::unordered_map<void*, size_t> sizes;
    std::unordered_map<void*, void*> skewed;
    uint32_t skew_ctr = 0;
    size_t cached = 0;
};
Pool& pool_for(int dev) {
    static Pool pools[64];
    return pools[(dev >= 0 && dev < 64) ? dev : 0];
}
size_t round_bytes(size_t b) {
    if (b <= (size_t(1) << 20)) return (b + 255) & ~size_t(255);
    return (b + (size_t(2) << 20) - 1) & ~((size_t(2) << 20) - 1);
}
void release_cached(Pool& P) {
    for (auto& kv : P.free_blocks) {
        (void)hipFree(kv.second);
        P.sizes.erase(kv.second);
    }
    P.free_blocks.clear();
    P.cached = 0;
}
// ... 596 lines not shown
}

PLGPU_API int plgpu_memcpy_d2h(void* dst, const void* src, size_t bytes, void* stream) {
    PLGPU_HIP(hipMemcpyAsync(dst, src, bytes, hipMemcpyDeviceToHost, as_stream(stream)));
    PLGPU_HIP(hipStreamSynchronize(as_stream(stream)));
    return PLGPU_OK;
}

namespace {
constexpr size_t kD2hStageMax = size_t(64) << 20;
std::mutex g_stage_mu;
void* g_stage = nullptr;
size_t g_stage_bytes = 0;
}

PLGPU_API int plgpu_memcpy_d2h_many(int32_t n, void* const* dst, const void* const* src, const size_t* bytes,
                                    void* stream) {
    if (n < 0 || (n > 0 && (dst == nullptr || src == nullptr || bytes == nullptr)))
        return fail(PLGPU_ERR_INVALID, "memcpy_d2h_many: bad arguments");
    hipStream_t s = as_stream(stream);
    size_t total = 0;
    for (int32_t i = 0; i < n; ++i)
        if (bytes[i] <= kD2hStageMax) total += (bytes[i] + 255) & ~size_t(255);
    std::lock_guard<std::mutex> lk(g_stage_mu);
    if (total > kD2hStageMax) total = 0;
    if (total > g_stage_bytes) {
        if (g_stage) (void)hipHostFree(g_stage);
        g_stage = nullptr;
        g_stage_bytes = 0;
        const size_t want = std::max<size_t>(total, size_t(1) << 20);
        if (hipHostMalloc(&g_stage, want, hipHostMallocDefault) != hipSuccess) {
            (void)hipGetLastError();
            g_stage = nullptr;
            total = 0;
        } else {
            g_stage_bytes = want;
        }
    }
    size_t off = 0;
    for (int32_t i = 0; i < n; ++i) {
        if (bytes[i] == 0) continue;
        if (total > 0 && bytes[i] <= kD2hStageMax) {
            PLGPU_HIP(hipMemcpyAsync((char*)g_stage + off, src[i], bytes[i], hipMemcpyDeviceToHost, s));
            off += (bytes[i] + 255) & ~size_t(255);
        } else {
            PLGPU_HIP(hipMemcpyAsync(dst[i], src[i], bytes[i], hipMemcpyDeviceToHost, s));
        }
    }
    PLGPU_HIP(hipStreamSynchronize(s));
    off = 0;
    for (int32_t i = 0; i < n; ++i) {
        if (bytes[i] == 0 || !(total > 0 && bytes[i] <= kD2hStageMax)) continue;
        std::memcpy(dst[i], (const char*)g_stage + off, bytes[i]);
        off += (bytes[i] + 255) & ~size_t(255);
    }
    return PLGPU_OK;
}

PLGPU_API int plgpu_memcpy_d2d(void* dst, const void* src, size_t bytes, void* stream) {
    PLGPU_HIP(hipMemcpyAsync(dst, src, bytes, hipMemcpyDeviceToDevice, as_stream(stream)));
    return PLGPU_OK;
}

PLGPU_API int plgpu_expr_dtype(const plgpu_column* cols, int32_t ncols, const plgpu_instr* program, int32_t n_instr,
                               int32_t* out_dtype) {
    if (out_dtype == nullptr || (ncols > 0 && cols == nullptr)) return fail(PLGPU_ERR_INVALID, "NULL argument");
    DevProgram dp;
    const int rc = lower_program(cols, ncols, program, n_instr, &dp);
    if (rc) return rc;
    *out_dtype = dp.out_dtype;
    return PLGPU_OK;
}

PLGPU_API int plgpu_set_option(const char* name, int64_t value) {
    if (name == nullptr) return fail(PLGPU_ERR_INVALID, "option name is NULL");
    const OptField* f = opt_field(name);
    if (f == nullptr) return fail(PLGPU_ERR_INVALID, std::string("unknown option ") + name);
    options().*(f->f) = (int)value;
    return PLGPU_OK;
}

PLGPU_API int plgpu_get_option(const char* name, int64_t* out) {
    if (name == nullptr || out == nullptr) return fail(PLGPU_ERR_INVALID, "NULL argument");
    const OptField* f = opt_field(name);
    if (f == nullptr) return fail(PLGPU_ERR_INVALID, std::string("unknown option ") + name);
    *out = options().*(f->f);
    return PLGPU_OK;
}

PLGPU_API int plgpu_release_cached(void) {
    int dev = 0;
    PLGPU_HIP(hipGetDevice(&dev));
    PLGPU_HIP(hipDeviceSynchronize());
    Pool& P = pool_for(dev);
    {
        std::lock_guard<std::mutex> lk(P.mu);
        release_cached(P);
    }
    gb_plan_cache_clear();
    return PLGPU_OK;
}

PLGPU_API int plgpu_ktime_read(char* buf, int64_t cap, int32_t reset) {
    if (buf == nullptr || cap <= 0) return fail(PLGPU_ERR_INVALID, "NULL argument");
    std::lock_guard<std::mutex> g(g_kt_mu);
    for (KtPending& p : g_kt_pending) {
        float ms = 0.f;
        const hipError_t e = hipEventSynchronize(p.b);
        if (e == hipSuccess && hipEventElapsedTime(&ms, p.a, p.b) == hipSuccess) {
            auto it = std::find_if(g_kt_sums.begin(), g_kt_sums.end(), [&](const KtSum& k) { return k.name == p.name; });
            if (it == g_kt_sums.end()) it = g_kt_sums.insert(g_kt_sums.end(), KtSum{p.name, 0.0, 0});
            it->ms += ms;
            it->count += 1;
        }
        g_kt_pool.push_back(p.a);
        g_kt_pool.push_back(p.b);
    }
    g_kt_pending.clear();
    std::string out;
    char line[256];
    for (const KtSum& k : g_kt_sums) {
        snprintf(line, sizeof line, "%s\t%.6f\t%lld\n", k.name.c_str(), k.ms, (long long)k.count);
        out += line;
    }
    if (reset) g_kt_sums.clear();
    if ((int64_t)out.size() + 1 > cap) return fail(PLGPU_ERR_CAPACITY, "ktime buffer too small");
    std::memcpy(buf, out.c_str(), out.size() + 1);
    return PLGPU_OK;
}

PLGPU_API void plgpu_column_release(plgpu_column* col) {
    if (col && col->release) col->release(col);
}
```

Before: 146,000 Mrows/s.

## Speculatively enqueue groupby finalize before status readback to cut host syncs

Fuses the table init, status clearing and bottoms upload into one prologue kernel. When the table is small, it speculatively launches the finalize and validity-pack kernels into max-capacity output columns before the status D2H wait. The finalize kernel skips itself on device if a repeat is needed, and gb_finalize reuses the speculative outputs without another stream synchronize. This removes a host round trip and several small launches per groupby, at the cost of over-allocating outputs and added complexity. A wait counter and a tunable plan-cache threshold are also added.

```diff
diff --git a/polaroid_amd/csrc/groupby.hip b/polaroid_amd/csrc/groupby.hip
--- a/polaroid_amd/csrc/groupby.hip
+++ b/polaroid_amd/csrc/groupby.hip
@@ -16,7 +16,13 @@
 namespace plgpu {
 
 static int d2h_stage(int n, void* const* dst, const void* const* src, const size_t* bytes, hipStream_t s) {
+    gb_wait_note();
     return plgpu_memcpy_d2h_many(n, dst, src, bytes, (void*)s);
+}
+
+static hipError_t gb_sync(hipStream_t s) {
+    gb_wait_note();
+    return hipStreamSynchronize(s);
 }
 
 
@@ -688,6 +694,25 @@
     }
 }
 
+struct GbBottoms {
+    int32_t v[kMaxAcc];
+};
+__global__ void gb_prologue_kernel(uint64_t* gtab, int64_t words_per_field, int nfields, uint64_t min_init_mask,
+                                   uint64_t* status, int32_t* bottoms, GbBottoms b) {
+    if (blockIdx.x == 0) {
+        for (int i = threadIdx.x; i < ST_WORDS; i += blockDim.x)
+            if (i < ST_DISTINCT || i >= ST_MAXEX) status[i] = 0;
+        if (threadIdx.x < kMaxAcc) bottoms[threadIdx.x] = b.v[threadIdx.x];
+    }
+    for (int f = 0; f < nfields; ++f) {
+        const uint64_t v = f == 0 ? kEmptyKey : (((min_init_mask >> f) & 1ull) ? ~0ull : 0ull);
+        uint64_t* q = gtab + (int64_t)f * words_per_field;
+        for (int64_t i = (int64_t)blockIdx.x * blockDim.x + threadIdx.x; i < words_per_field;
+             i += (int64_t)gridDim.x * blockDim.x)
+            q[i] = v;
+    }
+}
+
 
 constexpr int kVarWords = 16;
 
@@ -798,7 +823,8 @@
 struct FinParams {
     OutSpec out[PLGPU_MAX_COLS * 2];
     int32_t nout;
-    int32_t _pad;
+    int32_t spec;
+    uint64_t fx_mask;
     int64_t* out_keys;
     uint32_t* out_key_valid;
     uint64_t* out_first;
@@ -908,7 +934,12 @@
     }
 }
 
+__host__ __device__ inline bool gb_run_repeats(const uint64_t* st, uint64_t fx_mask) {
+    return st[ST_KPACK] != 0 || st[ST_TABLE_FULL] > 0 || (st[ST_FXFLAGS] & fx_mask) != 0;
+}
+
 __global__ __launch_bounds__(256) void gb_finalize_kernel(GbParams p, FinParams fp) {
+    if (fp.spec && gb_run_repeats(p.status, fp.fx_mask)) return;
     const int64_t total = p.gcap + 2;
     const int lane = threadIdx.x & 63, wid = threadIdx.x >> 6;
     const uint64_t lt = lane == 0 ? 0ull : (~0ull >> (64 - lane));
@@ -963,16 +994,18 @@
 struct PackValid {
     uint32_t* dst[PLGPU_MAX_COLS * 2 + 1];
     int32_t n;
+    const uint64_t* count;
 };
 __global__ void gb_pack_valid_kernel(const uint8_t* __restrict__ vb, int64_t cap, PackValid pv) {
-    const int64_t words = ((cap + 63) / 64) * 2;
+    const int64_t rows = pv.count ? std::min<int64_t>(cap, (int64_t)*pv.count) : cap;
+    const int64_t words = ((rows + 63) / 64) * 2;
     for (int64_t i = (int64_t)blockIdx.x * blockDim.x + threadIdx.x; i < words * pv.n;
          i += (int64_t)gridDim.x * blockDim.x) {
         const int c = (int)(i / words);
         const int64_t w = i - (int64_t)c * words;
         if (pv.dst[c] == nullptr) continue;
         const uint8_t* b = vb + (int64_t)c * cap + w * 32;
-        const int m = (int)std::max<int64_t>(0, std::min<int64_t>(32, cap - w * 32));
+        const int m = (int)std::max<int64_t>(0, std::min<int64_t>(32, rows - w * 32));
         uint32_t bits = 0;
         for (int j = 0; j < m; ++j) bits |= (uint32_t)(b[j] != 0) << j;
         pv.dst[c][w] = bits;
@@ -1574,14 +1607,28 @@
     std::vector<InSpec> ins;
     std::vector<plgpu_column> mat;
     std::vector<int> acc_input;
+    int32_t spec_naggs = -1;
+    bool spec_done = false;
+    plgpu_column spec_key;
+    plgpu_column spec_aggs[PLGPU_MAX_COLS * 2];
+    DevBuf<uint64_t> spec_first;
 
     GbRun() {
         std::memset(st, 0, sizeof st);
         std::memset(hb, 0, sizeof hb);
         std::memset(&pout, 0, sizeof pout);
+        std::memset(&spec_key, 0, sizeof spec_key);
+        std::memset(spec_aggs, 0, sizeof spec_aggs);
     }
     ~GbRun() {
         for (auto& c : mat) plgpu_column_release(&c);
+        spec_drop();
+    }
+    void spec_drop() {
+        plgpu_column_release(&spec_key);
+        for (auto& c : spec_aggs) plgpu_column_release(&c);
+        spec_first.reset();
+        spec_done = false;
     }
 };
 
@@ -1861,7 +1908,7 @@
         e = hipGetLastError();
     }
     if (e == hipSuccess) e = hipMemcpyAsync(h.data(), regs, h.size() * 4, hipMemcpyDeviceToHost, R.s);
-    if (e == hipSuccess) e = hipStreamSynchronize(R.s);
+    if (e == hipSuccess) e = gb_sync(R.s);
     if (e != hipSuccess) return hip_fail(e, "gb_hll_kernel");
     *out = (int64_t)hll_estimate(h.data());
     return PLGPU_OK;
@@ -1872,7 +1919,8 @@
     GbParams& p = pl.p;
     const int64_t n = p.n;
     const bool ps = R.pred == 1;
-    const bool use_cache = fixed == nullptr && options().plan_cache != 0 && n >= (int64_t(1) << 24);
+    const int64_t cache_rows = options().plan_cache_rows >= 0 ? options().plan_cache_rows : int64_t(1) << 24;
+    const bool use_cache = fixed == nullptr && options().plan_cache != 0 && n >= cache_rows;
     const std::string ckey = use_cache ? plan_key(R) : std::string();
     PlanStats cached;
     const bool hit = use_cache && plan_cache_get(ckey, &cached);
@@ -2191,7 +2239,7 @@
         if (e == hipSuccess) e = hipMemcpyAsync(hr1.data(), range1, (size_t)(P1 + 1) * 8, hipMemcpyDeviceToHost, s);
         if (e == hipSuccess && g1.keyrange)
             e = hipMemcpyAsync(krange.data(), g1.keyrange, krange.size() * 8, hipMemcpyDeviceToHost, s);
-        if (e == hipSuccess) e = hipStreamSynchronize(s);
+        if (e == hipSuccess) e = gb_sync(s);
         if (e != hipSuccess) rc = hip_fail(e, "gbp_count_kernel");
     }
     R.has_null_key = false;
@@ -2262,7 +2310,7 @@
                 e = hipGetLastError();
             }
             if (e == hipSuccess) e = hipMemcpyAsync(hr.data(), range, (size_t)(P + 1) * 8, hipMemcpyDeviceToHost, s);
-            if (e == hipSuccess) e = hipStreamSynchronize(s);
+            if (e == hipSuccess) e = gb_sync(s);
             if (e != hipSuccess) rc = hip_fail(e, "gbp_count_kernel (level 2)");
         }
         if (!rc) rc = gbp_alloc(R, (int64_t)hr[P], nul_out, &R.pbuf, &R.pout);
@@ -2373,7 +2421,7 @@
     return hipGetLastError();
 }
 
-static int gb_alloc_table(GbRun& R) {
+static int gb_alloc_table(GbRun& R, const int32_t* bottoms = nullptr) {
     GbParams& p = R.pl.p;
     R.gtab.reset();
     R.rtab.reset();
@@ -2397,6 +2445,14 @@
     if (rc) return rc;
     p.gtab = R.gtab;
     const int ig = (int)std::min<int64_t>((int64_t)(wpf + 255) / 256, 256 * 8);
+    if (bottoms) {
+        GbBottoms b;
+        for (int a = 0; a < kMaxAcc; ++a) b.v[a] = bottoms[a];
+        gb_prologue_kernel<<<ig, 256, 0, R.s>>>(R.gtab, (int64_t)wpf, p.nfields, p.min_init_mask, R.status,
+                                                R.bottoms, b);
+        PLGPU_HIP(hipGetLastError());
+        return PLGPU_OK;
+    }
     gb_init_table_kernel<<<ig, 256, 0, R.s>>>(R.gtab, (int64_t)wpf, p.nfields, p.min_init_mask);
     PLGPU_HIP(hipMemsetAsync(R.status, 0, 6 * 8, R.s));
     PLGPU_HIP(hipMemsetAsync(R.status + ST_MAXEX, 0, (ST_WORDS - ST_MAXEX) * 8, R.s));
@@ -2471,6 +2527,87 @@
     return w;
 }
 
+static bool out_nullable(const OutSpec& o) {
+    return o.kind == PLGPU_AGG_MEAN || o.kind == PLGPU_AGG_MIN || o.kind == PLGPU_AGG_MAX ||
+           o.kind == PLGPU_AGG_FIRST || o.kind == PLGPU_AGG_LAST || o.kind == PLGPU_AGG_VAR ||
+           o.kind == PLGPU_AGG_STD;
+}
+
+constexpr int64_t kBurstSlots = int64_t(1) << 16;
+
+static uint64_t gb_fx_mask(const GbRun& R) {
+    const GbParams& p = R.pl.p;
+    uint64_t m = 0;
+    for (int a = 0; a < p.nacc; ++a)
+        if ((p.acc[a].flags & (A_FSUM | A_FSUMCAST)) && !((R.wide >> a) & 1u)) m |= 3ull << (2 * a);
+    return m;
+}
+
+static bool gb_spec_applies(const GbRun& R) {
+    const Plan& pl = R.pl;
+    if (R.spec_naggs < 0 || options().gb_burst == 0 || R.part || R.wide != 0) return false;
+    if (pl.p.gcap + 2 > kBurstSlots + 2) return false;
+    for (int i = 0; i < R.spec_naggs; ++i) {
+        const OutSpec& o = pl.outs[i];
+        if ((o.kind == PLGPU_AGG_VAR || o.kind == PLGPU_AGG_STD) && R.hb[o.acc] < -484) return false;
+    }
+    return true;
+}
+
+static int gb_spec_launch(GbRun& R) {
+    Plan& pl = R.pl;
+    GbParams& p = pl.p;
+    hipStream_t s = R.s;
+    const int32_t naggs = R.spec_naggs;
+    const int64_t cap = p.gcap + 2;
+    R.spec_drop();
+    FinParams fp;
+    std::memset(&fp, 0, sizeof fp);
+    int rc = make_owned_column(&R.spec_key, PLGPU_I64, cap, true, s);
+    for (int i = 0; i < naggs && rc == PLGPU_OK; ++i)
+        rc = make_owned_column(&R.spec_aggs[i], pl.outs[i].out_dtype, cap, out_nullable(pl.outs[i]), s);
+    if (rc == PLGPU_OK && (R.maintain || R.want_first)) rc = R.spec_first.alloc(cap * 8, s);
+    DevBuf<uint8_t> vbytes;
+    if (rc == PLGPU_OK) rc = vbytes.alloc((size_t)(1 + naggs) * cap, s);
+    if (rc) {
+        R.spec_drop();
+        return rc;
+    }
+    fp.nout = naggs;
+    fp.spec = 1;
+    fp.fx_mask = gb_fx_mask(R);
+    for (int i = 0; i < naggs; ++i) {
+        fp.out[i] = pl.outs[i];
+        fp.out[i].values = (void*)R.spec_aggs[i].values;
+        fp.out[i].validity = (uint32_t*)R.spec_aggs[i].validity;
+    }
+    fp.out_keys = (int64_t*)R.spec_key.values;
+    fp.out_key_valid = (uint32_t*)R.spec_key.validity;
+    fp.out_first = R.spec_first;
+    fp.cap = cap;
+    fp.vbytes = vbytes;
+    {
+        KtScope kt("gb_finalize_kernel", s);
+        const int fg = (int)std::min<int64_t>((cap + 255) / 256, 256 * 16);
+        gb_finalize_kernel<<<fg, 256, 0, s>>>(p, fp);
+        PackValid pv;
+        std::memset(&pv, 0, sizeof pv);
+        pv.n = 1 + naggs;
+        pv.count = R.status + ST_GROUPS_OUT;
+        pv.dst[0] = (uint32_t*)R.spec_key.validity;
+        for (int i = 0; i < naggs; ++i) pv.dst[1 + i] = (uint32_t*)R.spec_aggs[i].validity;
+        const int64_t work = ((cap + 63) / 64) * 2 * pv.n;
+        gb_pack_valid_kernel<<<(unsigned)std::min<int64_t>((work + 255) / 256, 4096), 256, 0, s>>>(vbytes, cap, pv);
+    }
+    hipError_t e = hipGetLastError();
+    if (e != hipSuccess) {
+        R.spec_drop();
+        return hip_fail(e, "gb_finalize_kernel");
+    }
+    R.spec_done = true;
+    return PLGPU_OK;
+}
+
 static int gb_main(GbRun& R, bool auto_refit, bool* refit, int32_t* hint) {
     Plan& pl = R.pl;
     GbParams& p = pl.p;
@@ -2491,8 +2628,10 @@
         if (R.compact_now && R.region_cnt == nullptr &&
             (rc = R.region_cnt.alloc(((size_t)1 << R.pbits) * 4, R.s)))
             break;
-        if ((rc = gb_alloc_table(R))) break;
-        PLGPU_HIP(hipMemcpyAsync(R.bottoms, R.hb, sizeof R.hb, hipMemcpyHostToDevice, R.s));
+        const bool burst = !R.part && options().gb_burst != 0;
+        R.spec_drop();
+        if ((rc = gb_alloc_table(R, burst ? R.hb : nullptr))) break;
+        if (!burst) PLGPU_HIP(hipMemcpyAsync(R.bottoms, R.hb, sizeof R.hb, hipMemcpyHostToDevice, R.s));
         for (int a = 0; a < kMaxAcc; ++a) p.bottom[a] = R.hb[a];
         PLGPU_HIP(hipEventRecord(ev0, R.s));
         if (n > 0 && R.part) {
@@ -2506,7 +2645,9 @@
             }
         }
         PLGPU_HIP(hipEventRecord(ev1, R.s));
+        if (burst && gb_spec_applies(R) && (rc = gb_spec_launch(R))) break;
         if (int rs = d2h_status(R)) return rs;
+        if (R.spec_done && gb_run_repeats(R.st, gb_fx_mask(R))) R.spec_drop();
         if (debug) {
             fprintf(stderr,
                     "[plgpu] gb attempt %d: n=%lld grid=%d/%d lds=%d lcap=%d gcap=%lld nfields=%d lds_bytes=%zu "
@@ -2581,6 +2722,7 @@
             break;
         }
     }
+    if (rc != PLGPU_OK || R.kp_bad || R.wide) R.spec_drop();
     if (rc == PLGPU_OK) (void)hipEventElapsedTime(&R.ms, ev0, ev1);
     ev_release(ev0);
     ev_release(ev1);
@@ -2590,6 +2732,11 @@
         plan_cache_erase(R.plan_ckey);
     if (rc == PLGPU_OK && R.wide && !R.kp_bad) rc = gb_wide(R, R.wide_round);
     return rc;
+}
+
+static int gb_main_then_finalize(GbRun& R, int32_t naggs) {
+    R.spec_naggs = naggs;
+    return gb_main(R, true, nullptr, nullptr);
 }
 
 static int64_t gb_groups(const GbRun& R) {
@@ -2627,12 +2774,39 @@
     const int64_t groups = gb_groups(R);
     FinParams fp;
     std::memset(&fp, 0, sizeof fp);
-    int rc = make_owned_column(out_key, PLGPU_I64, groups, true, s);
-    for (int i = 0; i < naggs && rc == PLGPU_OK; ++i) {
+    const bool spec = R.spec_done && R.spec_naggs == naggs;
+    DevBuf<uint64_t> first;
+    int rc = PLGPU_OK;
+    if (spec) {
+        *out_key = R.spec_key;
+        std::memset(&R.spec_key, 0, sizeof R.spec_key);
+        out_key->length = groups;
+        for (int i = 0; i < naggs; ++i) {
+            out_aggs[i] = R.spec_aggs[i];
+            std::memset(&R.spec_aggs[i], 0, sizeof R.spec_aggs[i]);
+            out_aggs[i].length = groups;
+        }
+        first = std::move(R.spec_first);
+        R.spec_done = false;
+        if (R.st[ST_VAR_OUT]) rc = fail(PLGPU_ERR_CAPACITY, "var: the fused second moment is out of its exact range");
+        if (rc == PLGPU_OK && (int64_t)R.st[ST_GROUPS_OUT] != groups) {
+            char buf[256];
+            snprintf(buf, sizeof buf,
+                     "internal: group count mismatch (inserted %llu + specials %llu, finalized %llu, "
+                     "global rows %llu, table_full %llu)",
+                     (unsigned long long)R.st[ST_NEWKEYS], (unsigned long long)R.st[ST_SPECIAL],
+                     (unsigned long long)R.st[ST_GROUPS_OUT], (unsigned long long)R.st[ST_GLOBAL_ROWS],
+                     (unsigned long long)R.st[ST_TABLE_FULL]);
+            rc = fail(PLGPU_ERR_CAPACITY, buf);
+        }
+    } else {
+        R.spec_drop();
+        rc = make_owned_column(out_key, PLGPU_I64, groups, true, s);
+    }
+    bool enqueued = !spec;
+    for (int i = 0; i < naggs && rc == PLGPU_OK && !spec; ++i) {
         const OutSpec& o = pl.outs[i];
-        const bool nullable = o.kind == PLGPU_AGG_MEAN || o.kind == PLGPU_AGG_MIN || o.kind == PLGPU_AGG_MAX ||
-                              o.kind == PLGPU_AGG_FIRST || o.kind == PLGPU_AGG_LAST || o.kind == PLGPU_AGG_VAR ||
-                              o.kind == PLGPU_AGG_STD;
+        const bool nullable = out_nullable(o);
         if (o.kind == PLGPU_AGG_VAR || o.kind == PLGPU_AGG_STD) {
             const bool wide = ((R.wide >> o.acc) | (R.wide >> o.acc_hi) | (R.wide >> o.acc_lo)) & 1u;
             if (wide || R.hb[o.acc] < -484)
@@ -2640,9 +2814,8 @@
         }
         if (rc == PLGPU_OK) rc = make_owned_column(&out_aggs[i], o.out_dtype, groups, nullable, s);
     }
-    DevBuf<uint64_t> first;
-    if (rc == PLGPU_OK && (R.maintain || keep_first) && groups > 0) rc = first.alloc(groups * 8, s);
-    if (rc == PLGPU_OK && groups > 0) {
+    if (rc == PLGPU_OK && !spec && (R.maintain || keep_first) && groups > 0) rc = first.alloc(groups * 8, s);
+    if (rc == PLGPU_OK && !spec && groups > 0) {
         fp.nout = naggs;
         for (int i = 0; i < naggs; ++i) {
             fp.out[i] = pl.outs[i];
@@ -2715,6 +2888,7 @@
     }
     if (rc == PLGPU_OK && R.maintain && groups > 1) {
         plgpu_column fc, pidx;
+        enqueued = true;
         std::memset(&fc, 0, sizeof fc);
         std::memset(&pidx, 0, sizeof pidx);
         fc.dtype = PLGPU_I64;
@@ -2780,6 +2954,7 @@
         plgpu_column nk;
         rc = make_owned_column(&nk, R.key_dtype, groups, true, s);
         if (rc == PLGPU_OK && groups > 0) {
+            enqueued = true;
             const int gg = (int)std::min<int64_t>((groups + 255) / 256, 4096);
             narrow_i64_kernel<<<gg, 256, 0, s>>>((const int64_t*)out_key->values, (void*)nk.values, R.key_dtype,
                                                  groups);
@@ -2793,7 +2968,7 @@
     }
     if (rc == PLGPU_OK) {
         out_key->null_count = (R.st[ST_SPECIAL] & 1) ? 1 : 0;
-        hipError_t e = hipStreamSynchronize(s);
+        hipError_t e = enqueued ? gb_sync(s) : hipSuccess;
         if (e != hipSuccess) rc = hip_fail(e, "finalize sync");
     }
     if (rc == PLGPU_OK && keep_first) *keep_first = std::move(first);
@@ -2894,7 +3069,7 @@
                         deriv);
     R.compact_ok = maintain_order == 0;
     if (!rc) rc = gb_plan(R, nullptr);
-    if (!rc) rc = gb_main(R, true, nullptr, nullptr);
+    if (!rc) rc = gb_main_then_finalize(R, naggs);
     if (rc) return rc;
     if (info) gb_fill_info(R, info);
     return gb_finalize(R, naggs, out_key, out_aggs);
@@ -3040,7 +3215,7 @@
         }
     int rc = gb_wide(R, false);
     if (rc == PLGPU_OK) {
-        hipError_t e = hipStreamSynchronize(R.s);
+        hipError_t e = gb_sync(R.s);
         if (e != hipSuccess) rc = hip_fail(e, "gb_wide_kernel");
     }
     return rc;
@@ -3071,7 +3246,7 @@
     gb_export_count_kernel<<<fg, 256, 0, s>>>(p, W, counts);
     std::vector<uint64_t> hc(W), cur(W);
     PLGPU_HIP(hipMemcpyAsync(hc.data(), counts, (size_t)W * 8, hipMemcpyDeviceToHost, s));
-    PLGPU_HIP(hipStreamSynchronize(s));
+    PLGPU_HIP(gb_sync(s));
     uint64_t run = 0;
     for (int w = 0; w < W; ++w) {
         cur[w] = run;
@@ -3084,7 +3259,7 @@
         gb_export_kernel<<<fg, 256, 0, s>>>(p, W, counts + W, (uint64_t*)dst_records, wr, rw);
         PLGPU_HIP(hipGetLastError());
     }
-    PLGPU_HIP(hipStreamSynchronize(s));
+    PLGPU_HIP(gb_sync(s));
     return PLGPU_OK;
 }
 
@@ -3131,7 +3306,7 @@
         e = hipGetLastError();
     }
     if (e == hipSuccess) e = hipMemcpyAsync(hc.data(), ctr, (size_t)world * 8, hipMemcpyDeviceToHost, s);
-    if (e == hipSuccess) e = hipStreamSynchronize(s);
+    if (e == hipSuccess) e = gb_sync(s);
     unsigned long long run = 0;
     for (int w = 0; w < world; ++w) {
         cur[w] = run;
@@ -3144,7 +3319,7 @@
             gb_route_kernel<<<g, 256, 0, s>>>(k, n, world, 1, ctr + world, (uint32_t*)out_perm->values);
             e = hipGetLastError();
         }
-        if (e == hipSuccess) e = hipStreamSynchronize(s);
+        if (e == hipSuccess) e = gb_sync(s);
     }
     if (e != hipSuccess) {
         plgpu_column_release(out_perm);
@@ -3194,7 +3369,7 @@
         e = hipGetLastError();
     }
     if (e == hipSuccess) e = hipMemcpyAsync(h, st, sizeof h, hipMemcpyDeviceToHost, s);
-    if (e == hipSuccess) e = hipStreamSynchronize(s);
+    if (e == hipSuccess) e = gb_sync(s);
     if (e != hipSuccess) return hip_fail(e, "key range pass");
     for (int i = 0; i < nkeys; ++i) {
         out_ranges[3 * i] = (int64_t)(h[3 * i] ^ 0x8000000000000000ull);
@@ -3234,7 +3409,7 @@
         const int g = (int)std::min<int64_t>((n + 255) / 256, (int64_t)num_cus() * 16);
         mk_pack_launch(mk, pk, n, (uint64_t*)out_codes->values, nullptr, nullptr, g, s);
         hipError_t e = hipGetLastError();
-        if (e == hipSuccess) e = hipStreamSynchronize(s);
+        if (e == hipSuccess) e = gb_sync(s);
         if (e != hipSuccess) {
             plgpu_column_release(out_codes);
             return hip_fail(e, "mk_pack_kernel");
@@ -3275,7 +3450,7 @@
         if (e != hipSuccess) rc = hip_fail(e, "mk_unpack_kernel");
     }
     if (!rc) {
-        hipError_t e = hipStreamSynchronize(s);
+        hipError_t e = gb_sync(s);
         if (e != hipSuccess) rc = hip_fail(e, "key unpack");
     }
     if (rc)
@@ -3309,7 +3484,7 @@
         float_code_kernel<<<g, 256, 0, s>>>(to_dev(*keys), n, (int64_t*)out_codes->values,
                                             (uint64_t*)out_codes->validity);
         hipError_t e = hipGetLastError();
-        if (e == hipSuccess) e = hipStreamSynchronize(s);
+        if (e == hipSuccess) e = gb_sync(s);
         if (e != hipSuccess) {
             plgpu_column_release(out_codes);
             return hip_fail(e, "float key codes");
@@ -3392,7 +3567,7 @@
         std::memcpy(h.data(), start.data(), (size_t)(nsrc + 1) * 8);
         std::memcpy(h.data() + (size_t)(nsrc + 1) * 8, shift.data(), shift.size() * 4);
         hipError_t e = hipMemcpyAsync(dsrc, h.data(), bytes, hipMemcpyHostToDevice, R.s);
-        if (e == hipSuccess) e = hipStreamSynchronize(R.s);
+        if (e == hipSuccess) e = gb_sync(R.s);
         if (e != hipSuccess) return hip_fail(e, "merge sources");
     }
     for (R.attempts = 0;; ++R.attempts) {
@@ -3415,7 +3590,7 @@
             e = hipGetLastError();
         }
         if (e == hipSuccess) e = hipMemcpyAsync(R.st, R.status, sizeof R.st, hipMemcpyDeviceToHost, R.s);
-        if (e == hipSuccess) e = hipStreamSynchronize(R.s);
+        if (e == hipSuccess) e = gb_sync(R.s);
         if (e != hipSuccess) {
             rc = hip_fail(e, "gb_merge_kernel");
             break;
@@ -3582,7 +3757,7 @@
             rc = gb_plan(R, nullptr);
         }
         if (!rc && !R.kp_fallback) {
-            rc = gb_main(R, true, nullptr, nullptr);
+            rc = gb_main_then_finalize(R, naggs);
             if (!rc && R.kp_bad) {
                 if (!checked) return fail(PLGPU_ERR_HIP, "fused key packing: a row outside the exact packing plan");
                 *repack = true;
@@ -3609,7 +3784,7 @@
         }
         unsigned int bad = 0;
         if (e == hipSuccess && outside) e = hipMemcpyAsync(&bad, outside, 4, hipMemcpyDeviceToHost, s);
-        if (e == hipSuccess && outside) e = hipStreamSynchronize(s);
+        if (e == hipSuccess && outside) e = gb_sync(s);
         if (e != hipSuccess) rc = hip_fail(e, "mk_pack_kernel");
         if (!rc && bad) {
             *repack = true;
@@ -3629,7 +3804,7 @@
             rc = gb_prepare(R, &ck, cols, ncols, program, n_instr, aggs, naggs, maintain_order != 0, false, stream,
                             deriv);
         if (!rc) rc = gb_plan(R, nullptr);
-        if (!rc) rc = gb_main(R, true, nullptr, nullptr);
+        if (!rc) rc = gb_main_then_finalize(R, naggs);
         if (!rc && info) gb_fill_info(R, info);
         if (!rc) rc = gb_finalize(R, naggs, &hout, out_aggs);
     }
@@ -3646,7 +3821,7 @@
     const int64_t n = key.length;
     int64_t data_end = 0;
     PLGPU_HIP(hipMemcpyAsync(&data_end, (const int64_t*)key.values + key.offset + n, 8, hipMemcpyDeviceToHost, s));
-    PLGPU_HIP(hipStreamSynchronize(s));
+    PLGPU_HIP(gb_sync(s));
     KeyPack kp;
     std::memset(&kp, 0, sizeof kp);
     kp.n = 1;
@@ -3666,7 +3841,7 @@
         rc = gb_plan(R, nullptr);
     }
     if (rc || R.kp_fallback) return rc;
-    rc = gb_main(R, true, nullptr, nullptr);
+    rc = gb_main_then_finalize(R, naggs);
     if (rc || R.kp_bad) return rc;
     plgpu_column hout;
     std::memset(&hout, 0, sizeof hout);
@@ -3801,7 +3976,7 @@
         R.want_first = true;
         rc = gb_prepare(R, &hk, cols, ncols, program, n_instr, aggs, naggs, maintain_order != 0, false, stream, deriv);
         if (!rc) rc = gb_plan(R, nullptr);
-        if (!rc) rc = gb_main(R, true, nullptr, nullptr);
+        if (!rc) rc = gb_main_then_finalize(R, naggs);
         if (rc) break;
         plgpu_column hout;
         DevBuf<uint64_t> first;
@@ -3821,7 +3996,7 @@
             vw.reset();
             e = hipGetLastError();
             if (e == hipSuccess) e = hipMemcpyAsync(&coll, collision, 4, hipMemcpyDeviceToHost, s);
-            if (e == hipSuccess) e = hipStreamSynchronize(s);
+            if (e == hipSuccess) e = gb_sync(s);
             if (e != hipSuccess) rc = hip_fail(e, "mk_verify_kernel");
         }
         if (!rc && !coll) {
@@ -3843,7 +4018,7 @@
                 if (e != hipSuccess) rc = hip_fail(e, "mk_gather_key_kernel");
             }
             if (!rc) {
-                e = hipStreamSynchronize(s);
+                e = gb_sync(s);
                 if (e != hipSuccess) rc = hip_fail(e, "multi-key gather");
             }
             if (!rc && info) {
@@ -3904,7 +4079,7 @@
         out_aggs[i].null_count = (has_valid && !valid) ? 1 : 0;
     }
     if (rc == PLGPU_OK) {
-        hipError_t e = hipStreamSynchronize(s);
+        hipError_t e = gb_sync(s);
         if (e != hipSuccess) rc = hip_fail(e, "empty reduction");
     }
     if (rc)
@@ -4003,7 +4178,7 @@
     var_finalize_kernel<<<g, 256, 0, s>>>(to_dev(*sum_sq), to_dev(*count), n, ddof, take_sqrt,
                                           (double*)out->values, (uint64_t*)out->validity);
     hipError_t e = hipGetLastError();
-    if (e == hipSuccess) e = hipStreamSynchronize(s);
+    if (e == hipSuccess) e = gb_sync(s);
     if (e != hipSuccess) {
         plgpu_column_release(out);
         return hip_fail(e, "var finalize");
@@ -4165,7 +4340,7 @@
         }
         e = hipGetLastError();
     }
-    if (e == hipSuccess) e = hipStreamSynchronize(s);
+    if (e == hipSuccess) e = gb_sync(s);
     if (e != hipSuccess) {
         plgpu_column_release(out);
         return hip_fail(e, "squared deviations");
diff --git a/polaroid_amd/csrc/plgpu_internal.hpp b/polaroid_amd/csrc/plgpu_internal.hpp
--- a/polaroid_amd/csrc/plgpu_internal.hpp
+++ b/polaroid_amd/csrc/plgpu_internal.hpp
@@ -68,8 +68,11 @@
     int join_radix_batch = 0;
     int over_presorted = 1;
     int asof_path = 0;
+    int gb_burst = 1;
+    int plan_cache_rows = -1;
 };
 Options& options();
+void gb_wait_note();
 
 void gb_plan_cache_clear();
 hipEvent_t ev_acquire();
diff --git a/polaroid_amd/csrc/runtime.cpp b/polaroid_amd/csrc/runtime.cpp
--- a/polaroid_amd/csrc/runtime.cpp
+++ b/polaroid_amd/csrc/runtime.cpp
@@ -3,6 +3,7 @@
 #include <cstdio>
 #include <cstdlib>
 #include <algorithm>
+#include <atomic>
 #include <cmath>
 #include <cstdint>
 #include <cstring>
@@ -81,6 +82,8 @@
     {"join_radix_load", "PLGPU_JOIN_RADIX_LOAD", &Options::join_radix_load},
     {"join_radix_batch", "PLGPU_JOIN_RADIX_BATCH", &Options::join_radix_batch},
     {"asof_path", "PLGPU_ASOF_PATH", &Options::asof_path},
+    {"gb_burst", "PLGPU_GB_BURST", &Options::gb_burst},
+    {"plan_cache_rows", "PLGPU_PLAN_CACHE_ROWS", &Options::plan_cache_rows},
 };
 const OptField* opt_field(const char* name) {
     for (const OptField& f : kOptFields)
@@ -102,6 +105,9 @@
     static Options o = read_env_options();
     return o;
 }
+
+static std::atomic<int64_t> g_gb_waits{0};
+void gb_wait_note() { g_gb_waits.fetch_add(1, std::memory_order_relaxed); }
 
 namespace {
 struct KtPending {
@@ -864,6 +870,10 @@
 
 PLGPU_API int plgpu_get_option(const char* name, int64_t* out) {
     if (name == nullptr || out == nullptr) return fail(PLGPU_ERR_INVALID, "NULL argument");
+    if (!strcmp(name, "gb_waits")) {
+        *out = g_gb_waits.load(std::memory_order_relaxed);
+        return PLGPU_OK;
+    }
     const OptField* f = opt_field(name);
     if (f == nullptr) return fail(PLGPU_ERR_INVALID, std::string("unknown option ") + name);
     *out = options().*(f->f);
```

After: 144,800 Mrows/s. No clear change (-0.8%).
